# PreibischLab/multiview-simulation

Measured on AMD Instinct MI355X. Metric: simulated Mvoxel/s (views x input voxels / s), 512^3 volume x 8 views, higher is better.
Workload: dtype f32 (f64 attenuation/reductions/Poisson)

## Files before the change

include/mvsim.h:

```cpp
#ifndef MVSIM_H
#define MVSIM_H

#include <stddef.h>
#include <stdint.h>

#ifdef __cplusplus
extern "C" {
#endif

#define MVSIM_OK       0
#define MVSIM_EINVAL  (-1)
#define MVSIM_ENOMEM  (-2)
#define MVSIM_EHIP    (-3)
#define MVSIM_EFFT    (-4)
#define MVSIM_ERCCL   (-5)
#define MVSIM_ENODEV  (-6)

typedef struct mvsim_ctx mvsim_ctx;

const char* mvsim_version(void);
const char* mvsim_last_error(void);
int  mvsim_device_count(int* count);
int  mvsim_create(int device, mvsim_ctx** ctx);
int  mvsim_destroy(mvsim_ctx* ctx);
// ... 368 lines not shown
    int64_t  dim[3];
    int64_t  min[3], max[3];
    int32_t  inc;  float snr;
    uint64_t seed; uint32_t stream;
} mvsim_interval_job;
int mvsim_interval_out_dim(const mvsim_interval_job* job, int64_t out_dim[3]);
int mvsim_extract_intervals_dev(mvsim_ctx* ctx, const mvsim_interval_job* jobs, int n, float* const* out_dev);
int mvsim_extract_intervals(mvsim_ctx* ctx, const mvsim_interval_job* jobs, int n, float* const* out_host);
int mvsim_tile_interval(const int64_t dim[3], const double overlap_ratio[3], int tile,
                        int64_t min[3], int64_t max[3], int64_t overlap[3]);

typedef struct mvsim_view_params {
    int32_t  axis;
    int32_t  degrees;
    double   delta;
    float    min_value;
    float    target_average;
    int32_t  inc;
    float    snr;
    uint64_t seed;
    uint32_t stream;
    int32_t  conv_method;
} mvsim_view_params;

typedef struct mvsim_view_outputs {
    float* rot;
    float* att;
    float* con;
    float* acq;
} mvsim_view_outputs;

void mvsim_view_params_default(mvsim_view_params* p);

int mvsim_simulate_view_dev(mvsim_ctx* ctx, const float* gt, const int64_t dim[3],
                            float* psf_host, const int64_t kdim[3],
                            const mvsim_view_params* params, const mvsim_view_outputs* out,
                            double* correction);
int mvsim_simulate_views_dev(mvsim_ctx* ctx, const float* gt, const int64_t dim[3], float* const* psf_host,
                             const int64_t kdim[3], const mvsim_view_params* params, const mvsim_view_outputs* outs,
                             int n_views);
int mvsim_simulate_views(mvsim_ctx* ctx, const float* gt_host, const int64_t dim[3], float* const* psf_host,
                         const int64_t kdim[3], const mvsim_view_params* params, float* const* acq_host, int n_views);
typedef struct mvsim_iteration_outputs {
    float* iso;
    float* view;
    float* view_weights;
    float* view_psf;
} mvsim_iteration_outputs;
int mvsim_simulate_iteration_dev(mvsim_ctx* ctx, const float* gt, const int64_t dim[3],
                                 float* psf_host, const int64_t kdim[3],
                                 const mvsim_view_params* params, int back_degrees,
                                 const mvsim_view_outputs* out, const mvsim_iteration_outputs* more);
int mvsim_simulate_view(mvsim_ctx* ctx, const float* gt, const int64_t dim[3],
                        float* psf_host, const int64_t kdim[3],
                        const mvsim_view_params* params, const mvsim_view_outputs* out,
                        double* correction);

int mvsim_simulate_view_async(mvsim_ctx* ctx, const float* gt_host, uint64_t gt_generation, const int64_t dim[3],
                              float* psf_host, const int64_t kdim[3], const mvsim_view_params* params,
                              const mvsim_view_outputs* out_host, int64_t* ticket);
int mvsim_wait(mvsim_ctx* ctx, int64_t ticket, double* correction);
int mvsim_get_transfer_stats(mvsim_ctx* ctx, int64_t* views_as_u16, int64_t* fallbacks);
int mvsim_simulate_view_zslabs(mvsim_ctx* ctx, const float* const* gt_slabs, const int64_t* gt_slab_nz, int n_gt_slabs,
                               const int64_t dim[3], float* psf_host, const int64_t kdim[3],
                               const mvsim_view_params* params, float* const* acq_slabs, const int64_t* acq_slab_nz,
                               int n_acq_slabs, double* correction);

int mvsim_rotate_around_axis_zslabs(mvsim_ctx* ctx, const float* const* in_slabs, const int64_t* in_slab_nz, int n_in, const int64_t dim[3],
                                    int axis, int degrees, float* const* out_slabs, const int64_t* out_slab_nz, int n_out);
int mvsim_attenuate3d_zslabs(mvsim_ctx* ctx, const float* const* in_slabs, const int64_t* in_slab_nz, int n_in, const int64_t dim[3],
                             double delta, float* const* out_slabs, const int64_t* out_slab_nz, int n_out);
int mvsim_convolve_zslabs(mvsim_ctx* ctx, const float* const* in_slabs, const int64_t* in_slab_nz, int n_in, const int64_t dim[3],
                          float* psf, const int64_t kdim[3], int method, float* const* out_slabs, const int64_t* out_slab_nz, int n_out);
int mvsim_extract_slices_zslabs(mvsim_ctx* ctx, const float* const* in_slabs, const int64_t* in_slab_nz, int n_in, const int64_t dim[3],
                                int inc, float snr, uint64_t seed, uint32_t stream, float* const* out_slabs, const int64_t* out_slab_nz,
                                int n_out);

typedef struct mvsim_timings {
    float rotate_ms, attenuate_ms, psf_ms, convolve_ms, adjust_ms, extract_ms, total_ms;
    float pass_a_ms, pass_b_ms, pass_c_ms, pass_d_ms, pass_e_ms;
} mvsim_timings;
int mvsim_fft_geometry(const int64_t dim[3], const int64_t kdim[3], int64_t geometry[5]);
int mvsim_zpass_geometry(const int64_t dim[3], const int64_t kdim[3], int inc, int64_t out[4]);
int mvsim_stencil_geometry(const int64_t kdim[3], int64_t geometry[5]);
int mvsim_extract_path(const int64_t dim[3], int inc, int index_inc, uint64_t index_offset, int aligned16, int queue_share, int64_t path[4]);
int mvsim_get_extract_path(mvsim_ctx* ctx, int64_t path[5]);
int mvsim_fused_tail_geometry(mvsim_ctx* ctx, const int64_t dim[3], const int64_t kdim[3], int inc, int want_con, int64_t out[2]);
int mvsim_get_plane_stats(mvsim_ctx* ctx, int64_t stats[3]);
int mvsim_get_tail_path(mvsim_ctx* ctx, int64_t out[2]);
int mvsim_get_psf_cache_stats(mvsim_ctx* ctx, int64_t out[4]);
int mvsim_get_queue_stats(mvsim_ctx* ctx, int64_t stats[6]);
int mvsim_enable_timing(mvsim_ctx* ctx, int enable);
int mvsim_get_timings(mvsim_ctx* ctx, mvsim_timings* t);

#define MVSIM_UNIQUE_ID_BYTES 128
int mvsim_comm_unique_id(unsigned char id[MVSIM_UNIQUE_ID_BYTES]);
int mvsim_comm_init(mvsim_ctx* ctx, int nranks, int rank, const unsigned char id[MVSIM_UNIQUE_ID_BYTES]);
int mvsim_comm_library_info(char* path, size_t path_capacity, int* version);
int mvsim_comm_broadcast_volume(mvsim_ctx* ctx, float* vol_dev, int64_t count, int root);
int mvsim_comm_register_volume(mvsim_ctx* ctx, float* vol_dev, int64_t count);
typedef struct mvsim_bcast_op { int32_t stage, kind, peer, pad; int64_t first, count; } mvsim_bcast_op;
int mvsim_comm_broadcast_plan(int nranks, int rank, int root, int64_t count, int pieces, mvsim_bcast_op* ops, int capacity, int* n_ops);
int mvsim_comm_unregister_volume(mvsim_ctx* ctx, const float* vol_dev);
int mvsim_comm_allreduce_sum(mvsim_ctx* ctx, float* buf_dev, int64_t count);
int mvsim_comm_allreduce_sum_f64(mvsim_ctx* ctx, double* value_host);
int mvsim_comm_allreduce_sum_f64_dev(mvsim_ctx* ctx, double* value_dev, void* hip_stream);
int mvsim_comm_destroy(mvsim_ctx* ctx);
int mvsim_shard_views(int n_views, int nranks, int rank, int* view_idx, int max_out);

typedef struct mvsim_group mvsim_group;
int        mvsim_group_create(int ndev, const int* devices, mvsim_group** group);
int        mvsim_group_destroy(mvsim_group* group);
int        mvsim_group_size(const mvsim_group* group);
mvsim_ctx* mvsim_group_ctx(mvsim_group* group, int index);
int        mvsim_group_broadcast_volume(mvsim_group* group, const float* gt_host, const int64_t dim[3]);
int        mvsim_group_simulate_views(mvsim_group* group, float* const* psf_host, const int64_t kdim[3],
                                      const mvsim_view_params* params, int n_views, float* const* acq_host);

int mvsim_slab_range(int64_t nz, int nranks, int rank, int64_t* z0, int64_t* z1);
int mvsim_view_slab_convolve_dev(mvsim_ctx* ctx, const float* gt, const int64_t dim[3], float* psf_host,
                                 const int64_t kdim[3], const mvsim_view_params* params, int64_t z0, int64_t z1,
                                 double* slab_sum);
int mvsim_view_slab_finish_dev(mvsim_ctx* ctx, const int64_t dim[3], const mvsim_view_params* params, int64_t z0,
                               int64_t z1, double total_sum, float* acq, int64_t* n_planes);
int mvsim_view_slab_dev(mvsim_ctx* ctx, mvsim_ctx* comm_ctx, const float* gt, const int64_t dim[3], float* psf_host,
                        const int64_t kdim[3], const mvsim_view_params* params, int64_t z0, int64_t z1, float* acq,
                        int64_t* n_planes);

#ifdef __cplusplus
}
#endif
#endif
```

multiview-simulation_amd/__init__.py:

```python
from __future__ import annotations

import ctypes as C
import math
import os

import numpy as np

from . import _lib
from ._lib import DeconParams, DeconStat, IntervalJob, MvsimError, MvsimNoDeviceError, Sphere, Timings, ViewOutputs, ViewParams
from .aberrations import ContextAberrations
from .deconvolution import ContextDeconvolution, MultiViewDeconvolution, decon_geometry, decon_params, flip_psf
from .detection import ContextDetection, DifferenceOfGaussian, dog_geometry, dog_params, dog_taps
from ._lib import DogParams, MatchParams
from .registration import BeadRegistration, ContextRegistration, descriptor_subsets, fit_affine, match_geometry, match_params
from ._lib import FuseParams, FuseView
from .fusion import (ContextFusion, ViewFusion, fuse_invert, fuse_params, fusion_bounds, fusion_geometry, psf_matrix,
                     transform_psf)
from ._lib import PsfParams, PsfResult
from .psf import (ContextPsf, PsfExtraction, gaussian_psf, psf_finish, psf_geometry, psf_offsets, psf_params, psf_rendered,
                  psf_select)
from .phantoms import ContextPhantoms

__all__ = ["AffineTransform3D", "BeadRegistration", "Context", "DeconParams", "DifferenceOfGaussian", "DogParams", "MatchParams", "MultiViewDeconvolution", "Group", "Hessian", "HypersphereCollectionRealRandomAccessible", "JavaRandom", "Lightsheet",
           "PerlinNoiseRealRandomAccessible", "PointRejectionSampling", "RayTracingTest", "Raytrace", "RefractiveIndexMap", "ClearingMap", "SimpleCalculatedRealRandomAccessible", "SimulateBeads",
           "SimulateBeads2", "SimulateMultiViewAberrations", "SimulateMultiViewDataset", "Tools", "VolumeInjection", "broadcast_plan", "default_context", "MvsimError", "MvsimNoDeviceError", "ViewParams", "shard_views",
           "version", "zpass_geometry", "ViewFusion", "FuseParams", "PsfExtraction", "PsfParams"]


def broadcast_plan(nranks: int, rank: int, root: int, count: int, pieces: int = 8):
    L = _lib.load()
    n = C.c_int(0)
    _lib.check(L.mvsim_comm_broadcast_plan(nranks, rank, root, count, pieces, None, 0, C.byref(n)))
    ops = (_lib.BcastOp * max(1, n.value))()
    _lib.check(L.mvsim_comm_broadcast_plan(nranks, rank, root, count, pieces, ops, n.value, C.byref(n)))
    return [(o.stage, "send" if o.kind == 0 else "recv", o.peer, o.first, o.count) for o in ops[: n.value]]


def version() -> str:
    return _lib.load().mvsim_version().decode()


def zpass_geometry(dim_xyz, kdim_xyz, inc: int = 1):
    g = (C.c_int64 * 4)()
    rc = _lib.load().mvsim_zpass_geometry((C.c_int64 * 3)(*dim_xyz), (C.c_int64 * 3)(*kdim_xyz), int(inc), g)
    return tuple(int(x) for x in g) if rc == 0 else None


class JavaRandom:
    _MULT = 0x5DEECE66D
    _MASK = (1 << 48) - 1

    def __init__(self, seed: int):
        self.setSeed(seed)

    def setSeed(self, seed: int) -> None:
        self._s = (seed ^ self._MULT) & self._MASK
        self._pending = None

    def next(self, bits: int) -> int:
        self._s = (self._s * self._MULT + 0xB) & self._MASK
        v = self._s >> (48 - bits)
        v &= 0xFFFFFFFF
        return v - (1 << 32) if v & 0x80000000 else v

    def nextInt(self, bound: int | None = None) -> int:
        if bound is None:
            return self.next(32)
        if bound <= 0:
            raise ValueError("bound must be positive")
        r = self.next(31)
        m = bound - 1
        if bound & m == 0:
            return (bound * r) >> 31
        u = r
        while True:
            r = u % bound
            t = (u - r + m) & 0xFFFFFFFF
            if not (t & 0x80000000):
                return r
            u = self.next(31)

    def nextLong(self) -> int:
        v = ((self.next(32) << 32) + self.next(32)) & 0xFFFFFFFFFFFFFFFF
        return v - (1 << 64) if v & (1 << 63) else v

    def nextDouble(self) -> float:
        return ((self.next(26) << 27) + self.next(27)) * (1.0 / (1 << 53))

    def nextGaussian(self) -> float:
        from .phantoms import strict_log
        if self._pending is not None:
            g, self._pending = self._pending, None
            return g
        while True:
            v1 = 2 * self.nextDouble() - 1
            v2 = 2 * self.nextDouble() - 1
            s = v1 * v1 + v2 * v2
            if not (s >= 1 or s == 0):
                break
        multiplier = math.sqrt(-2 * strict_log(s) / s)
        self._pending = v2 * multiplier
        return v1 * multiplier

    def shuffle(self, lst: list) -> None:
        for i in range(len(lst), 1, -1):
            j = self.nextInt(i)
            lst[i - 1], lst[j] = lst[j], lst[i - 1]


def _seed_from(rnd) -> int:
    if rnd is None:
        rnd = SimulateMultiViewDataset.rnd
    if isinstance(rnd, int):
        return rnd & 0xFFFFFFFFFFFFFFFF
    return rnd.nextLong() & 0xFFFFFFFFFFFFFFFF


def _as_volume(a, name="image") -> np.ndarray:
    v = np.ascontiguousarray(a, dtype=np.float32)
    if v.ndim != 3:
        raise ValueError(f"{name}: expected 3 dimensions, got {v.ndim}")
    if v.size == 0:
        raise ValueError(f"{name}: empty interval")
    return v


def _dim(v: np.ndarray):
    nz, ny, nx = v.shape
# ... 1069 lines not shown
```

multiview-simulation_amd/_lib.py:

```python
from __future__ import annotations

import ctypes as C
import os

HERE = os.path.dirname(os.path.abspath(__file__))
LIB_PATH = os.path.join(HERE, "libmvsim.so")

MVSIM_OK, MVSIM_EINVAL, MVSIM_ENOMEM, MVSIM_EHIP, MVSIM_EFFT, MVSIM_ERCCL, MVSIM_ENODEV = 0, -1, -2, -3, -4, -5, -6
UNIQUE_ID_BYTES = 128


class MvsimError(RuntimeError):

    def __init__(self, status: int, message: str):
        super().__init__(f"libmvsim status {status}: {message}")
        self.status = status


class MvsimNoDeviceError(MvsimError):
    pass


class ViewParams(C.Structure):
    _fields_ = [
# ... 125 lines not shown
    def as_dict(self):
        return {n: float(getattr(self, n)) for n, _ in self._fields_}


_i64p = C.POINTER(C.c_int64)
_vp = C.c_void_p
_dp = C.POINTER(C.c_double)

SIGNATURES = {
    "mvsim_version": (C.c_char_p, []),
    "mvsim_last_error": (C.c_char_p, []),
    "mvsim_device_count": (C.c_int, [C.POINTER(C.c_int)]),
    "mvsim_create": (C.c_int, [C.c_int, C.POINTER(_vp)]),
    "mvsim_destroy": (C.c_int, [_vp]),
    "mvsim_set_stream": (C.c_int, [_vp, _vp]),
    "mvsim_synchronize": (C.c_int, [_vp]),
    "mvsim_join": (C.c_int, [_vp]),
    "mvsim_set_option": (C.c_int, [_vp, C.c_char_p, C.c_char_p]),
    "mvsim_release_caches": (C.c_int, [_vp]),
    "mvsim_dev_alloc": (C.c_int, [_vp, C.c_size_t, C.POINTER(_vp)]),
    "mvsim_dev_free": (C.c_int, [_vp, _vp]),
    "mvsim_upload": (C.c_int, [_vp, _vp, _vp, C.c_size_t]),
    "mvsim_dev_memset": (C.c_int, [_vp, _vp, C.c_int, C.c_size_t]),
    "mvsim_host_alloc": (C.c_int, [_vp, C.c_size_t, C.POINTER(C.c_void_p)]),
    "mvsim_host_free": (C.c_int, [_vp, _vp]),
    "mvsim_download": (C.c_int, [_vp, _vp, _vp, C.c_size_t]),
    "mvsim_axis_rotation": (C.c_int, [_i64p, C.c_int, C.c_int, C.POINTER(C.c_double)]),
    "mvsim_extract_nz": (C.c_int64, [C.c_int64, C.c_int]),
    "mvsim_isotropic_nz": (C.c_int64, [C.c_int64, C.c_int]),
    "mvsim_poisson_mul": (C.c_double, [C.c_double]),
    "mvsim_rotate_around_axis": (C.c_int, [_vp, _vp, _i64p, C.c_int, C.c_int, _vp]),
    "mvsim_attenuate3d": (C.c_int, [_vp, _vp, _i64p, C.c_double, _vp]),
    "mvsim_norm_image": (C.c_int, [_vp, _vp, C.c_int64]),
    "mvsim_convolve": (C.c_int, [_vp, _vp, _i64p, _vp, _i64p, C.c_int, _vp]),
    "mvsim_adjust_image": (C.c_int, [_vp, _vp, C.c_int64, C.c_float, C.c_float, C.POINTER(C.c_double)]),
    "mvsim_extract_slices": (C.c_int, [_vp, _vp, _i64p, C.c_int, C.c_float, C.c_uint64, C.c_uint32, _vp]),
    "mvsim_poisson_process": (C.c_int, [_vp, _vp, C.c_int64, C.c_double, C.c_uint64, C.c_uint32, C.c_uint64]),
    "mvsim_make_isotropic": (C.c_int, [_vp, _vp, _i64p, C.c_int, _vp]),
    "mvsim_compute_weight_image": (C.c_int, [_vp, _i64p, _vp]),
    "mvsim_rotate_around_axis_dev": (C.c_int, [_vp, _vp, _i64p, C.c_int, C.c_int, _vp]),
    "mvsim_attenuate3d_dev": (C.c_int, [_vp, _vp, _i64p, C.c_double, _vp]),
    "mvsim_convolve_dev": (C.c_int, [_vp, _vp, _i64p, _vp, _i64p, C.c_int, _vp]),
    "mvsim_adjust_image_dev": (C.c_int, [_vp, _vp, C.c_int64, C.c_float, C.c_float, C.POINTER(C.c_double)]),
    "mvsim_extract_slices_dev": (C.c_int, [_vp, _vp, _i64p, C.c_int, C.c_float, C.c_uint64, C.c_uint32, _vp]),
    "mvsim_make_isotropic_dev": (C.c_int, [_vp, _vp, _i64p, C.c_int, _vp]),
    "mvsim_interval_out_dim": (C.c_int, [C.POINTER(IntervalJob), _i64p]),
    "mvsim_extract_intervals_dev": (C.c_int, [_vp, C.POINTER(IntervalJob), C.c_int, C.POINTER(_vp)]),
    "mvsim_extract_intervals": (C.c_int, [_vp, C.POINTER(IntervalJob), C.c_int, C.POINTER(_vp)]),
    "mvsim_tile_interval": (C.c_int, [_i64p, _dp, C.c_int, _i64p, _i64p, _i64p]),
    "mvsim_draw_spheres": (C.c_int, [_vp, _vp, _i64p, C.c_double, C.c_double, C.c_int, C.c_int,
                                     C.POINTER(C.c_uint64), C.POINTER(C.c_int64)]),
    "mvsim_draw_spheres_dev": (C.c_int, [_vp, _vp, _i64p, C.c_double, C.c_double, C.c_int, C.c_int,
                                         C.POINTER(C.c_uint64), C.POINTER(C.c_int64)]),
    "mvsim_downsample2x": (C.c_int, [_vp, _vp, _i64p, _vp]),
    "mvsim_downsample2x_dev": (C.c_int, [_vp, _vp, _i64p, _vp]),
    "mvsim_compute_weight_image_dev": (C.c_int, [_vp, _i64p, _vp]),
    "mvsim_sum_views_dev": (C.c_int, [_vp, C.POINTER(_vp), C.c_int, C.c_int64, _vp]),
    "mvsim_normalize_weights_dev": (C.c_int, [_vp, C.POINTER(_vp), C.c_int, C.c_int64, _vp, C.c_float]),
    "mvsim_normalize_weights": (C.c_int, [_vp, C.POINTER(_vp), C.c_int, C.c_int64, C.c_float]),
    "mvsim_view_params_default": (None, [C.POINTER(ViewParams)]),
    "mvsim_simulate_view_dev": (C.c_int, [_vp, _vp, _i64p, _vp, _i64p, C.POINTER(ViewParams),
                                          C.POINTER(ViewOutputs), C.POINTER(C.c_double)]),
    "mvsim_get_plane_stats": (C.c_int, [_vp, _i64p]),
    "mvsim_get_tail_path": (C.c_int, [_vp, _i64p]),
    "mvsim_get_psf_cache_stats": (C.c_int, [_vp, _i64p]),
    "mvsim_get_queue_stats": (C.c_int, [_vp, _i64p]),
    "mvsim_get_transfer_stats": (C.c_int, [_vp, C.POINTER(C.c_int64), C.POINTER(C.c_int64)]),
    "mvsim_simulate_views_dev": (C.c_int, [_vp, _vp, _i64p, C.POINTER(_vp), _i64p, C.POINTER(ViewParams),
                                           C.POINTER(ViewOutputs), C.c_int]),
    "mvsim_simulate_views": (C.c_int, [_vp, _vp, _i64p, C.POINTER(_vp), _i64p, C.POINTER(ViewParams), C.POINTER(_vp), C.c_int]),
    "mvsim_simulate_iteration_dev": (C.c_int, [_vp, _vp, _i64p, _vp, _i64p, C.POINTER(ViewParams), C.c_int,
                                               C.POINTER(ViewOutputs), C.POINTER(IterationOutputs)]),
    "mvsim_simulate_view": (C.c_int, [_vp, _vp, _i64p, _vp, _i64p, C.POINTER(ViewParams),
                                      C.POINTER(ViewOutputs), C.POINTER(C.c_double)]),
    "mvsim_splat_spheres": (C.c_int, [_vp, _vp, _i64p, _vp, C.c_int64]),
    "mvsim_splat_spheres_dev": (C.c_int, [_vp, _vp, _i64p, _vp, C.c_int64]),
    "mvsim_simulate_view_async": (C.c_int, [_vp, _vp, C.c_uint64, _i64p, _vp, _i64p, C.POINTER(ViewParams),
                                            C.POINTER(ViewOutputs), C.POINTER(C.c_int64)]),
    "mvsim_wait": (C.c_int, [_vp, C.c_int64, C.POINTER(C.c_double)]),
    "mvsim_simulate_view_zslabs": (C.c_int, [_vp, C.POINTER(_vp), _i64p, C.c_int, _i64p, _vp, _i64p, C.POINTER(ViewParams),
                                             C.POINTER(_vp), _i64p, C.c_int, C.POINTER(C.c_double)]),
    "mvsim_fft_geometry": (C.c_int, [_i64p, _i64p, _i64p]),
    "mvsim_zpass_geometry": (C.c_int, [_i64p, _i64p, C.c_int, _i64p]),
    "mvsim_rotate_around_axis_zslabs": (C.c_int, [_vp, C.POINTER(_vp), _i64p, C.c_int, _i64p, C.c_int, C.c_int, C.POINTER(_vp), _i64p, C.c_int]),
    "mvsim_attenuate3d_zslabs": (C.c_int, [_vp, C.POINTER(_vp), _i64p, C.c_int, _i64p, C.c_double, C.POINTER(_vp), _i64p, C.c_int]),
    "mvsim_convolve_zslabs": (C.c_int, [_vp, C.POINTER(_vp), _i64p, C.c_int, _i64p, _vp, _i64p, C.c_int, C.POINTER(_vp), _i64p, C.c_int]),
    "mvsim_extract_slices_zslabs": (C.c_int, [_vp, C.POINTER(_vp), _i64p, C.c_int, _i64p, C.c_int, C.c_float, C.c_uint64, C.c_uint32,
                                              C.POINTER(_vp), _i64p, C.c_int]),
    "mvsim_stencil_geometry": (C.c_int, [_i64p, _i64p]),
    "mvsim_extract_path": (C.c_int, [_i64p, C.c_int, C.c_int, C.c_uint64, C.c_int, C.c_int, _i64p]),
    "mvsim_fused_tail_geometry": (C.c_int, [_vp, _i64p, _i64p, C.c_int, C.c_int, _i64p]),
    "mvsim_get_extract_path": (C.c_int, [_vp, _i64p]),
    "mvsim_enable_timing": (C.c_int, [_vp, C.c_int]),
    "mvsim_get_timings": (C.c_int, [_vp, C.POINTER(Timings)]),
    "mvsim_comm_unique_id": (C.c_int, [C.POINTER(C.c_ubyte)]),
    "mvsim_comm_init": (C.c_int, [_vp, C.c_int, C.c_int, C.POINTER(C.c_ubyte)]),
    "mvsim_comm_library_info": (C.c_int, [C.c_char_p, C.c_size_t, C.POINTER(C.c_int)]),
    "mvsim_comm_broadcast_volume": (C.c_int, [_vp, _vp, C.c_int64, C.c_int]),
    "mvsim_comm_broadcast_plan": (C.c_int, [C.c_int, C.c_int, C.c_int, C.c_int64, C.c_int, _vp, C.c_int, C.POINTER(C.c_int)]),
    "mvsim_comm_register_volume": (C.c_int, [_vp, _vp, C.c_int64]),
    "mvsim_comm_unregister_volume": (C.c_int, [_vp, _vp]),
    "mvsim_comm_allreduce_sum": (C.c_int, [_vp, _vp, C.c_int64]),
    "mvsim_comm_allreduce_sum_f64": (C.c_int, [_vp, C.POINTER(C.c_double)]),
    "mvsim_slab_range": (C.c_int, [C.c_int64, C.c_int, C.c_int, C.POINTER(C.c_int64), C.POINTER(C.c_int64)]),
    "mvsim_view_slab_convolve_dev": (C.c_int, [_vp, _vp, _i64p, _vp, _i64p, _vp, C.c_int64, C.c_int64,
                                               C.POINTER(C.c_double)]),
    "mvsim_view_slab_finish_dev": (C.c_int, [_vp, _i64p, _vp, C.c_int64, C.c_int64, C.c_double, _vp,
                                             C.POINTER(C.c_int64)]),
    "mvsim_view_slab_dev": (C.c_int, [_vp, _vp, _vp, _i64p, _vp, _i64p, _vp, C.c_int64, C.c_int64, _vp, C.POINTER(C.c_int64)]),
    "mvsim_comm_allreduce_sum_f64_dev": (C.c_int, [_vp, _vp, _vp]),
    "mvsim_host_copy": (C.c_int, [_vp, _vp, _vp, C.c_size_t]),
    "mvsim_comm_destroy": (C.c_int, [_vp]),
    "mvsim_group_create": (C.c_int, [C.c_int, C.POINTER(C.c_int), C.POINTER(_vp)]),
    "mvsim_group_destroy": (C.c_int, [_vp]),
    "mvsim_group_size": (C.c_int, [_vp]),
    "mvsim_group_ctx": (_vp, [_vp, C.c_int]),
    "mvsim_group_broadcast_volume": (C.c_int, [_vp, _vp, _i64p]),
    "mvsim_group_simulate_views": (C.c_int, [_vp, C.POINTER(_vp), _i64p, C.POINTER(ViewParams), C.c_int, C.POINTER(_vp)]),
    "mvsim_shard_views": (C.c_int, [C.c_int, C.c_int, C.c_int, C.POINTER(C.c_int), C.c_int]),
    "mvsim_beads_random_points": (C.c_int, [C.POINTER(C.c_uint64), C.c_int64, _i64p, _i64p, C.POINTER(C.c_double)]),
    "mvsim_render_beads": (C.c_int, [_vp, C.POINTER(C.c_double), _i64p, C.c_int64, C.POINTER(C.c_double), C.c_int, _i64p, _i64p,
                                     C.POINTER(C.c_double), C.POINTER(_vp), C.POINTER(_vp)]),
    "mvsim_render_beads_dev": (C.c_int, [_vp, C.POINTER(C.c_double), _i64p, C.c_int64, C.POINTER(C.c_double), C.c_int, _i64p, _i64p,
                                         C.POINTER(C.c_double), C.POINTER(_vp), C.POINTER(_vp)]),
    "mvsim_beads_normalize": (C.c_int, [_vp, _vp, C.c_int64]),
    "mvsim_beads_normalize_dev": (C.c_int, [_vp, _vp, C.c_int64]),
    "mvsim_perlin_init": (C.c_int, [C.POINTER(C.c_uint64), C.c_int32, _dp, C.POINTER(C.c_int32), _dp]),
    "mvsim_perlin_at": (C.c_int, [_vp, C.POINTER(Perlin), _vp, C.c_int64, _vp]),
    "mvsim_perlin_at_dev": (C.c_int, [_vp, C.POINTER(Perlin), _vp, C.c_int64, _vp]),
    "mvsim_perlin_raster": (C.c_int, [_vp, C.POINTER(Perlin), _i64p, _i64p, _vp]),
    "mvsim_perlin_raster_dev": (C.c_int, [_vp, C.POINTER(Perlin), _i64p, _i64p, _vp]),
    "mvsim_spheres_at": (C.c_int, [_vp, C.POINTER(SphereSet), _vp, C.c_int64, _vp]),
    "mvsim_spheres_at_dev": (C.c_int, [_vp, C.POINTER(SphereSet), _vp, C.c_int64, _vp]),
    "mvsim_spheres_raster": (C.c_int, [_vp, C.POINTER(SphereSet), _i64p, _i64p, C.c_int, _vp]),
    "mvsim_spheres_raster_dev": (C.c_int, [_vp, C.POINTER(SphereSet), _i64p, _i64p, C.c_int, _vp]),
    "mvsim_rejection_sample": (C.c_int, [_vp, C.POINTER(C.c_uint64), _dp, _dp, C.c_int64, C.POINTER(Density), C.c_int64, _dp,
                                         C.POINTER(C.c_int64)]),
    "mvsim_lightsheet_fit": (C.c_int, [C.c_double, C.c_double, C.c_double, C.c_double, _dp]),
    "mvsim_hessian_at": (C.c_int, [_vp, _vp, _i64p, _dp, C.c_int64, _dp, _dp, _dp]),
    "mvsim_hessian_at_dev": (C.c_int, [_vp, _vp, _i64p, _dp, C.c_int64, _dp, _dp, _dp]),
    "mvsim_hessian_images": (C.c_int, [_vp, _vp, _i64p, _vp, _vp]),
    "mvsim_hessian_images_dev": (C.c_int, [_vp, _vp, _i64p, _vp, _vp]),
    "mvsim_refract3d_ray_starts": (C.c_int, [_vp, C.POINTER(C.c_uint64), _i64p, C.c_int, C.c_int, _dp, C.c_int64, _dp, _dp]),
    "mvsim_camera_ray_starts": (C.c_int, [_vp, C.POINTER(C.c_uint64), _i64p, C.c_int, _dp]),
    "mvsim_refract3d": (C.c_int, [_vp, _vp, _vp, _i64p, C.c_int, C.c_int, C.c_double, C.c_double, C.c_double, C.c_int64,
                                  C.POINTER(C.c_uint64), _vp, _vp, C.POINTER(RaySteps)]),
    "mvsim_refract3d_dev": (C.c_int, [_vp, _vp, _vp, _i64p, C.c_int, C.c_int, C.c_double, C.c_double, C.c_double, C.c_int64,
                                      C.POINTER(C.c_uint64), _vp, _vp, C.POINTER(RaySteps)]),
    "mvsim_trace_params_default": (C.c_int, [_i64p, C.POINTER(TraceParams)]),
    "mvsim_trace_rays": (C.c_int, [_vp, _vp, _vp, _i64p, _dp, _dp, C.POINTER(C.c_float), C.c_int64, C.POINTER(TraceParams), _vp, _vp,
                                   C.POINTER(RaySteps), _dp, _dp, C.POINTER(C.c_int64)]),
    "mvsim_trace_rays_dev": (C.c_int, [_vp, _vp, _vp, _i64p, _dp, _dp, C.POINTER(C.c_float), C.c_int64, C.POINTER(TraceParams), _vp, _vp,
                                       C.POINTER(RaySteps), _dp, _dp, C.POINTER(C.c_int64)]),
    "mvsim_sandbox_ray_starts": (C.c_int, [_vp, C.POINTER(C.c_uint64), _i64p, C.c_int, C.c_int, C.c_int64, _dp, _dp]),
    "mvsim_grid_ray_starts": (C.c_int, [_vp, _i64p, C.c_int, C.c_int, C.c_int64, _dp, _dp, C.POINTER(C.c_int64)]),
    "mvsim_draw_simple_image": (C.c_int, [_vp, _vp, _i64p, C.c_float, C.c_float]),
    "mvsim_draw_simple_image_dev": (C.c_int, [_vp, _vp, _i64p, C.c_float, C.c_float]),
    "mvsim_hessian_plane": (C.c_int, [_vp, _vp, _i64p, C.c_int, _vp, _vp]),
    "mvsim_hessian_plane_dev": (C.c_int, [_vp, _vp, _i64p, C.c_int, _vp, _vp]),
    "mvsim_volume_inject": (C.c_int, [_vp, _vp, _vp, _i64p, _dp, _dp, _dp, C.c_int64, C.c_int]),
    "mvsim_volume_inject_dev": (C.c_int, [_vp, _vp, _vp, _i64p, _dp, _dp, _dp, C.c_int64, C.c_int]),
    "mvsim_volume_inject_info": (C.c_int, [_dp, C.POINTER(C.c_int32), _dp, C.POINTER(C.c_int32)]),
    "mvsim_volume_normalize": (C.c_int, [_vp, _vp, _vp, C.c_int64, _vp]),
    "mvsim_volume_normalize_dev": (C.c_int, [_vp, _vp, _vp, C.c_int64, _vp]),
    "mvsim_volume_project": (C.c_int, [_vp, _vp, _vp, _i64p, _vp]),
    "mvsim_volume_project_dev": (C.c_int, [_vp, _vp, _vp, _i64p, _vp]),
# ... 90 lines not shown
```

multiview-simulation_amd/build.py:

```python
from __future__ import annotations

import os
import shutil
import subprocess
import sys

HERE = os.path.dirname(os.path.abspath(__file__))
CSRC = os.path.join(HERE, "csrc")
LIB = os.path.join(HERE, "libmvsim.so")
SOURCES = ["api.cpp", "api_view.cpp", "api_host.cpp", "api_sims.cpp", "comm.cpp", "kernels.hip", "rotate.hip", "extract.hip", "extract_interval.hip", "fftconv.hip", "fft_driver.hip", "fft_passes.hip", "zconv.hip", "rotate_fft.hip", "stencil.hip", "phantom.hip", "beads.hip", "aberrations.hip", "raytrace.hip", "procedural.hip", "sphere_walk.hip", "api_decon.cpp", "deconvolve.hip", "api_detect.cpp", "detect.hip", "api_register.cpp", "register.hip", "api_fuse.cpp", "fuse.hip", "api_psf.cpp", "psf.hip"]
HEADERS = ["common.h", "api_internal.h", "host_pool.h", "jrandom.h", "extract_plan.h", "interval_plan.h", "poisson_dev.h", "poisson_recipe.h", "fft_dev.h", "fft_host.h", "rotate_rounds.h", "row_bits.h", "rotate_dev.h", "sphere_walk.h", "aberr_dev.h", "bricks.h", "decon.h", "detect.h", "register.h", "register_dev.h", "fuse.h", "fuse_dev.h", "psf.h", "psf_dev.h", "psf_cache.h", "../../include/mvsim.h"]
ROCM = os.environ.get("ROCM_PATH", "/opt/rocm")


def _hipcc() -> str:
    for cand in (os.path.join(ROCM, "bin", "hipcc"), shutil.which("hipcc")):
        if cand and os.path.exists(cand):
            return cand
    raise RuntimeError("hipcc not found (ROCm toolchain required to build libmvsim.so)")


def sources():
    return [os.path.join(CSRC, s) for s in SOURCES if os.path.exists(os.path.join(CSRC, s))]


def source_sha() -> str:
    import hashlib
    h = hashlib.sha256()
    files = sorted(sources() + [os.path.normpath(os.path.join(CSRC, x)) for x in HEADERS])
    for f in files:
        h.update(os.path.basename(f).encode() + b"\0")
        with open(f, "rb") as fh:
            h.update(fh.read())
    return h.hexdigest()[:16]


def _common_flags():
    return [
        "--offload-arch=gfx950", "-O3", "-std=c++17", "-fPIC", "-ffp-contract=off", "-fno-fast-math",
        *os.environ.get("MVSIM_EXTRA_CFLAGS", "").split(),
        "-Wall", "-Wno-unused-result", "-I" + os.path.join(ROCM, "include"),
    ]


def is_current() -> bool:
    if not os.path.exists(LIB) or not os.path.exists(LIB + ".flags"):
        return False
    with open(LIB + ".flags") as fh:
        if fh.read() != " ".join(_common_flags()):
            return False
    t = os.path.getmtime(LIB)
    deps = sources() + [os.path.normpath(os.path.join(CSRC, h)) for h in HEADERS] + [os.path.abspath(__file__)]
    return all(os.path.getmtime(d) <= t for d in deps if os.path.exists(d))


def build(force: bool = False, verbose: bool = False) -> str:
    if not force and is_current():
        return LIB
    hipcc = _hipcc()
    objs = []
    os.makedirs(os.path.join(HERE, "build"), exist_ok=True)
    common = _common_flags()
    flags_id = " ".join(common)
    hdr_time = max(os.path.getmtime(os.path.normpath(os.path.join(CSRC, h))) for h in HEADERS)
    hdr_time = max(hdr_time, os.path.getmtime(os.path.abspath(__file__)))
    procs = []
    for src in sources():
        obj = os.path.join(HERE, "build", os.path.basename(src) + ".o")
        objs.append(obj)
        stamp = obj + ".flags"
        fresh = (not force and os.path.exists(obj) and os.path.exists(stamp) and open(stamp).read() == flags_id
                 and os.path.getmtime(obj) >= max(os.path.getmtime(src), hdr_time))
        if fresh:
            continue
        cmd = [hipcc, "-x", "hip", "-c", src, "-o", obj] + common
        if verbose:
            print(" ".join(cmd), file=sys.stderr)
        procs.append((src, stamp, subprocess.Popen(cmd, stdout=subprocess.PIPE, stderr=subprocess.STDOUT, text=True)))
    failed = False
    for src, stamp, p in procs:
        out, _ = p.communicate()
        if p.returncode != 0:
            failed = True
            if os.path.exists(stamp):
                os.remove(stamp)
            sys.stderr.write(f"--- {src} ---\n{out}\n")
        else:
            with open(stamp, "w") as fh:
                fh.write(flags_id)
            if verbose and out.strip():
                sys.stderr.write(out)
    if failed:
        raise RuntimeError("hipcc failed")
    link = [hipcc, "-shared", "-fPIC", "--offload-arch=gfx950", "-o", LIB] + objs + [
# ... 13 lines not shown
```

multiview-simulation_amd/csrc/api.cpp:

```cpp
#include "api_internal.h"

#include <cstdlib>
#include <mutex>
#include <thread>

namespace mvsim {

static thread_local char g_err[512] = "";

void set_error(const char* fmt, ...)
{
    va_list ap;
    va_start(ap, fmt);
    vsnprintf(g_err, sizeof(g_err), fmt, ap);
    va_end(ap);
}

int parse_option(Options& o, const char* name, const char* value)
{
    if (!name || !value) return MVSIM_EINVAL;
    const std::string n(name), v(value);
    auto word = [&](std::initializer_list<std::pair<const char*, int>> words, auto* dst) {
        for (const auto& w : words)
            if (v == w.first) { *dst = w.second; return MVSIM_OK; }
        return MVSIM_EINVAL;
    };
    auto flag = [&](bool* dst) { return word({{"1", 1}, {"on", 1}, {"true", 1}, {"0", 0}, {"off", 0}, {"false", 0}}, dst); };
    auto number = [&](size_t digits, long long lo, long long hi, auto* dst, int when_auto = -1) {
        if (when_auto >= 0 && v == "auto") { *dst = when_auto; return MVSIM_OK; }
        if (v.empty() || v.size() > digits || v.find_first_not_of("0123456789") != std::string::npos) return MVSIM_EINVAL;
        const long long k = atoll(v.c_str());
        if (k < lo || k > hi) return MVSIM_EINVAL;
        *dst = k;
        return MVSIM_OK;
    };
    if (n == "fft_zpass") return word({{"auto", 0}, {"direct", 1}, {"fft", 2}, {"inline", 3}}, &o.zpass);
    if (n == "fft_backend") return word({{"custom", 0}, {"auto", 0}, {"rocfft", 1}}, &o.rocfft);
    if (n == "fused_rotate") return word({{"1", 1}, {"on", 1}, {"lds", 1}, {"0", 0}, {"off", 0}, {"2", 2}, {"lane", 2}, {"3", 3}, {"auto", 3}}, &o.fused_rotate);
    if (n == "poisson_queue") return word({{"1", 1}, {"on", 1}, {"0", 0}, {"off", 0}}, &o.poisson_queue);
    if (n == "poisson_queue_share") return number(2, 1, 16, &o.poisson_queue_share, 0);
    if (n == "attenuate") return word({{"serial", 0}, {"scan", 1}}, &o.attenuate_scan);
    if (n == "early_sum") return flag(&o.early_sum);
    if (n == "zconv_strided") return flag(&o.zconv_strided);
    if (n == "exp") return number(2, 0, 15, &o.exp);
    if (n == "beads_pair_cap") return number(10, 1024, 1LL << 31, &o.beads_pair_cap);
    if (n == "reject_batch") return number(7, 1, 1LL << 20, &o.reject_batch, 0);
    if (n == "dog_pass") return word({{"both", 0}, {"xy", 1}, {"z", 2}}, &o.dog_pass);
    if (n == "sphere_walk") return word({{"host", 0}, {"device", 1}, {"device_only", 2}, {"auto", -1}}, &o.sphere_walk);
    if (n == "fuse_tail") return flag(&o.fuse_tail);
    if (n == "psf_overlap") return flag(&o.psf_overlap);
    if (n == "fused_fftx") return word({{"auto", 2}, {"1", 1}, {"on", 1}, {"0", 0}, {"off", 0}, {"roles", 3}}, &o.fused_fftx);
    if (n == "tail_overlap") return word({{"0", 0}, {"off", 0}, {"1", 1}, {"on", 1}, {"own", 1}, {"2", 2}, {"any", 2}}, &o.tail_overlap);
    if (n == "acq_transfer") return word({{"auto", 1}, {"u16", 1}, {"f32", 0}}, &o.acq_u16);
    if (n == "host_threads") return number(3, 1, 256, &o.host_threads, 0);
    if (n == "view_batch") return word({{"auto", 2}, {"1", 1}, {"on", 1}, {"0", 0}, {"off", 0}}, &o.view_batch);
    if (n == "view_lanes") return number(2, 1, MVSIM_MAX_VIEWS, &o.view_lanes, 0);
    if (n == "graph") { bool g = false; const int rc = flag(&g); o.graph = g ? 1 : 0; return rc; }
    if (n == "broadcast") {
        int how = 0;
        if (word({{"scatter_allgather", 0}, {"auto", 0}, {"ring", 1}, {"peer_copy", 2}, {"pipelined", 3}}, &how) != MVSIM_OK) return MVSIM_EINVAL;
        o.bcast_ring = how == 1; o.bcast_peer_copy = how == 2; o.bcast_pipelined = how == 3;
        return MVSIM_OK;
    }
    if (n == "skip_empty") return flag(&o.skip_empty);
    if (n == "skip_rows") return flag(&o.skip_rows);
    if (n == "skip_tail") return flag(&o.skip_tail);
    if (n == "psf_cache") return number(7, 0, 1 << 20, &o.psf_cache);
    if (n == "fft_pad") {
        long long a = 0, b = 0, c = 0;
        if (v == "auto" || v.empty()) { o.fft_pad[0] = o.fft_pad[1] = o.fft_pad[2] = 0; return MVSIM_OK; }
        if (sscanf(v.c_str(), "%lld,%lld,%lld", &a, &b, &c) != 3 || a < 0 || b < 0 || c < 0) return MVSIM_EINVAL;
        o.fft_pad[0] = a; o.fft_pad[1] = b; o.fft_pad[2] = c;
        return MVSIM_OK;
    }
    return MVSIM_EINVAL;
}

const Options& env_options()
{
    static Options o;
    static std::once_flag once;
    std::call_once(once, [] {
        if (const char* e = getenv("MVSIM_FFT_ZPASS")) (void)parse_option(o, "fft_zpass", e);
        if (const char* e = getenv("MVSIM_FFT_BACKEND")) (void)parse_option(o, "fft_backend", e);
        if (const char* e = getenv("MVSIM_FFT_PAD")) (void)parse_option(o, "fft_pad", e);
        if (getenv("MVSIM_NO_FUSED_ROTATE")) o.fused_rotate = 0;
        if (getenv("MVSIM_POISSON_NOQUEUE")) o.poisson_queue = 0;
        if (getenv("MVSIM_NO_EARLY_SUM")) o.early_sum = false;
        if (getenv("MVSIM_NO_FUSE_TAIL")) o.fuse_tail = false;
        if (const char* e = getenv("MVSIM_GRAPH")) (void)parse_option(o, "graph", e);
        if (const char* e = getenv("MVSIM_BROADCAST")) (void)parse_option(o, "broadcast", e);
        if (const char* e = getenv("MVSIM_OPTIONS")) {
            std::string all(e);
            size_t pos = 0;
            while (pos < all.size()) {
                size_t end = all.find(';', pos);
                if (end == std::string::npos) end = all.size();
                const std::string kv = all.substr(pos, end - pos);
                const size_t eq = kv.find('=');
                if (eq != std::string::npos) (void)parse_option(o, kv.substr(0, eq).c_str(), kv.substr(eq + 1).c_str());
                pos = end + 1;
            }
        }
    });
    return o;
}

int ensure_lds_attr(mvsim_ctx* ctx, const void* kernel, size_t bytes)
{
    if (bytes <= 64 * 1024) return MVSIM_OK;
    if (bytes > 160 * 1024) { set_error("kernel needs %zu bytes of LDS (> 160 KiB)", bytes); return MVSIM_EINVAL; }
    if (ctx->lds_attr_set.count(kernel)) return MVSIM_OK;
    MVSIM_HIP(hipFuncSetAttribute(kernel, hipFuncAttributeMaxDynamicSharedMemorySize, 160 * 1024));
    ctx->lds_attr_set.insert(kernel);
    return MVSIM_OK;
}

int DevBuf::reserve(size_t need)
{
    if (need <= bytes) return MVSIM_OK;
    if (epoch) *epoch += 1;
    if (p) { (void)hipFree(p); p = nullptr; bytes = 0; }
    hipError_t e = hipMalloc(&p, need);
    if (e != hipSuccess) {
        p = nullptr;
        set_error("hipMalloc(%zu bytes) failed: %s", need, hipGetErrorString(e));
// ... 799 lines not shown
    if (fallbacks) *fallbacks = ctx->u16_fallbacks;
    return MVSIM_OK;
}

int mvsim_stencil_geometry(const int64_t kdim[3], int64_t geometry[5])
{
    if (!kdim || !geometry) { set_error("invalid argument: null pointer"); return MVSIM_EINVAL; }
    if (!stencil_chunk_geometry(kdim, geometry)) {
        set_error("direct stencil: PSF outside 1..64 taps per axis");
        return MVSIM_EINVAL;
    }
    return MVSIM_OK;
}

int mvsim_extract_path(const int64_t dim[3], int inc, int index_inc, uint64_t index_offset, int aligned16, int queue_share, int64_t path[4])
{
    if (!dim || !path) { set_error("invalid argument: null pointer"); return MVSIM_EINVAL; }
    MVSIM_TRY(check_dim(dim));
    MVSIM_CHECK_ARG(inc >= 1 && index_inc >= 0, "inc must be >= 1 and index_inc >= 0");
    MVSIM_CHECK_ARG(0 <= queue_share && queue_share <= 16, "queue_share must be 0 (no queue) or 1..16 sixteenths");
    extract_path(dim, inc, index_inc, index_offset, aligned16 != 0, queue_share, path);
    return MVSIM_OK;
}

int mvsim_get_extract_path(mvsim_ctx* ctx, int64_t path[5])
{
    MVSIM_CHECK_ARG(ctx != nullptr && path != nullptr, "null pointer");
    std::memcpy(path, ctx->extract_path, sizeof(ctx->extract_path));
    return MVSIM_OK;
}

int mvsim_get_tail_path(mvsim_ctx* ctx, int64_t out[2])
{
    MVSIM_CHECK_ARG(ctx != nullptr && out != nullptr, "null pointer");
    out[0] = ctx->tail_path[0]; out[1] = ctx->tail_path[1];
    return MVSIM_OK;
}

int mvsim_get_psf_cache_stats(mvsim_ctx* ctx, int64_t out[4])
{
    MVSIM_CHECK_ARG(ctx != nullptr && out != nullptr, "null pointer");
    const PsfCache::Stats& st = ctx->psf_cache.stats();
    out[0] = st.hits; out[1] = st.misses; out[2] = st.evictions; out[3] = st.bytes;
    return MVSIM_OK;
}

int mvsim_fused_tail_geometry(mvsim_ctx* ctx, const int64_t dim[3], const int64_t kdim[3], int inc, int want_con, int64_t out[2])
{
    MVSIM_CHECK_ARG(ctx != nullptr && dim && kdim && out, "null pointer");
    MVSIM_TRY(check_dim(dim));
    MVSIM_CHECK_ARG(inc >= 1, "inc must be >= 1");
    ExtractPlan fp{};
    if (!ctx->opt.fuse_tail || ctx->opt.poisson_queue != 1 || !fused_tail_geometry(dim, kdim, inc, want_con != 0, ctx->opt, &fp)) {
        set_error("this view would not take the fused tail");
        return MVSIM_EINVAL;
    }
    out[0] = fp.blocks; out[1] = fp.segcap;
    return MVSIM_OK;
}

int mvsim_fft_geometry(const int64_t dim[3], const int64_t kdim[3], int64_t geometry[5])
{
    if (!dim || !kdim || !geometry) { set_error("invalid argument: null pointer"); return MVSIM_EINVAL; }
    MVSIM_TRY(check_dim(dim));
    if (!custom_fft_geometry(dim, kdim, geometry, env_options())) {
        set_error("no hand-written FFT size for this volume / PSF");
        return MVSIM_EINVAL;
    }
    return MVSIM_OK;
}

int mvsim_zpass_geometry(const int64_t dim[3], const int64_t kdim[3], int inc, int64_t out[4])
{
    if (!dim || !kdim || !out) { set_error("invalid argument: null pointer"); return MVSIM_EINVAL; }
    MVSIM_TRY(check_dim(dim));
    MVSIM_CHECK_ARG(inc >= 1, "inc must be >= 1");
    if (!custom_zpass_geometry(dim, kdim, inc, out, env_options())) {
        set_error("this view's z pass is not the direct convolution");
        return MVSIM_EINVAL;
    }
    return MVSIM_OK;
}

int mvsim_enable_timing(mvsim_ctx* ctx, int enable)
{
    MVSIM_TRY(set_device(ctx));
    if (enable && !ctx->ev_created) {
        for (int k = 0; k < mvsim_ctx::TIMING_SLOTS; ++k)
            for (int s = 0; s < ST_COUNT; ++s) {
                MVSIM_HIP(hipEventCreate(&ctx->evr[k][s][0]));
                MVSIM_HIP(hipEventCreate(&ctx->evr[k][s][1]));
            }
        ctx->ev_created = true;
    }
    ctx->timing = enable != 0;
    ctx->ev_cur = 0;
    ctx->ev_calls = 0;
    for (int s = 0; s < ST_COUNT; ++s) ctx->ev_used[0][s] = false;
    return MVSIM_OK;
}

int mvsim_get_timings(mvsim_ctx* ctx, mvsim_timings* t)
{
    MVSIM_TRY(set_device(ctx));
    MVSIM_CHECK_ARG(t != nullptr, "timings pointer is null");
    MVSIM_CHECK_ARG(ctx->ev_created, "timing was never enabled");
    MVSIM_HIP(hipStreamSynchronize(ctx->stream));
    double sum[ST_COUNT] = {};
    int cnt[ST_COUNT] = {};
    const long long calls = ctx->ev_calls == 0 ? 1 : ctx->ev_calls;
    const int nslots = (int)(calls < mvsim_ctx::TIMING_SLOTS ? calls : mvsim_ctx::TIMING_SLOTS);
    for (int j = 0; j < nslots; ++j) {
        const int k = ((ctx->ev_cur - j) % mvsim_ctx::TIMING_SLOTS + mvsim_ctx::TIMING_SLOTS) % mvsim_ctx::TIMING_SLOTS;
        for (int s = 0; s < ST_COUNT; ++s) {
            if (!ctx->ev_used[k][s]) continue;
            float ms = 0.f;
            MVSIM_HIP(hipEventElapsedTime(&ms, ctx->evr[k][s][0], ctx->evr[k][s][1]));
            sum[s] += ms;
            cnt[s] += 1;
            ctx->ev_used[k][s] = false;
        }
    }
    float ms[ST_COUNT];
    float total = 0.f;
    for (int s = 0; s < ST_COUNT; ++s) {
        ms[s] = cnt[s] ? (float)(sum[s] / cnt[s]) : 0.f;
        if (s == ST_PSF && cnt[ST_CONVOLVE] > cnt[s]) ms[s] = (float)(sum[s] / cnt[ST_CONVOLVE]);
        if (s == ST_PSF && ctx->psf_on_side) ms[s] = 0.f;
        if (s < ST_PASS_A) total += ms[s];
    }
    t->rotate_ms = ms[ST_ROTATE]; t->attenuate_ms = ms[ST_ATTENUATE]; t->psf_ms = ms[ST_PSF];
    t->convolve_ms = ms[ST_CONVOLVE]; t->adjust_ms = ms[ST_ADJUST]; t->extract_ms = ms[ST_EXTRACT];
    t->total_ms = total;
    t->pass_a_ms = ms[ST_PASS_A]; t->pass_b_ms = ms[ST_PASS_B]; t->pass_c_ms = ms[ST_PASS_C];
    t->pass_d_ms = ms[ST_PASS_D]; t->pass_e_ms = ms[ST_PASS_E];
    ctx->last = *t;
    ctx->ev_cur = 0;
    ctx->ev_calls = 0;
    return MVSIM_OK;
}

}
```

multiview-simulation_amd/csrc/api_view.cpp:

```cpp
#include "api_internal.h"

using namespace mvsim;

void mvsim::view_graphs_release(mvsim_ctx* ctx)
{
    for (auto& g : ctx->graphs) {
        if (g.exec) (void)hipGraphExecDestroy(g.exec);
        if (g.graph) (void)hipGraphDestroy(g.graph);
    }
    ctx->graphs.clear();
    ctx->graph_seen.clear();
}

extern "C" {

static bool ranges_meet(const void* a, size_t abytes, const char* lo, const char* hi)
{
    const char* p = reinterpret_cast<const char*>(a);
    return a && lo && p < hi && lo < p + abytes;
}

static int view_enqueue(mvsim_ctx* ctx, const float* gt, const int64_t dim[3], const int64_t kdim[3], const mvsim_view_params* p,
                        const mvsim_view_outputs* o, bool overlap_ok = false)
{
// ... 45 lines not shown
    const int method = pick_method(p->conv_method, kdim);
    const bool materialise = o->con != nullptr;
    const bool noise = p->snr >= 0.0f;
    ConvTail tail;
    tail.zstride = (!materialise && p->inc > 1 && (!noise || ctx->opt.poisson_queue == 1)) ? p->inc : 1;
    tail.corr_n = n; tail.min_value = p->min_value; tail.target_average = p->target_average;
    tail.x_done = x_done;
    tail.plane_nz = x_done ? plane_nz : nullptr;
    tail.row_bits = x_done ? row_bits : nullptr;
    tail.want_sparse = tail.plane_nz != nullptr &&
                       tail_sparse_caller(ctx->opt.skip_tail, materialise, extract_stage_queued(ctx, dim, p->inc, noise));
    if (method == 1 && ctx->opt.fuse_tail && (!noise || ctx->opt.poisson_queue == 1)) {
        const size_t qb = noise ? fused_tail_queue_bytes(dim, kdim, p->inc, materialise, ctx->opt) : 0;
        if (!noise || qb > 0) {
            if (qb) MVSIM_TRY(ctx->pqueue.reserve(qb));
            tail.want_fuse = true;
            tail.min_value = p->min_value; tail.target_average = p->target_average;
            tail.con_adj = materialise ? con : nullptr;
            tail.acq = o->acq; tail.inc = p->inc; tail.noise = noise;
            tail.mul = mvsim_poisson_mul((double)p->snr); tail.seed = p->seed; tail.stream = p->stream;
        }
    }
    MVSIM_TRY(convolve_dev_impl(ctx, att, dim, kdim, method, con, &tail));
    if (tail.fused) {
        const int64_t fused[5] = {EXTRACT_FUSED_TAIL, 0, tail.fused_blocks, noise ? (int64_t)tail.fused_segcap : 0, 1};
        std::memcpy(ctx->extract_path, fused, sizeof(fused));
        ctx->tail_path[0] = ctx->tail_path[1] = 0;
        return MVSIM_OK;
    }
    if (tail.sparse && (materialise || method != 1)) { set_error("sparse tail behind a view that did not ask for it"); return MVSIM_EINVAL; }

    ev_begin(ctx, ST_ADJUST);
    if (method == 2) MVSIM_TRY(launch_sum(ctx->stream, con, n, partial, scal));
    if (!tail.corr_done) MVSIM_TRY(launch_adjust_corr(ctx->stream, scal, n, p->min_value, p->target_average));
    if (materialise) MVSIM_TRY(launch_adjust_apply(ctx->stream, con, n, scal, p->min_value));
    ev_end(ctx, ST_ADJUST);

    const int64_t n_out = dim[0] * dim[1] * mvsim_extract_nz(dim[2], p->inc);
    ExtractOps ops;
    ops.in = con; ops.out = o->acq; ops.scal = scal;
    ops.min_value = p->min_value; ops.noise = noise; ops.mul = mvsim_poisson_mul((double)p->snr); ops.seed = p->seed; ops.stream = p->stream;
    ops.adjust = !materialise;
    if (tail.sparse) { ops.empty_flags = tail.sparse_flags; ops.empty_stride = tail.sparse_stride; }
    ExtractPlan xpl;
    MVSIM_TRY(extract_stage_plan(ctx, tail.zstride > 1 ? ExtractGeom::compact(dim, p->inc) : ExtractGeom::strided(dim, p->inc), ops, &xpl));
    if (x_done) overlap_ok = false;
    if (tail.sparse) overlap_ok = false;
    hipStream_t tail_on = ctx->stream;
    if (overlap_ok) {
        if (!ctx->tail_stream) {
            MVSIM_HIP(hipStreamCreateWithFlags(&ctx->tail_stream, hipStreamNonBlocking));
            MVSIM_HIP(hipEventCreateWithFlags(&ctx->ev_tail_fork, hipEventDisableTiming));
            MVSIM_HIP(hipEventCreateWithFlags(&ctx->ev_tail, hipEventDisableTiming));
        }
        MVSIM_HIP(hipEventRecord(ctx->ev_tail_fork, ctx->stream));
        MVSIM_HIP(hipStreamWaitEvent(ctx->tail_stream, ctx->ev_tail_fork, 0));
        tail_on = ctx->tail_stream;
    }
    StreamSwap swap(ctx, tail_on);
    MVSIM_TRY(extract_stage_run(ctx, xpl, ops));
    if (overlap_ok) {
        MVSIM_HIP(hipEventRecord(ctx->ev_tail, ctx->tail_stream));
        ctx->tail_pending = true;
        ctx->tail_lo[0] = reinterpret_cast<const char*>(o->acq); ctx->tail_hi[0] = ctx->tail_lo[0] + (size_t)n_out * sizeof(float);
        ctx->tail_lo[1] = reinterpret_cast<const char*>(con);    ctx->tail_hi[1] = ctx->tail_lo[1] + vbytes;
    }
    return MVSIM_OK;
}


static std::string view_graph_key(mvsim_ctx* ctx, const float* gt, const int64_t dim[3], const int64_t kdim[3],
                                  const mvsim_view_params* p, const mvsim_view_outputs* o)
{
    std::string k;
    auto add = [&](const void* ptr, size_t bytes) { k.append(reinterpret_cast<const char*>(ptr), bytes); };
    add(&gt, sizeof(gt)); add(dim, 3 * sizeof(int64_t)); add(kdim, 3 * sizeof(int64_t));
    add(&p->axis, sizeof(p->axis)); add(&p->degrees, sizeof(p->degrees)); add(&p->delta, sizeof(p->delta));
    add(&p->min_value, sizeof(p->min_value)); add(&p->target_average, sizeof(p->target_average)); add(&p->inc, sizeof(p->inc));
    add(&p->snr, sizeof(p->snr)); add(&p->seed, sizeof(p->seed)); add(&p->stream, sizeof(p->stream));
    add(&p->conv_method, sizeof(p->conv_method));
    add(&o->rot, sizeof(o->rot)); add(&o->att, sizeof(o->att)); add(&o->con, sizeof(o->con)); add(&o->acq, sizeof(o->acq));
    add(&ctx->stream, sizeof(ctx->stream));
    const Options& q = ctx->opt;
    const int oo[16] = {q.zpass, q.rocfft ? 1 : 0, q.fused_rotate, q.poisson_queue, q.early_sum ? 1 : 0, q.fuse_tail ? 1 : 0, q.psf_overlap ? 1 : 0,
                        q.attenuate_scan ? 1 : 0, q.fused_fftx, q.zconv_strided ? 1 : 0, q.skip_empty ? 1 : 0, q.exp, q.poisson_queue_share, ctx->queue_share_learned,
                        q.skip_rows ? 1 : 0, q.skip_tail ? 1 : 0};
    add(oo, sizeof(oo));
    add(q.fft_pad, sizeof(q.fft_pad));
    return k;
}

static int view_graph_launch(mvsim_ctx* ctx, const float* gt, const int64_t dim[3], const int64_t kdim[3], const mvsim_view_params* p,
                             const mvsim_view_outputs* o)
{
    const std::string key = view_graph_key(ctx, gt, dim, kdim, p, o);
    ctx->graph_tick += 1;
    const unsigned long long epoch = ctx->alloc_epoch;
    if (ctx->graph_epoch != epoch) {
        for (auto& g : ctx->graphs) { (void)hipGraphExecDestroy(g.exec); (void)hipGraphDestroy(g.graph); }
        ctx->graphs.clear();
        ctx->graph_epoch = epoch;
    }
    for (auto& g : ctx->graphs)
        if (g.key == key) {
            g.last_use = ctx->graph_tick;
            MVSIM_HIP(hipGraphLaunch(g.exec, ctx->stream));
            return MVSIM_OK;
        }
    if (!ctx->graph_seen.count(key)) {
        if (ctx->graph_seen.size() > 4096) ctx->graph_seen.clear();
        ctx->graph_seen.insert(key);
        return view_enqueue(ctx, gt, dim, kdim, p, o);
    }
    MVSIM_HIP(hipStreamBeginCapture(ctx->stream, hipStreamCaptureModeRelaxed));
    const int rc = view_enqueue(ctx, gt, dim, kdim, p, o);
    hipGraph_t graph = nullptr;
    const hipError_t e = hipStreamEndCapture(ctx->stream, &graph);
    if (rc != MVSIM_OK) { if (graph) (void)hipGraphDestroy(graph); return rc; }
    if (ctx->alloc_epoch != epoch) {
        if (graph) (void)hipGraphDestroy(graph);
        return view_enqueue(ctx, gt, dim, kdim, p, o);
    }
    if (e != hipSuccess || !graph) { set_error("hipStreamEndCapture failed: %s", hipGetErrorString(e)); return MVSIM_EHIP; }
    hipGraphExec_t exec = nullptr;
    const hipError_t ei = hipGraphInstantiate(&exec, graph, nullptr, nullptr, 0);
    if (ei != hipSuccess) { (void)hipGraphDestroy(graph); set_error("hipGraphInstantiate failed: %s", hipGetErrorString(ei)); return MVSIM_EHIP; }
    if (ctx->graphs.size() >= 32) {
        size_t victim = 0;
        for (size_t i = 1; i < ctx->graphs.size(); ++i) if (ctx->graphs[i].last_use < ctx->graphs[victim].last_use) victim = i;
        (void)hipGraphExecDestroy(ctx->graphs[victim].exec);
        (void)hipGraphDestroy(ctx->graphs[victim].graph);
        ctx->graphs.erase(ctx->graphs.begin() + (long)victim);
    }
    ctx->graphs.push_back(mvsim_ctx::ViewGraph{key, graph, exec, ctx->graph_tick});
    MVSIM_HIP(hipGraphLaunch(exec, ctx->stream));
    return MVSIM_OK;
}

static int simulate_view_dev(mvsim_ctx* ctx, const float* gt, const int64_t dim[3], float* psf_host, const int64_t kdim[3],
                             const mvsim_view_params* p, const mvsim_view_outputs* o, double* correction, bool keep_psf_dev)
{
    MVSIM_TRY(set_device(ctx, true));
    const bool overlap = ctx->opt.tail_overlap != 0 && (ctx->opt.tail_overlap == 2 || ctx->stream == ctx->own_stream) &&
                         !ctx->opt.graph && !correction && dim &&
                         dim[0] > 0 && dim[1] > 0 && dim[2] > 0 && dim[0] * dim[1] * dim[2] >= ((int64_t)1 << 24);
    if (!overlap) MVSIM_TRY(join_tail(ctx));
    MVSIM_TRY(check_dim(dim));
    MVSIM_CHECK_ARG(gt && p && o, "null pointer");
    MVSIM_CHECK_ARG(o->acq != nullptr, "outputs.acq is required");
    MVSIM_CHECK_ARG(p->axis >= 0 && p->axis <= 2, "axis must be 0, 1 or 2");
    MVSIM_CHECK_ARG(p->inc >= 1, "inc must be >= 1");
    MVSIM_CHECK_ARG(p->conv_method >= 0 && p->conv_method <= 2, "conv_method must be 0, 1 or 2");
    MVSIM_CHECK_ARG(dim[0] <= dim[1], "attenuate3d: Nx > Ny walks outside the interval in the reference");
    ev_next(ctx);
    MVSIM_TRY(psf_prepare(ctx, psf_host, kdim, dim, !keep_psf_dev && kdim && pick_method(p->conv_method, kdim) == 1));
    int64_t P[3];
    const bool capturable = pick_method(p->conv_method, kdim) == 2 || custom_fft_sizes(dim, kdim, P, ctx->opt);
    if (ctx->opt.graph && !ctx->timing && capturable) MVSIM_TRY(view_graph_launch(ctx, gt, dim, kdim, p, o));
    else MVSIM_TRY(view_enqueue(ctx, gt, dim, kdim, p, o, overlap));
    if (correction) {
        double *partial, *scal;
        MVSIM_TRY(scal_ptr(ctx, &partial, &scal));
        MVSIM_HIP(hipMemcpyAsync(correction, scal + 1, sizeof(double), hipMemcpyDeviceToHost, ctx->stream));
        MVSIM_HIP(hipStreamSynchronize(ctx->stream));
    }
    return MVSIM_OK;
}

int mvsim_simulate_view_dev(mvsim_ctx* ctx, const float* gt, const int64_t dim[3], float* psf_host,
// ... 367 lines not shown
```

multiview-simulation_amd/csrc/common.h:

```cpp
#pragma once

#include <hip/hip_runtime.h>
#include <rocfft/rocfft.h>
#include <roctracer/roctx.h>

#include <algorithm>
#include <array>
#include <cstdarg>
#include <cstdint>
#include <cstdio>
#include <map>
#include <string>
#include <type_traits>
#include <unordered_set>
#include <utility>
#include <vector>

#include "../../include/mvsim.h"
#include "extract_plan.h"
#include "interval_plan.h"
#include "psf_cache.h"
#include "rotate_dev.h"
#include "sphere_walk.h"

// ... 37 lines not shown
    do {                                                                                        \
        int rc_ = (expr);                                                                       \
        if (rc_ != MVSIM_OK) return rc_;                                                        \
    } while (0)

#define MVSIM_CHECK_ARG(cond, msg)                                                              \
    do {                                                                                        \
        if (!(cond)) {                                                                          \
            mvsim::set_error("invalid argument: %s", msg);                                      \
            return MVSIM_EINVAL;                                                                \
        }                                                                                       \
    } while (0)

struct DevBuf {
    void*  p     = nullptr;
    size_t bytes = 0;
    unsigned long long* epoch = nullptr;
    int    reserve(size_t need);
    void   release();
    template <class T> T* as() const { return reinterpret_cast<T*>(p); }
};

struct Scratch {
    DevBuf b[12];
    ~Scratch() { for (DevBuf& x : b) x.release(); }
};

inline int suggested_kernel_diameter(double sigma)
{
    if (!(sigma > 0)) return 3;
    const int s = 2 * (int)(3 * sigma + 0.5) + 1;
    return s > 3 ? s : 3;
}

inline bool affine_is_x_rotation(const Affine& a)
{
    return a.m[0] == 1.0 && a.m[1] == 0.0 && a.m[2] == 0.0 && a.m[3] == 0.0 && a.m[4] == 0.0 && a.m[8] == 0.0;
}

struct FftPlan {
    int64_t      P[3]      = {0, 0, 0};
    rocfft_plan  fwd       = nullptr;
    rocfft_plan  inv       = nullptr;
    rocfft_execution_info info = nullptr;
    size_t       work_bytes = 0;
};

struct PinnedRing {
    static constexpr int SLOTS = 4;
    void*      p[SLOTS]     = {};
    size_t     bytes[SLOTS] = {};
    hipEvent_t ev[SLOTS]    = {};
    bool       busy[SLOTS]  = {};
    int        next         = 0;
    int  acquire(size_t need, int* slot);
    void release_all();
};

struct CountsStaging {
    DevBuf dev;
    void*  host       = nullptr;
    size_t host_bytes = 0;
    std::vector<long long> count;
    std::vector<size_t>    body;
    std::vector<char>      packed;
    int  reserve(const long long* counts, int views);
    int  pack(hipStream_t s, int view, const float* src);
    int  fetch(hipStream_t s);
    int  land(mvsim_ctx* ctx, const float* const* src_dev, float* const* dst_host);
    void release();
};

struct Options {
    int     zpass = 0;
    bool    rocfft = false;
    int     fused_rotate = 3;
    int     fused_fftx = 2;
    bool    attenuate_scan = false;
    int     poisson_queue = 1;
    int     poisson_queue_share = 16;
    bool    early_sum = true;
    int     exp = 0;
    bool    zconv_strided = true;
    bool    psf_overlap = true;
    int     tail_overlap = 1;
    bool    fuse_tail = false;
    int     graph = 0;
    int     acq_u16 = 1;
    int     host_threads = 0;
    int     view_lanes = 0;
    int     view_batch = 2;
    bool    bcast_ring = false;
    bool    bcast_peer_copy = false;
    bool    bcast_pipelined = false;
    int64_t fft_pad[3] = {0, 0, 0};
    bool    skip_empty = true;
    bool    skip_rows = true;
    int     psf_cache = 1024;
    bool    skip_tail = true;
    int64_t beads_pair_cap = (int64_t)1 << 28;
    int64_t reject_batch = 0;
    int     dog_pass = 0;
    int     sphere_walk = -1;
};
const Options& env_options();
int parse_option(Options& o, const char* name, const char* value);

enum Stage { ST_ROTATE = 0, ST_ATTENUATE, ST_PSF, ST_CONVOLVE, ST_ADJUST, ST_EXTRACT, ST_PASS_A, ST_PASS_B, ST_PASS_C, ST_PASS_D,
             ST_PASS_E, ST_COUNT };

}

struct mvsim_ctx {
    mvsim_ctx();
    mvsim_ctx(const mvsim_ctx&) = delete;
    mvsim_ctx& operator=(const mvsim_ctx&) = delete;
    template <class F> void each_workspace(F&& f);
    unsigned long long alloc_epoch = 1;
    int         roctx_depth = 0;
    int         device     = 0;
    hipStream_t own_stream = nullptr;
    hipStream_t stream     = nullptr;
    int         num_cu     = 256;

    mvsim::DevBuf vol_a, vol_b, vol_c;
    mvsim::DevBuf out_buf;
    mvsim::DevBuf psf_dev;
    mvsim::PsfCache psf_cache;
    mvsim::PsfCache::Entry* psf_entry = nullptr;
    mvsim::DevBuf view_tab;
    mvsim::DevBuf interval_tab;
    mvsim::DevBuf stencil_psf;
    mvsim::PinnedRing pinned;
    mvsim::DevBuf fft_real;
    mvsim::DevBuf fft_spec_img, fft_spec_psf;
    mvsim::DevBuf fft_work;
    mvsim::DevBuf pqueue;
    mvsim::DevBuf sphere_list;
    mvsim::DevBuf beads_buf[8];
    mvsim::DevBuf proc_buf[10];
    mvsim::DevBuf walk_buf[4];
    mvsim::DevBuf plane_flags;
    int*          empty_hint = nullptr;
    unsigned int* queue_hint = nullptr;
    int           queue_share_learned = 0;
    int64_t       extract_path[5] = {-1, 0, 0, 0, 0};
    int64_t       tail_path[2] = {0, 0};
    int           views_since_flags = 0;
    mvsim::DevBuf weight_img;
    mvsim::DevBuf decon_work[2];
    mvsim::DevBuf decon_psf;
    mvsim::DevBuf decon_stat;
    mvsim::DevBuf detect_buf[6];
    mvsim::DevBuf register_buf[4];
    mvsim::DevBuf fuse_buf;
    mvsim::DevBuf psfx_buf[3];
    int64_t       weight_dim[3] = {0, 0, 0};
    mvsim::DevBuf host_gt, host_rot, host_att, host_con;
    mvsim::DevBuf partials;
    mvsim::DevBuf partials_e;
    mvsim::DevBuf cfft_f, cfft_g;
    mvsim::DevBuf cfft_g1, cfft_g2;
    mvsim::Options opt;
    std::unordered_set<const void*> lds_attr_set;
    std::map<std::string, void*> box_weights;
    mvsim::DevBuf partials_z;
// ... 193 lines not shown
                     int rays_per_pixel, int64_t n, double* pos3, double* dir3);
int aberr_hessian_at_dev(mvsim_ctx* ctx, const float* img, const int64_t dim[3], const double* xyz, int64_t n, double* matrix9,
                         double* eigvec3, double* eigval);
int aberr_hessian_images_dev(mvsim_ctx* ctx, const float* img, const int64_t dim[3], int z0, int planes, float* eigval, float* eigvec);
int64_t trace_rays_per_range(int64_t pair_cap, int64_t max_moves);
struct StepRanges {
    Scratch ws;
    int64_t rays_per_range = 0, max_rays = 0;
    int     max_moves = 0;
    double *slot_xyz = nullptr, *xyz = nullptr;
    float  *slot_val = nullptr, *val = nullptr;
    int    *moves = nullptr, *offs = nullptr;
    int reserve(mvsim_ctx* ctx, int64_t nrays, int max_moves);
    int finish(mvsim_ctx* ctx, const char* who, int64_t r0, int nr, const int64_t dim[3], const double sigma[3], double sumw, float* image,
               float* weight, mvsim_ray_steps* steps);
};
int trace_rays_dev(mvsim_ctx* ctx, const float* ri_img, const float* img, const int64_t dim[3], const double* pos3, const double* dir3,
                   const float* intensity, int64_t n, const mvsim_trace_params* tp, double sumw, float* image, float* weight,
                   mvsim_ray_steps* steps, double* end_pos3, double* end_dir3, int64_t* n_capped);
int trace_ray_starts(mvsim_ctx* ctx, int bundle, uint64_t state, const int64_t dim[3], int x, int z, int64_t n, double* pos3, double* dir3);
int draw_simple_image_dev(mvsim_ctx* ctx, float* out, const int64_t dim[3], float low, float high);
int aberr_normalize_dev(mvsim_ctx* ctx, const float* image, const float* weight, int64_t n, float* out);
int aberr_project_dev(mvsim_ctx* ctx, const float* image, const float* weight, const int64_t dim[3], float* proj);
int launch_weight_image(hipStream_t s, float* out, const int64_t dim[3]);
int launch_weights(hipStream_t s, float* const* views, int nv, int64_t n, const float* sum_in, float* sum_out,
                   float osem, bool sum_only);

int launch_pad_mirror(hipStream_t s, const float* img, const int64_t dim[3], const int64_t kdim[3],
                      float* padded, const int64_t P[3]);
int launch_psf_embed(hipStream_t s, const float* psf, const int64_t kdim[3], float* padded, const int64_t P[3]);
int launch_cmul(hipStream_t s, float2* f, const float2* g, int64_t n);
int launch_crop_scale_sum(hipStream_t s, const float* real, const int64_t P[3], float* out,
                          const int64_t dim[3], float scale, double* partial, double* scal);
int launch_stencil(mvsim_ctx* ctx, const float* img, const int64_t dim[3], const float* psf,
                   const int64_t kdim[3], float* out);
bool stencil_chunk_geometry(const int64_t kdim[3], int64_t out[5]);
int ensure_lds_attr(mvsim_ctx* ctx, const void* kernel, size_t bytes);

struct ConvTail {
    int views = 1;
    int zstride = 1;
    bool     want_fuse = false;
    float    min_value = 0.f, target_average = 1.f;
    float*   con_adj = nullptr;
    float*   acq = nullptr;
    int      inc = 1;
    bool     noise = false;
    double   mul = 0.0;
    uint64_t seed = 0;
    uint32_t stream = 0;
    bool     fused = false;
    long long    fused_blocks = 0;
    unsigned int fused_segcap = 0;
    bool     x_done = false;
    long long corr_n = 0;
    bool      corr_done = false;
    const int* plane_nz = nullptr;
    const unsigned int* row_bits = nullptr;
    bool       want_sparse = false;
    bool       sparse = false;
    const int* sparse_flags = nullptr;
    int        sparse_stride = 0;
};
size_t fused_tail_queue_bytes(const int64_t dim[3], const int64_t kdim[3], int inc, bool con_wanted, const Options& opt);
int comm_allreduce_f64_on_stream(mvsim_ctx* cc, double* value_dev, hipStream_t s);
int rotate_attenuate_fftx(mvsim_ctx* ctx, const float* gt, float* rot_or_null, float* att_or_null, const int64_t dim[3],
                          const int64_t kdim[3], const Affine& inv, double delta, bool* done, const int** plane_nz = nullptr,
                          int z_first = 0, int nzl = -1, const unsigned int** row_bits = nullptr);
int fft_convolve(mvsim_ctx* ctx, const float* img_dev, const int64_t dim[3], const float* psf_dev,
                 const int64_t kdim[3], float* out_dev, ConvTail* tail);
void fft_release(mvsim_ctx* ctx);
void choose_padded(const int64_t dim[3], const int64_t kdim[3], int64_t P[3], const Options& opt);
bool custom_fft_sizes(const int64_t dim[3], const int64_t kdim[3], int64_t P[3], const Options& opt);
int  join_tail(mvsim_ctx* ctx);
struct ConvPlan {
    int     n[3], k[3];
    int64_t P[3];
    int     px, py, pz, M;
    int     tile_y, tile_z;
    bool    zdirect;
    bool    ymirror;
    bool    early;
    bool    zinline_auto;
    int     hxp, pyb;
    int     e_rows;
    size_t spectrum_bytes(int nz_in, int nz_out, int nz_pitch, int views) const
    {
        const size_t planes = zdirect ? (size_t)views * std::max(nz_in, std::max(nz_out, nz_pitch)) : (size_t)pz;
        return (size_t)hxp * (zdirect ? pyb : py) * planes * sizeof(float2);
    }
};
bool conv_plan(const int64_t dim[3], const int64_t kdim[3], const Options& opt, ConvPlan* pl);
int  custom_fft_convolve(mvsim_ctx* ctx, const float* img, const int64_t dim[3], const float* psf,
                         const int64_t kdim[3], float* out, ConvTail* tail);
struct SlabRange {
    int z_in0, nz_in, z_out0, nz_out;
};
int  custom_fft_convolve_slab(mvsim_ctx* ctx, const float* img, const int64_t dim[3], const float* psf,
                              const int64_t kdim[3], const SlabRange& slab, float* out, ConvTail* tail);
void custom_fft_release(mvsim_ctx* ctx);
bool custom_fft_geometry(const int64_t dim[3], const int64_t kdim[3], int64_t g[5], const Options& opt);
bool custom_zpass_geometry(const int64_t dim[3], const int64_t kdim[3], int inc, int64_t g[4], const Options& opt);
bool fused_tail_geometry(const int64_t dim[3], const int64_t kdim[3], int inc, bool con_wanted, const Options& opt, ExtractPlan* fp);
bool custom_fft_batchable(const mvsim_ctx* ctx, const int64_t dim[3], const int64_t kdim[3]);

inline const char* stage_name(int st)
{
    static const char* const names[ST_COUNT] = {"mvsim:rotate", "mvsim:attenuate", "mvsim:psf_spectrum", "mvsim:convolve", "mvsim:adjust",
                                               "mvsim:extract_poisson", "mvsim:pass_A_x_r2c", "mvsim:pass_B_y_fwd", "mvsim:pass_C_z",
                                               "mvsim:pass_D_y_inv", "mvsim:pass_E_x_c2r"};
    return names[st];
}
inline void ev_begin(mvsim_ctx* ctx, int st)
{
    (void)roctxRangePushA(stage_name(st));
    ctx->roctx_depth += 1;
    if (ctx->timing) (void)hipEventRecord(ctx->evr[ctx->ev_cur][st][0], ctx->stream);
}
inline void ev_end(mvsim_ctx* ctx, int st)
{
    if (ctx->roctx_depth > 0) { (void)roctxRangePop(); ctx->roctx_depth -= 1; }
    if (ctx->timing) {
        (void)hipEventRecord(ctx->evr[ctx->ev_cur][st][1], ctx->stream);
        ctx->ev_used[ctx->ev_cur][st] = true;
    }
}
inline void ev_rebalance(mvsim_ctx* ctx)
{
    while (ctx->roctx_depth > 0) { (void)roctxRangePop(); ctx->roctx_depth -= 1; }
}
inline void ev_next(mvsim_ctx* ctx)
{
    if (!ctx->timing) return;
    if (ctx->ev_calls > 0) ctx->ev_cur = (ctx->ev_cur + 1) % mvsim_ctx::TIMING_SLOTS;
    ctx->ev_calls += 1;
    for (int s = 0; s < ST_COUNT; ++s) ctx->ev_used[ctx->ev_cur][s] = false;
}

constexpr int SCAL_DOUBLES = 2 * MVSIM_MAX_VIEWS;
constexpr size_t PARTIALS_BYTES = (size_t)(SUM_BLOCKS + SCAL_DOUBLES + 8) * sizeof(double);
inline double* scal_of(mvsim_ctx* ctx, int view = 0) { return ctx->partials.as<double>() + SUM_BLOCKS + 2 * view; }

void comm_forget_range(mvsim_ctx* ctx, const void* p, size_t bytes);

void axis_rotation_host(const int64_t dim[3], int axis, int degrees, double m[12]);
void affine_invert_host(const double m[12], double inv[12]);

}
```

multiview-simulation_amd/csrc/fft_driver.hip:

```cpp
#include "fft_host.h"

#include <algorithm>
#include <cmath>
#include <cstdlib>
#include <cstring>

namespace mvsim {
namespace fft {

#ifndef MVSIM_ZINLINE_MIN_KZ
#define MVSIM_ZINLINE_MIN_KZ 48
#endif

__global__ __launch_bounds__(1024) void k_plane_flags_finish(const int* __restrict__ flags, int n, int kz, int c, unsigned int* __restrict__ bits,
                                                             int nwords, int* __restrict__ dil, int* __restrict__ empty_hint)
{
    __shared__ unsigned char sf[16384];
    __shared__ int cnt, cnt_dil;
    const int t = threadIdx.x;
    const bool in_lds = n <= 16384;
    if (t == 0) { cnt = 0; cnt_dil = 0; }
    __syncthreads();
    int mine = 0;
    for (int z = t; z < n; z += 1024) {
// ... 36 lines not shown
                                                          double* __restrict__ scal, double factor, long long corr_n,
                                                          float min_value, float target)
{
    __shared__ double sh[16];
    partial += (long long)blockIdx.x * count;
    scal += 2 * blockIdx.x;
    double a0 = 0.0, a1 = 0.0, a2 = 0.0, a3 = 0.0;
    long long i = threadIdx.x;
    for (; i + 3 * 1024 < count; i += 4 * 1024) {
        a0 += partial[i];
        a1 += partial[i + 1024];
        a2 += partial[i + 2 * 1024];
        a3 += partial[i + 3 * 1024];
    }
    for (; i < count; i += 1024) a0 += partial[i];
    double acc = (a0 + a1) + (a2 + a3);
#pragma unroll
    for (int off = 32; off > 0; off >>= 1) acc += __shfl_down(acc, off, 64);
    if ((threadIdx.x & 63) == 0) sh[threadIdx.x >> 6] = acc;
    __syncthreads();
    if (threadIdx.x == 0) {
        double t = 0.0;
        for (int w = 0; w < 16; ++w) t += sh[w];
        const double sum = t * factor;
        scal[0] = sum;
        if (corr_n > 0) scal[1] = (double)(target - min_value) / (sum / (double)corr_n);
    }
}

struct LenEntry {
    int len, nrad, rad[5];
    int nl;
    int nlx;
};

static constexpr LenEntry kLens[] = {
#define X(L, ...) {L, (int)(sizeof((int[]){__VA_ARGS__}) / sizeof(int)), {__VA_ARGS__}, Cfg<L>::NL, CfgX<L>::NL},
    MVSIM_FFT_SIZES(X)
#undef X
};

static const LenEntry* pick_len(int64_t need)
{
    const LenEntry* e = std::lower_bound(std::begin(kLens), std::end(kLens), need, [](const LenEntry& x, int64_t v) { return x.len < v; });
    return e == std::end(kLens) ? nullptr : e;
}
static const LenEntry* find_len(int L)
{
    const LenEntry* e = pick_len(L);
    return e && e->len == L ? e : nullptr;
}

static int lines_per_tile(int L) { const LenEntry* e = find_len(L); return e ? e->nl : 16; }
}

bool custom_fft_sizes(const int64_t dim[3], const int64_t kdim[3], int64_t P[3], const Options& opt)
{
    if (opt.rocfft) return false;
    for (int d = 0; d < 3; ++d) {
        const int64_t need = dim[d] + kdim[d] - 1;
        const fft::LenEntry* e = fft::pick_len(d == 0 ? (need + 1) / 2 : need);
        if (!e) return false;
        P[d] = d == 0 ? 2 * (int64_t)e->len : e->len;
    }
    return true;
}

bool conv_plan(const int64_t dim[3], const int64_t kdim[3], const Options& opt, ConvPlan* pl)
{
    using namespace fft;
    if (!custom_fft_sizes(dim, kdim, pl->P, opt)) return false;
    for (int d = 0; d < 3; ++d) { pl->n[d] = (int)dim[d]; pl->k[d] = (int)kdim[d]; }
    pl->px = (int)pl->P[0]; pl->py = (int)pl->P[1]; pl->pz = (int)pl->P[2]; pl->M = pl->px / 2;
    pl->tile_y = lines_per_tile(pl->py); pl->tile_z = lines_per_tile(pl->pz);
    const int ny = pl->n[1], ky = pl->k[1], kz = pl->k[2];
    pl->zdirect = opt.zpass == 2 ? false : kz <= 64;
    pl->ymirror = pl->zdirect && ny > 1 && ky / 2 < ny && ky - 1 - ky / 2 < ny;
    pl->early = pl->zdirect && opt.early_sum;
    pl->zinline_auto = opt.zpass == 0 && kz >= MVSIM_ZINLINE_MIN_KZ && pl->pz >= 512 && pl->tile_z == 16;
    const int tw_max = std::max(pl->tile_y, pl->zdirect ? NLZ : pl->tile_z);
    pl->hxp = (pl->M + 1 + tw_max - 1) / tw_max * tw_max;
    pl->pyb = (pl->py + ZB - 1) / ZB * ZB;
    pl->e_rows = find_len(pl->M)->nlx;
    return true;
}

int ensure_twiddles(mvsim_ctx* ctx, int L, int kind, const float2** out)
{
    const int key = L * 2 + kind;
    auto it = ctx->twiddles.find(key);
    if (it != ctx->twiddles.end()) { *out = reinterpret_cast<const float2*>(it->second); return MVSIM_OK; }
    std::vector<float2> h((size_t)L + 1, make_float2(0.f, 0.f));
    if (kind == 1) {
        for (int k = 0; k <= L; ++k) {
            const double a = -2.0 * M_PI * (double)k / (double)L;
            h[k] = make_float2((float)std::cos(a), (float)std::sin(a));
        }
    } else {
        const fft::LenEntry* pd = fft::find_len(L);
        if (!pd) { set_error("custom FFT: no plan for length %d", L); return MVSIM_EINVAL; }
        int P = 1, off = 0;
        for (int i = 0; i < pd->nrad; ++i) {
            const int R = pd->rad[i];
            if (P > 1) {
                for (int r = 1; r < R; ++r)
                    for (int k = 0; k < P; ++k) {
                        const double a = -2.0 * M_PI * (double)r * (double)k / ((double)P * (double)R);
                        h[(size_t)off + (size_t)(r - 1) * P + k] = make_float2((float)std::cos(a), (float)std::sin(a));
                    }
                off += (R - 1) * P;
            }
            P *= R;
        }
    }
    void* d = nullptr;
    MVSIM_HIP(hipMalloc(&d, h.size() * sizeof(float2)));
    hipError_t e = hipMemcpy(d, h.data(), h.size() * sizeof(float2), hipMemcpyHostToDevice);
    if (e != hipSuccess) { (void)hipFree(d); set_error("twiddle upload failed: %s", hipGetErrorString(e)); return MVSIM_EHIP; }
    ctx->twiddles[key] = d;
    *out = reinterpret_cast<const float2*>(d);
    return MVSIM_OK;
}

static int ensure_box_weights(mvsim_ctx* ctx, int N, int P, int len, bool half, const double2** out)
{
    char key[64];
    snprintf(key, sizeof(key), "%d/%d/%d/%d", N, P, len, half ? 1 : 0);
    auto it = ctx->box_weights.find(key);
    if (it != ctx->box_weights.end()) { *out = reinterpret_cast<const double2*>(it->second); return MVSIM_OK; }
    std::vector<double> ct((size_t)P), st((size_t)P);
    for (int j = 0; j < P; ++j) {
        const double a = 2.0 * M_PI * (double)j / (double)P;
        ct[j] = std::cos(a); st[j] = std::sin(a);
    }
    std::vector<double2> h((size_t)len, make_double2(0.0, 0.0));
    for (int k = 0; k < len; ++k) {
        if (half && k > P / 2) break;
        if (!half && k >= P) break;
        long double re = 0.0L, im = 0.0L;
        for (int n = 0; n < N; ++n) {
            const int j = (int)(((long long)k * n) % P);
            re += ct[j]; im += st[j];
        }
        const double c = half ? ((k == 0 || 2 * k == P) ? 1.0 : 2.0) : 1.0;
        h[k] = make_double2(c * (double)re, c * (double)im);
    }
    void* d = nullptr;
    MVSIM_HIP(hipMalloc(&d, h.size() * sizeof(double2)));
    hipError_t e = hipMemcpy(d, h.data(), h.size() * sizeof(double2), hipMemcpyHostToDevice);
    if (e != hipSuccess) { (void)hipFree(d); set_error("weight upload failed: %s", hipGetErrorString(e)); return MVSIM_EHIP; }
    ctx->box_weights[key] = d;
    *out = reinterpret_cast<const double2*>(d);
    return MVSIM_OK;
}

static bool fused_tail_of(const ConvPlan& pl, int inc, bool con_wanted, ExtractPlan* fp)
{
    if (!pl.early || (pl.n[0] & 3) != 0) return false;
    const int64_t dim[3] = {pl.n[0], pl.n[1], pl.n[2]};
    const long long nk = con_wanted ? pl.n[2] : (pl.n[2] - 1) / inc + 1;
    const long long rows = pl.n[1] * nk;
    if (rows * pl.n[0] >= (1ll << 32)) return false;
    *fp = ExtractPlan{};
    fp->geom = ExtractGeom::compact(dim, inc);
    fp->kernel = EXTRACT_FUSED_TAIL; fp->share = 16;
    fp->blocks = (int)((rows + pl.e_rows - 1) / pl.e_rows);
    fp->segcap = fp->full_items = (unsigned int)(pl.e_rows * pl.n[0]);
    fp->layout = QueueLayout(fp->blocks, fp->segcap, false);
    return true;
}

bool fused_tail_geometry(const int64_t dim[3], const int64_t kdim[3], int inc, bool con_wanted, const Options& opt, ExtractPlan* fp)
{
    ConvPlan pl;
    return conv_plan(dim, kdim, opt, &pl) && fused_tail_of(pl, inc, con_wanted, fp);
}

size_t fused_tail_queue_bytes(const int64_t dim[3], const int64_t kdim[3], int inc, bool con_wanted, const Options& opt)
{
    ExtractPlan fp{};
    return fused_tail_geometry(dim, kdim, inc, con_wanted, opt, &fp) ? fp.layout.total_bytes : 0;
}

void custom_fft_release(mvsim_ctx* ctx)
{
    for (auto& kv : ctx->twiddles) (void)hipFree(kv.second);
    ctx->twiddles.clear();
    for (auto& kv : ctx->box_weights) (void)hipFree(kv.second);
    ctx->box_weights.clear();
    ctx->partials_z.release();
    ctx->cfft_f.release();
    ctx->cfft_g.release();
    ctx->cfft_g1.release();
    ctx->cfft_g2.release();
}

bool custom_fft_geometry(const int64_t dim[3], const int64_t kdim[3], int64_t g[5], const Options& opt)
{
    ConvPlan pl;
    if (!conv_plan(dim, kdim, opt, &pl)) return false;
    g[0] = pl.px; g[1] = pl.py; g[2] = pl.zdirect ? pl.n[2] : pl.pz; g[3] = pl.hxp; g[4] = pl.zdirect ? 1 : 0;
    return true;
}

bool custom_zpass_geometry(const int64_t dim[3], const int64_t kdim[3], int inc, int64_t g[4], const Options& o)
{
    using namespace fft;
    ConvPlan pl;
    if (inc < 1 || !conv_plan(dim, kdim, o, &pl) || !pl.zdirect) return false;
    const int nz = pl.n[2], kz = pl.k[2];
    const int zstride = (pl.early && inc > 1) ? inc : 1;
    int frows = 0;
    size_t lds = 0;
    const int zs_chunk = (zstride > 1 && o.zconv_strided && o.zpass != 3) ? zconv_strided_chunk(nz, kz, zstride, (o.exp & 2) != 0, &frows, &lds) : 0;
    if (zs_chunk == 0 && (o.zpass == 3 || pl.zinline_auto)) return false;
    const int zc = zs_chunk > 0 ? zs_chunk : zconv_chunk(nz, kz);
    g[0] = zs_chunk > 0 ? zstride : 0; g[1] = zc; g[2] = (nz + zc - 1) / zc; g[3] = pl.hxp / NLZ;
    return true;
}

bool custom_fft_batchable(const mvsim_ctx* ctx, const int64_t dim[3], const int64_t kdim[3])
{
    const Options& o = ctx->opt;
    ConvPlan pl;
    return conv_plan(dim, kdim, o, &pl) && pl.early && !o.fuse_tail && o.zpass != 3 && !pl.zinline_auto && pl.ymirror;
}

int rotate_attenuate_fftx(mvsim_ctx* ctx, const float* gt, float* rot_or_null, float* att_or_null, const int64_t dim[3],
                          const int64_t kdim[3], const Affine& inv, double delta, bool* done, const int** plane_nz, int z_first, int nzl,
                          const unsigned int** row_bits)
{
    using namespace fft;
    *done = false;
    if (plane_nz) *plane_nz = nullptr;
    if (row_bits) *row_bits = nullptr;
    if (ctx->opt.fused_fftx == 0) return MVSIM_OK;
    if (!affine_is_x_rotation(inv)) return MVSIM_OK;
    ConvPlan pl;
    if (!conv_plan(dim, kdim, ctx->opt, &pl)) return MVSIM_OK;
    const int nx = pl.n[0], ny = pl.n[1], nz = pl.n[2], kx = pl.k[0];
    if (nzl < 0) { z_first = 0; nzl = nz; }
    if (z_first < 0 || nzl < 1 || z_first + nzl > nz) return MVSIM_OK;
    if (!pl.ymirror || nx > 1024 || nx < 64 || kx > nx || nx > ny) return MVSIM_OK;
    const int px = pl.px, py = pl.py, M = pl.M, hxp = pl.hxp;
    if (!rot_fftx_len_ok(M)) return MVSIM_OK;
    if (ctx->opt.fused_fftx == 2 && (int64_t)nx * nzl < 131072) return MVSIM_OK;
    const size_t cbytes = pl.spectrum_bytes(nzl, 0, 0, 1);
    MVSIM_TRY(ctx->cfft_f.reserve(cbytes));
    MVSIM_TRY(ctx->cfft_g.reserve(cbytes));
    const float2 *tw_m, *tw_px;
    MVSIM_TRY(ensure_twiddles(ctx, M, 0, &tw_m));
    MVSIM_TRY(ensure_twiddles(ctx, px, 1, &tw_px));
    RotFftArgs a{};
    a.in = gt; a.rot_out = rot_or_null; a.att_out = att_or_null; a.dst = ctx->cfft_f.as<float2>();
    a.twg = tw_m; a.twx = tw_px;
    a.nx = nx; a.ny = ny; a.nz = nz; a.steps = nx;
    a.z_first = z_first; a.nzl = nzl;
    a.hxp = hxp; a.py = py;
    a.halo_r = kx / 2; a.halo_l = kx - 1 - kx / 2;
    a.a = inv; a.delta = delta;
    bool want_flags = plane_nz && ctx->opt.skip_empty && nzl == nz;
    if (want_flags) {
        if (!ctx->empty_hint) {
            MVSIM_HIP(hipHostMalloc(reinterpret_cast<void**>(&ctx->empty_hint), 4 * sizeof(int), hipHostMallocDefault));
            ctx->empty_hint[0] = -1; ctx->empty_hint[1] = -1; ctx->empty_hint[2] = 0; ctx->empty_hint[3] = 0;
        }
        const int hint = *reinterpret_cast<volatile int*>(ctx->empty_hint);
        if (hint == 0 && ctx->views_since_flags < 15) { want_flags = false; ctx->views_since_flags += 1; }
        else ctx->views_since_flags = 0;
    }
    if (want_flags) {
        const bool want_rows = row_bits && ctx->opt.skip_rows && pl.zdirect && row_bits_len_ok(py) && !(py % 2 == 0 && lines_split_exists(py / 2));
        const size_t flag_bytes = ((size_t)(3 * nz + 1024) * sizeof(int) + 255) & ~(size_t)255;
        MVSIM_TRY(ctx->plane_flags.reserve(flag_bytes + (want_rows ? row_bits_bytes(py, nz) : 0)));
        a.plane_nz = ctx->plane_flags.as<int>();
        *plane_nz = a.plane_nz;
        if (want_rows) {
            a.rowbits = reinterpret_cast<unsigned int*>(ctx->plane_flags.as<char>() + flag_bytes);
            a.ky = pl.k[1];
            *row_bits = a.rowbits;
        }
    }
    MVSIM_TRY(launch_rot_fftx(ctx, M, a, rot_or_null != nullptr || att_or_null != nullptr, ctx->opt.fused_fftx >= 2));
    *done = true;
    return MVSIM_OK;
}

namespace fft {
struct ConvRun {
    const ConvPlan& pl;
    SlabRange slab;
    bool is_slab;
    long long plane;
    int V, zstride;
    int nzp;
    int nk;
    int zs_chunk, zs_frows;
    size_t zs_lds;
    bool zinline;
    long long corr_n;
    float corr_min, corr_target;
    const float2 *tw_m, *tw_px, *tw_py, *tw_pz;
    float2 *F, *G, *G1, *G2;
    double* scal;
    const int *pnz, *pnz_dil;
    const unsigned int* pnz_bits;
    const unsigned int* rowbits;
};

static int psf_passes(mvsim_ctx* ctx, const ConvRun& r, const float* psf)
{
    const ConvPlan& pl = r.pl;
    const int kx = pl.k[0], ky = pl.k[1], kz = pl.k[2], hxp = pl.hxp, V = r.V;
    SrcMap m{};
    m.x = DimMap{kx, pl.px, kx - kx / 2, kx / 2, 1, kx / 2};
    m.y = DimMap{ky, ky, ky, 0, 1, 0};
    m.z = DimMap{kz * V, kz * V, kz * V, 0, 1, 0};
    MVSIM_TRY(launch_r2c(ctx, pl.M, psf, m, r.G1, r.tw_m, r.tw_px, hxp, (long long)ky * kz * V));
    LinesArgs a{};
    a.src = r.G1; a.dst = r.G2; a.spec = nullptr; a.tw = r.tw_py;
    a.src_es = hxp; a.src_outer = (long long)hxp * ky;
    a.dst_es = hxp; a.dst_outer = r.plane;
    if (pl.zdirect) { a.dst_outer = (long long)ZB * hxp; a.dst_blk = (long long)kz * V * ZB * hxp; }
    a.lmap = DimMap{ky, pl.py, ky - ky / 2, ky / 2, 1, ky / 2};
    MVSIM_TRY(launch_lines(ctx, pl.py, FWD, true, a, hxp / pl.tile_y, kz * V));
    if (pl.zdirect) return MVSIM_OK;
    LinesArgs c{};
    c.src = r.G2; c.dst = r.G; c.spec = nullptr; c.tw = r.tw_pz;
    c.src_es = r.plane; c.src_outer = hxp;
    c.dst_es = r.plane; c.dst_outer = hxp;
    c.lmap = DimMap{kz, pl.pz, kz - kz / 2, kz / 2, 1, kz / 2};
    c.dst_tile_major = 1;
    return launch_lines(ctx, pl.pz, FWD, true, c, hxp / pl.tile_z, pl.py);
}

static int psf_spectrum(mvsim_ctx* ctx, const ConvRun& r, const float* psf, PsfCache::Entry* entry, bool flags_follow)
{
    hipStream_t s = ctx->stream;
    const bool hit = entry && entry->filled;
    const bool side = ctx->opt.psf_overlap && (int64_t)r.pl.n[0] * r.pl.n[1] * r.pl.n[2] >= (int64_t)1 << 24 && (!hit || flags_follow);
    ctx->psf_on_side = side;
    if (side) {
        if (!ctx->side_stream) {
            MVSIM_HIP(hipStreamCreateWithFlags(&ctx->side_stream, hipStreamNonBlocking));
            MVSIM_HIP(hipEventCreateWithFlags(&ctx->ev_fork, hipEventDisableTiming));
            MVSIM_HIP(hipEventCreateWithFlags(&ctx->ev_join, hipEventDisableTiming));
        }
        MVSIM_HIP(hipEventRecord(ctx->ev_fork, s));
        MVSIM_HIP(hipStreamWaitEvent(ctx->side_stream, ctx->ev_fork, 0));
        if (hit) return MVSIM_OK;
        ctx->stream = ctx->side_stream;
    }
    if (hit) return MVSIM_OK;
    ev_begin(ctx, ST_PSF);
    const int rc = psf_passes(ctx, r, psf);
    ev_end(ctx, ST_PSF);
    if (entry && rc == MVSIM_OK) entry->filled = true;
    if (side) {
        ctx->stream = s;
        MVSIM_HIP(hipEventRecord(ctx->ev_join, ctx->side_stream));
    }
    return rc;
}

static int pass_a(mvsim_ctx* ctx, const ConvRun& r, const float* img)
{
    const ConvPlan& pl = r.pl;
    const int planes = r.slab.nz_in * r.V;
    SrcMap m{};
    DimMap* dm[3] = {&m.x, &m.y, &m.z};
    for (int d = 0; d < 3; ++d) *dm[d] = DimMap{pl.n[d], (int)pl.P[d], pl.n[d] + pl.k[d] / 2, pl.k[d] - 1 - pl.k[d] / 2, 0, 0};
    if (pl.zdirect) m.z = DimMap{planes, planes, planes, 0, 0, 0};
    if (pl.ymirror) { m.y = DimMap{pl.n[1], pl.py, pl.n[1], 0, 0, 0}; m.enum_y = pl.n[1]; }
    const long long rows = pl.zdirect ? (long long)(pl.ymirror ? pl.n[1] : pl.py) * planes : (long long)pl.py * pl.pz;
    ev_begin(ctx, ST_PASS_A);
    MVSIM_TRY(launch_r2c(ctx, pl.M, img, m, r.F, r.tw_m, r.tw_px, pl.hxp, rows));
    ev_end(ctx, ST_PASS_A);
    return MVSIM_OK;
}

static int plane_flags_setup(mvsim_ctx* ctx, ConvRun& r, const int* pnz)
{
    const int nz = r.pl.n[2], kz = r.pl.k[2];
    int* base = ctx->plane_flags.as<int>();
    const int nwords = (nz + 2 * NZ_EXT + 64 + 31) / 32 + ZNIT + 2;
    const bool side = ctx->psf_on_side;
    hipLaunchKernelGGL(k_plane_flags_finish, dim3(1), dim3(1024), 0, side ? ctx->side_stream : ctx->stream, pnz, nz, kz, kz / 2,
                       reinterpret_cast<unsigned int*>(base + 2 * nz), nwords, base + nz, ctx->empty_hint);
    MVSIM_HIP(hipGetLastError());
    if (side) MVSIM_HIP(hipEventRecord(ctx->ev_join, ctx->side_stream));
    r.pnz = pnz;
    r.pnz_dil = base + nz;
    r.pnz_bits = reinterpret_cast<const unsigned int*>(base + 2 * nz);
    return MVSIM_OK;
}

static int pass_b(mvsim_ctx* ctx, const ConvRun& r)
{
    const ConvPlan& pl = r.pl;
    const int hxp = pl.hxp, ny = pl.n[1], ky = pl.k[1], kz = pl.k[2];
    LinesArgs b{};
    b.src = r.F; b.dst = r.F; b.tw = r.tw_py; b.src_es = b.dst_es = hxp; b.src_outer = b.dst_outer = r.plane;
    b.lmap = DimMap{0, 0, 0, 0, 1, 0};
    if (pl.ymirror) { b.lmap = DimMap{ny, pl.py, ny + ky / 2, ky - 1 - ky / 2, 0, 0}; b.src_mirror = 1; }
    b.gap_lo = ny + ky / 2; b.gap_hi = pl.py - (ky - 1 - ky / 2);
    if (pl.zdirect) {
        b.outer_skip_lo = 1 << 30;
        b.dst = r.G; b.dst_outer = (long long)ZB * hxp; b.dst_blk = (long long)r.slab.nz_in * r.V * ZB * hxp;
    } else {
        b.outer_skip_lo = pl.n[2] + kz / 2;
        b.outer_skip_len = std::max(0, pl.pz - (kz - 1 - kz / 2) - b.outer_skip_lo);
    }
    if (r.pnz) { b.nzflags = r.pnz; b.nz_stride = 1; }
    if (r.rowbits) { b.rowbits = r.rowbits; b.rowbits_stride = row_bits_words(pl.py); }
    ev_begin(ctx, ST_PASS_B);
    MVSIM_TRY(launch_lines(ctx, pl.py, FWD, false, b, hxp / pl.tile_y, pl.zdirect ? r.slab.nz_in * r.V : pl.pz - b.outer_skip_len));
    ev_end(ctx, ST_PASS_B);
    return MVSIM_OK;
}

static int zpass_inline(mvsim_ctx* ctx, const ConvRun& r)
{
    const ConvPlan& pl = r.pl;
    const int nz = pl.n[2], kz = pl.k[2], pz = pl.pz, hxp = pl.hxp;
    LinesArgs c{};
    c.src = r.G; c.dst = r.F; c.tw = r.tw_pz;
    c.src_es = c.dst_es = (long long)ZB * hxp; c.src_outer = c.dst_outer = hxp;
    c.src_oblk = (long long)r.slab.nz_in * ZB * hxp; c.dst_oblk = (long long)r.slab.nz_out * ZB * hxp;
    c.lmap = DimMap{nz, pz, nz + kz / 2, kz - 1 - kz / 2, 0, 0};
    c.src_mirror = 1;
    c.gap_lo = nz + kz / 2; c.gap_hi = pz - (kz - 1 - kz / 2);
    c.outer_skip_lo = 1 << 30;
    c.store_limit = nz;
    c.taps = r.G2; c.taps_es = (long long)ZB * hxp; c.taps_outer = hxp; c.taps_oblk = (long long)kz * ZB * hxp;
    c.pmap = DimMap{kz, pz, kz - kz / 2, kz / 2, 1, kz / 2};
    const float scale_f = (float)(0.25 / ((double)pl.px * (double)pl.py * (double)pz));
    const long long zblocks = (long long)(hxp / pl.tile_z) * pl.py;
    if (pl.early) {
        MVSIM_TRY(ensure_box_weights(ctx, pl.n[0], pl.px, hxp, true, &c.wx));
        MVSIM_TRY(ensure_box_weights(ctx, pl.n[1], pl.py, pl.py, false, &c.wy));
        MVSIM_TRY(ctx->partials_z.reserve((size_t)zblocks * sizeof(double)));
        c.sum_partial = ctx->partials_z.as<double>();
    }
    MVSIM_TRY(launch_lines(ctx, pz, CONVZ, false, c, hxp / pl.tile_z, pl.py));
    if (pl.early) {
        hipLaunchKernelGGL(k_reduce_partials, dim3(1), dim3(1024), 0, ctx->stream, c.sum_partial, zblocks, r.scal, (double)scale_f,
                           r.corr_n, r.corr_min, r.corr_target);
        MVSIM_HIP(hipGetLastError());
    }
    return MVSIM_OK;
}

static int zpass_direct(mvsim_ctx* ctx, const ConvRun& r)
{
    const ConvPlan& pl = r.pl;
    const int kz = pl.k[2], hxp = pl.hxp, V = r.V;
    ZConvArgs z{};
    z.src = r.G; z.dst = r.F; z.taps = r.G2; z.hxp = hxp; z.nz = r.slab.nz_out; z.kz = kz; z.c = kz / 2;
    z.zs = (long long)ZB * hxp; z.src_blk = (long long)r.slab.nz_in * V * ZB * hxp; z.dst_blk = (long long)r.nzp * V * ZB * hxp;
    z.taps_blk = (long long)kz * V * ZB * hxp;
    z.src_view = (long long)r.slab.nz_in * z.zs; z.dst_view = (long long)r.nzp * z.zs; z.taps_view = (long long)kz * z.zs;
    z.nz_global = pl.n[2]; z.z_in0 = r.slab.z_in0; z.z_out0 = r.slab.z_out0;
    z.zc = r.zs_chunk > 0 ? r.zs_chunk : zconv_chunk(r.slab.nz_out, kz);
    z.stride = r.zs_chunk > 0 ? r.zstride : 1; z.frows = r.zs_frows;
    z.nzbits = r.pnz_bits;
    const float scale_f = (float)(0.25 / ((double)pl.px * (double)pl.py));
    long long zblocks = 0;
    if (pl.early) {
        MVSIM_TRY(ensure_box_weights(ctx, pl.n[0], pl.px, hxp, true, &z.wx));
        MVSIM_TRY(ensure_box_weights(ctx, pl.n[1], pl.py, pl.py, false, &z.wy));
        zblocks = zconv_blocks(z, pl.py);
        MVSIM_TRY(ctx->partials_z.reserve((size_t)zblocks * V * sizeof(double)));
        z.sum_partial = ctx->partials_z.as<double>();
    }
    if (r.zs_chunk > 0) MVSIM_TRY(launch_zconv_strided(ctx, z, pl.py, r.zs_lds, V));
    else MVSIM_TRY(launch_zconv(ctx, z, pl.py, V));
    if (pl.early) {
        hipLaunchKernelGGL(k_reduce_partials, dim3(V), dim3(1024), 0, ctx->stream, z.sum_partial, zblocks, r.scal, (double)scale_f,
                           r.corr_n, r.corr_min, r.corr_target);
        MVSIM_HIP(hipGetLastError());
    }
    return MVSIM_OK;
}

static int zpass_fft(mvsim_ctx* ctx, const ConvRun& r)
{
    const ConvPlan& pl = r.pl;
    const int nz = pl.n[2], kz = pl.k[2], hxp = pl.hxp;
    LinesArgs c{};
    c.src = r.F; c.dst = r.F; c.spec = r.G; c.tw = r.tw_pz;
    c.src_es = c.dst_es = c.spec_es = r.plane; c.src_outer = c.dst_outer = c.spec_outer = hxp;
    c.lmap = DimMap{0, 0, 0, 0, 1, 0};
    c.gap_lo = nz + kz / 2; c.gap_hi = pl.pz - (kz - 1 - kz / 2);
    c.outer_skip_lo = 1 << 30;
    c.store_limit = nz;
    return launch_lines(ctx, pl.pz, CONV, false, c, hxp / pl.tile_z, pl.py);
}

static int pass_d(mvsim_ctx* ctx, const ConvRun& r, float2* dst)
{
    const ConvPlan& pl = r.pl;
    const int hxp = pl.hxp;
    LinesArgs d{};
    d.src = r.F; d.dst = dst; d.tw = r.tw_py; d.src_es = d.dst_es = hxp;
    d.src_outer = d.dst_outer = r.plane * r.zstride;
    if (pl.zdirect) { d.src_outer = (long long)ZB * hxp * r.zstride; d.src_blk = (long long)r.nzp * r.V * ZB * hxp; }
    d.lmap = DimMap{0, 0, 0, 0, 1, 0};
    d.outer_skip_lo = 1 << 30;
    d.store_limit = pl.n[1];
    if (r.pnz) { d.nzflags = r.pnz_dil; d.nz_stride = r.zstride; }
    ev_begin(ctx, ST_PASS_D);
    MVSIM_TRY(launch_lines(ctx, pl.py, INV, false, d, hxp / pl.tile_y, r.nk));
    ev_end(ctx, ST_PASS_D);
    return MVSIM_OK;
}

static int fused_tail_args(mvsim_ctx* ctx, const ConvRun& r, const ConvTail& tail, const ExtractPlan& fp, C2RFuse* fz)
{
    if (!tail.corr_done) {
        ev_begin(ctx, ST_ADJUST);
        MVSIM_TRY(launch_adjust_corr(ctx->stream, r.scal, (int64_t)r.pl.n[0] * r.pl.n[1] * r.pl.n[2], tail.min_value, tail.target_average));
        ev_end(ctx, ST_ADJUST);
    }
    fz->scal = r.scal; fz->min_value = tail.min_value; fz->con = tail.con_adj; fz->acq = tail.acq;
    fz->acq_every = tail.con_adj ? tail.inc : 1; fz->idx_zstride = r.zstride; fz->noise = tail.noise ? 1 : 0;
    fz->mul = tail.mul; fz->k0 = (uint32_t)tail.seed; fz->k1 = (uint32_t)(tail.seed >> 32); fz->stream = tail.stream;
    if (tail.noise) {
        if (ctx->pqueue.bytes < fp.layout.total_bytes) {
            set_error("fused tail: queue workspace not reserved");
            return MVSIM_EINVAL;
        }
        const QueueLayout::Region q = fp.layout.region(ctx->pqueue.p);
        fz->qcount = q.counts; fz->queue = reinterpret_cast<PItem*>(q.items);
        fz->segcap = fp.segcap;
    }
    return MVSIM_OK;
}
}

int custom_fft_convolve(mvsim_ctx* ctx, const float* img, const int64_t dim[3], const float* psf,
                        const int64_t kdim[3], float* out, ConvTail* tail)
{
    const SlabRange whole{0, (int)dim[2], 0, (int)dim[2]};
    return custom_fft_convolve_slab(ctx, img, dim, psf, kdim, whole, out, tail);
}

int custom_fft_convolve_slab(mvsim_ctx* ctx, const float* img, const int64_t dim[3], const float* psf,
                             const int64_t kdim[3], const SlabRange& slab, float* out, ConvTail* tail)
{
    using namespace fft;
    ConvPlan pl;
    if (!conv_plan(dim, kdim, ctx->opt, &pl)) { set_error("custom FFT: no hand-written size for this volume / PSF"); return MVSIM_EINVAL; }
    const Options& o = ctx->opt;
    const int kz = pl.k[2];
    ConvRun r{pl, slab};
    r.plane = (long long)pl.hxp * pl.py;
    r.is_slab = slab.nz_in != pl.n[2] || slab.nz_out != pl.n[2];
    r.V = (tail && tail->views > 1) ? tail->views : 1;
    r.zstride = (tail && pl.early && tail->zstride > 1 && (!r.is_slab || slab.z_out0 % tail->zstride == 0)) ? tail->zstride : 1;
    ExtractPlan fp{};
    const bool fuse = tail && tail->want_fuse && !r.is_slab && tail->acq &&
                      fused_tail_of(pl, tail->inc, tail->con_adj != nullptr, &fp) &&
                      ((reinterpret_cast<uintptr_t>(tail->acq) | reinterpret_cast<uintptr_t>(tail->con_adj)) & 15) == 0;
    if (fuse) r.zstride = tail->con_adj ? 1 : tail->inc;
    if (tail) { tail->zstride = r.zstride; tail->fused = fuse; tail->fused_blocks = fp.blocks; tail->fused_segcap = fp.segcap; }
    r.corr_n = (tail && tail->corr_n > 0 && !r.is_slab) ? tail->corr_n : 0;
    r.corr_min = tail ? tail->min_value : 0.f; r.corr_target = tail ? tail->target_average : 1.f;
    if (tail) tail->corr_done = r.corr_n > 0;
    const bool x_done = tail && tail->x_done;
    if (r.is_slab && !pl.zdirect) {
        set_error("z-slab tiling needs the direct z pass (PSF depth %d > 64 or option fft_zpass=fft)", kz);
        return MVSIM_EINVAL;
    }
    if (r.V > 1 && (r.is_slab || !pl.early || fuse || x_done || tail->plane_nz)) {
        set_error("stacked views need the direct z pass with the early sum on whole views");
        return MVSIM_EINVAL;
    }
    const int nkv = (r.slab.nz_out - 1) / r.zstride + 1;
    r.nzp = r.V > 1 ? nkv * r.zstride : r.slab.nz_out;
    r.nk = nkv * r.V;
    const size_t cbytes = pl.spectrum_bytes(r.slab.nz_in, r.slab.nz_out, r.nzp, r.V);
    const long long rows_out_early = (long long)pl.n[1] * r.slab.nz_out * r.V;
    if (x_done && cbytes > ctx->cfft_f.bytes) {
        set_error("custom FFT: the spectrum needs %zu bytes, the fused x transform left it in %zu", cbytes, ctx->cfft_f.bytes);
        return MVSIM_EINVAL;
    }
    if (!x_done) MVSIM_TRY(ctx->cfft_f.reserve(cbytes));
    MVSIM_TRY(ctx->cfft_g.reserve(cbytes));
    r.zs_chunk = (pl.zdirect && r.zstride > 1 && o.zconv_strided && o.zpass != 3)
                     ? zconv_strided_chunk(slab.nz_out, kz, r.zstride, (o.exp & 2) != 0, &r.zs_frows, &r.zs_lds) : 0;
    r.zinline = pl.zdirect && !r.is_slab && r.zs_chunk == 0 && r.V == 1 && (o.zpass == 3 || pl.zinline_auto);
    const size_t g2_bytes = (size_t)r.V * pl.hxp * pl.pyb * kz * sizeof(float2);
    PsfCache::Entry* pe = ctx->psf_entry;
    ctx->psf_entry = nullptr;
    if (pe && !(r.V == 1 && !r.is_slab && pl.zdirect && !r.zinline && psf == pe->psf && pe->g2_bytes == g2_bytes)) pe = nullptr;
    if (!(pe && pe->filled)) MVSIM_TRY(ctx->cfft_g1.reserve((size_t)r.V * pl.hxp * pl.k[1] * kz * sizeof(float2)));
    if (!pe) MVSIM_TRY(ctx->cfft_g2.reserve(g2_bytes));
    MVSIM_TRY(ctx->partials.reserve(PARTIALS_BYTES));
    MVSIM_TRY(ctx->partials_e.reserve((size_t)((rows_out_early + 3) / 4 + 16) * sizeof(double)));
    r.scal = scal_of(ctx);
    MVSIM_TRY(ensure_twiddles(ctx, pl.M, 0, &r.tw_m));
    MVSIM_TRY(ensure_twiddles(ctx, pl.px, 1, &r.tw_px));
    MVSIM_TRY(ensure_twiddles(ctx, pl.py, 0, &r.tw_py));
    if (!pl.zdirect || r.zinline) MVSIM_TRY(ensure_twiddles(ctx, pl.pz, 0, &r.tw_pz));
    r.F = ctx->cfft_f.as<float2>(); r.G = ctx->cfft_g.as<float2>();
    r.G1 = ctx->cfft_g1.as<float2>(); r.G2 = pe ? static_cast<float2*>(pe->g2) : ctx->cfft_g2.as<float2>();
    hipStream_t s = ctx->stream;

    const bool flags_follow = x_done && tail->plane_nz && !r.zinline && !r.is_slab && !fuse;
    MVSIM_TRY(psf_spectrum(ctx, r, psf, pe, flags_follow));

    ev_begin(ctx, ST_CONVOLVE);
    if (x_done) {
        if (!pl.ymirror || r.V != 1) { set_error("x_done without the geometry of the fused x transform"); return MVSIM_EINVAL; }
        if (tail->row_bits) {
            if (r.is_slab || !pl.zdirect) { set_error("row bits on a view pass B cannot read them for"); return MVSIM_EINVAL; }
            r.rowbits = tail->row_bits;
        }
    } else {
        MVSIM_TRY(pass_a(ctx, r, img));
    }
    if (flags_follow) MVSIM_TRY(plane_flags_setup(ctx, r, tail->plane_nz));
    MVSIM_TRY(pass_b(ctx, r));
    if (ctx->psf_on_side) MVSIM_HIP(hipStreamWaitEvent(s, ctx->ev_join, 0));
    ev_begin(ctx, ST_PASS_C);
    if (r.zinline) MVSIM_TRY(zpass_inline(ctx, r));
    else if (pl.zdirect) MVSIM_TRY(zpass_direct(ctx, r));
    else MVSIM_TRY(zpass_fft(ctx, r));
    ev_end(ctx, ST_PASS_C);
    float2* Fz = pl.zdirect ? r.G : r.F;
    MVSIM_TRY(pass_d(ctx, r, Fz));
    C2RFuse fz{};
    if (fuse) MVSIM_TRY(fused_tail_args(ctx, r, *tail, fp, &fz));
    ev_begin(ctx, ST_PASS_E);
    const float scale = (float)(0.25 / ((double)pl.px * (double)pl.py * ((pl.zdirect && !r.zinline) ? 1.0 : (double)pl.pz)));
    int nblk = 0;
    const bool sparse = tail_sparse_ok(tail && tail->want_sparse, r.pnz_dil != nullptr, fuse) && r.V == 1 && !r.is_slab;
    if (tail) { tail->sparse = sparse; tail->sparse_flags = sparse ? r.pnz_dil : nullptr; tail->sparse_stride = sparse ? r.zstride : 0; }
    MVSIM_TRY(launch_c2r(ctx, pl.M, Fz, out, r.tw_m, r.tw_px, pl.hxp, pl.py * r.zstride, pl.n[0], pl.n[1], (long long)pl.n[1] * r.nk, scale,
                         pl.early ? nullptr : ctx->partials_e.as<double>(), &nblk, fuse ? &fz : nullptr,
                         C2REmpty{r.pnz_dil, r.zstride, sparse ? 1 : 0}));
    if (fuse && nblk != fp.blocks) { set_error("fused tail: block count mismatch"); return MVSIM_EINVAL; }
    if (!pl.early) hipLaunchKernelGGL(k_reduce_partials, dim3(1), dim3(1024), 0, s, ctx->partials_e.as<double>(), (long long)nblk, r.scal, 1.0,
                                      r.corr_n, r.corr_min, r.corr_target);
    MVSIM_HIP(hipGetLastError());
    ev_end(ctx, ST_PASS_E);
    if (fuse && tail->noise) {
        ev_end(ctx, ST_CONVOLVE);
        ev_begin(ctx, ST_EXTRACT);
        ExtractOps ops;
        ops.out = tail->acq; ops.queue_ws = ctx->pqueue.p; ops.mul = tail->mul; ops.seed = tail->seed; ops.stream = tail->stream;
        MVSIM_TRY(launch_resolve(s, fp, ops));
        ev_end(ctx, ST_EXTRACT);
        return MVSIM_OK;
    }
    ev_end(ctx, ST_CONVOLVE);
    return MVSIM_OK;
}

}
```

multiview-simulation_amd/csrc/fft_host.h:

```cpp
#pragma once
#include "fft_dev.h"

namespace mvsim {
struct PItem;
namespace fft {

enum Mode { FWD = 0, INV = 1, CONV = 2, CONVZ = 3 };

struct LinesArgs {
    const float2* src;
    float2*       dst;
    const float2* spec;
    const float2* tw;
    long long     src_es, src_outer, dst_es, dst_outer, spec_es, spec_outer;
    DimMap        lmap;
    int           gap_lo, gap_hi;
    int           outer_skip_lo, outer_skip_len;
    int           store_limit;
    int           dst_tile_major;
    long long     src_blk, dst_blk;
    int           src_mirror;
    const int*    nzflags;
    int           nz_stride;
    long long     src_oblk, dst_oblk;
    const float2* taps;
    long long     taps_es, taps_oblk, taps_outer;
    DimMap        pmap;
    const double2* wx;
    const double2* wy;
    double*       sum_partial;
    int           pair_tiles;
    const unsigned int* rowbits;
    int           rowbits_stride;
};

#ifndef MVSIM_ZBS
#define MVSIM_ZBS 4
#endif
constexpr int ZBS = MVSIM_ZBS, ZB = 1 << ZBS;
constexpr int NZ_EXT = 96;

__device__ __forceinline__ int mirror_index(int i, int n)
{
    if (n == 1) return 0;
    const int p = 2 * n - 2;
    i %= p;
    if (i < 0) i += p;
    return i < n ? i : p - i;
}

__device__ __forceinline__ float4 keep4(float4 t, bool keep)
{
    const unsigned int m = keep ? 0xFFFFFFFFu : 0u;
    return make_float4(__uint_as_float(__float_as_uint(t.x) & m), __uint_as_float(__float_as_uint(t.y) & m),
                       __uint_as_float(__float_as_uint(t.z) & m), __uint_as_float(__float_as_uint(t.w) & m));
}

__device__ __forceinline__ long long line_off(int n, long long es, long long blk)
{
    return blk ? (long long)(n >> ZBS) * blk + (long long)(n & (ZB - 1)) * es : (long long)n * es;
}

struct C2RFuse {
    const double* scal;
    float         min_value;
    float*        con;
    float*        acq;
    int           acq_every;
    int           idx_zstride;
    int           noise;
    double        mul;
    uint32_t      k0, k1, stream;
    PItem*        queue;
    unsigned int* qcount;
    unsigned int  segcap;
};

struct C2REmpty {
    const int* flags;
    int        stride;
    int        sparse;
};

#ifndef MVSIM_EXP_NLZ
#define MVSIM_EXP_NLZ 16
#endif
#ifndef MVSIM_ZNIT
#define MVSIM_ZNIT 9
#endif
constexpr int NLZ = MVSIM_EXP_NLZ, ZU = 16, ZJ = 8, ZT = 256;
constexpr int ZRPI = ZT / (NLZ / 2);
constexpr int ZNIT = MVSIM_ZNIT;

struct ZConvArgs {
    const float2* src;
    float2*       dst;
    const float2* taps;
    long long     src_blk, dst_blk, taps_blk, zs;
    int           hxp, nz, kz, c, zc;
    int           nz_global, z_in0, z_out0;
    const double2* wx;
    const double2* wy;
    double*       sum_partial;
    const unsigned int* nzbits;
    int           stride, frows;
    int           nch, nkxb, py, plain_order;
    long long     src_view, dst_view, taps_view;
};

template <class K> static int set_lds(mvsim_ctx* ctx, K kernel, size_t bytes)
{
    return ensure_lds_attr(ctx, reinterpret_cast<const void*>(kernel), bytes);
}

int  launch_lines(mvsim_ctx* ctx, int L, int mode, bool sparse, const LinesArgs& a, int tiles, int nouter);
bool lines_split_exists(int LH);
int  launch_r2c(mvsim_ctx* ctx, int M, const float* src, const SrcMap& map, float2* dst, const float2* tw, const float2* twx, int hxp,
                long long rows);
int  launch_c2r(mvsim_ctx* ctx, int M, const float2* srcc, float* out, const float2* tw, const float2* twx, int hxp, int py, int nx, int ny,
                long long rows, float scale, double* partial, int* nblocks, const C2RFuse* fuse, const C2REmpty& em);
int       zconv_chunk(int nz, int kz);
long long zconv_blocks(const ZConvArgs& a, int py, int cols = 0);
int       zconv_strided_chunk(int nz, int kz, int s, bool force, int* frows_out, size_t* lds_out);
int       launch_zconv(mvsim_ctx* ctx, const ZConvArgs& args, int py, int views = 1);
int       launch_zconv_strided(mvsim_ctx* ctx, const ZConvArgs& args, int py, size_t lds, int views = 1);

}

int ensure_twiddles(mvsim_ctx* ctx, int L, int kind, const float2** out);

}
```

multiview-simulation_amd/csrc/fft_passes.hip:

```cpp
#include "fft_host.h"
#include "poisson_dev.h"

namespace mvsim {
namespace fft {

#if defined(MVSIM_DEV_ATTRIBUTION) && defined(MVSIM_EXP_LINES_STAMPS)
constexpr int STAMP_BLOCKS = 1 << 20;
__device__ unsigned long long g_line_stamps[2][STAMP_BLOCKS][8];
#define MVSIM_STAMP(k)                                                                                                       \
    do {                                                                                                                     \
        if (!SPARSE && (MODE == FWD || MODE == INV) && threadIdx.x == 0) {                                                   \
            const unsigned long long sb_ = (unsigned long long)blockIdx.y * gridDim.x + blockIdx.x;                          \
            if (sb_ < (unsigned long long)STAMP_BLOCKS) g_line_stamps[MODE == INV][sb_][k] = __builtin_amdgcn_s_memtime();   \
        }                                                                                                                    \
    } while (0)
#else
#define MVSIM_STAMP(k) do { } while (0)
#endif

#ifndef MVSIM_ROWBITS_MASKED
#define MVSIM_ROWBITS_MASKED 0
#endif

__device__ __forceinline__ long long outer_off(int by, long long outer, long long oblk)
{
    return oblk ? (long long)(by >> ZBS) * oblk + (long long)(by & (ZB - 1)) * outer : (long long)by * outer;
}

template <int L> constexpr int lines_blocks_per_cu() { return 2 * Cfg<L>::LDS <= 160 * 1024 ? 2 : 1; }
template <class PLAN, int MODE, bool SPARSE>
__global__ __launch_bounds__(Cfg<PLAN::len>::T, (lines_blocks_per_cu<PLAN::len>() * Cfg<PLAN::len>::T + 255) / 256)
void k_fft_lines(LinesArgs p)
{
    constexpr int L = PLAN::len;
    using C = Cfg<L>;
    constexpr int NL = C::NL, LP = C::LP, T = C::T, LW = C::LW, NW = C::NW;
    constexpr int LPR = NL / 2;
    constexpr int ROWS = T / LPR;
    constexpr int NIT = (L + ROWS - 1) / ROWS;
    extern __shared__ __align__(16) float2 lds[];
    float2* buf = lds;
    float2* tw = lds + NL * LP;
    const int tid = threadIdx.x, lane = tid & 63, wave = tid >> 6;
    const int c2 = (tid % LPR) * 2;
    const int r0 = tid / LPR;
    float2* wbuf = buf + wave * LW * LP;
    int tile_x = (int)blockIdx.x, tile_o = (int)blockIdx.y;
    if constexpr (NL * sizeof(float2) < 128) {
        const unsigned nt = gridDim.x, total = nt * gridDim.y, b = blockIdx.y * nt + blockIdx.x;
        if ((nt & 1u) == 0 && b < (total & ~15u) && p.pair_tiles) {
            const unsigned xcd = b & 7u, slot = b >> 3;
            const unsigned lin = ((((slot >> 1) << 3) + xcd) << 1) | (slot & 1u);
            tile_x = (int)(lin % nt); tile_o = (int)(lin / nt);
        }
    }
    MVSIM_STAMP(0);
    const int by = tile_o >= p.outer_skip_lo ? tile_o + p.outer_skip_len : tile_o;
    constexpr bool ROWBITS = MODE == FWD && !SPARSE && row_bits_len_ok(L);
    constexpr int RB_WPI = ROWS >= 32 ? ROWS / 32 : 1;
    constexpr int RB_N = (ROWBITS && ROWS >= 32) ? NIT * RB_WPI : 1;
    unsigned int rb[RB_N];
    const unsigned int* rec = nullptr;
    if constexpr (ROWBITS) {
        const int* const nzf = p.nzflags;
        const unsigned int* const rbp = p.rowbits;
        if (rbp) {
            rec = rbp + (long long)by * p.rowbits_stride;
            const int flag = *(nzf ? nzf + by * p.nz_stride : reinterpret_cast<const int*>(rbp));
            if constexpr (ROWS >= 32) {
#pragma unroll
                for (int i = 0; i < RB_N; ++i) rb[i] = i < row_bits_words(L) ? rec[i] : 0u;
            }
            if (nzf && flag == 0) return;
        } else if (nzf) {
            if (nzf[by * p.nz_stride] == 0) return;
        }
    } else if (p.nzflags) {
        if (p.nzflags[by * p.nz_stride] == 0) return;
    }
    const float2* sbase = p.src + outer_off(by, p.src_outer, p.src_oblk) + (long long)tile_x * NL + c2;
    float4 vp[MODE == CONVZ ? NIT : 1];
    if (MODE == CONVZ) {
        const float2* tbase = p.taps + outer_off(by, p.taps_outer, p.taps_oblk) + (long long)tile_x * NL + c2;
#pragma unroll
        for (int it = 0; it < NIT; ++it) {
            const int n = r0 + it * ROWS;
            vp[it] = make_float4(0.f, 0.f, 0.f, 0.f);
            if ((L % ROWS == 0) || n < L) {
                const int t = map_src(p.pmap, n);
                if (t >= 0) vp[it] = *reinterpret_cast<const float4*>(tbase + (long long)t * p.taps_es);
            }
        }
    }
    float4 v[NIT];
    bool under_bits = false;
    if constexpr (ROWBITS) {
        if (rec) {
            under_bits = true;
#pragma unroll
            for (int it = 0; it < NIT; ++it) {
                const int n = r0 + it * ROWS;
                bool keep;
                if constexpr (ROWS >= 32) {
                    unsigned int w = rb[it * RB_WPI];
                    if constexpr (RB_WPI > 1) {
                        const int sel = __builtin_amdgcn_readfirstlane(r0 >> 5);
#pragma unroll
                        for (int k = 1; k < RB_WPI; ++k) w = sel == k ? rb[it * RB_WPI + k] : w;
                    }
                    keep = (w >> (r0 & 31)) & 1u;
                } else {
                    keep = n < L && ((rec[n >> 5] >> (n & 31)) & 1u);
                }
                const int sn = keep ? (p.src_mirror ? map_src(p.lmap, n) : n) : 0;
#if MVSIM_ROWBITS_MASKED
                v[it] = keep4(*reinterpret_cast<const float4*>(sbase + line_off(sn, p.src_es, p.src_blk)), keep);
#else
                v[it] = make_float4(0.f, 0.f, 0.f, 0.f);
                if (keep) v[it] = *reinterpret_cast<const float4*>(sbase + line_off(sn, p.src_es, p.src_blk));
#endif
            }
        }
    }
    if (!under_bits) {
#pragma unroll
    for (int it = 0; it < NIT; ++it) {
        const int n = r0 + it * ROWS;
        v[it] = make_float4(0.f, 0.f, 0.f, 0.f);
        if ((L % ROWS == 0) || n < L) {
            if (SPARSE) {
                const int sn = map_src(p.lmap, n);
                if (sn >= 0) v[it] = *reinterpret_cast<const float4*>(sbase + sn * p.src_es);
            } else if (n < p.gap_lo || n >= p.gap_hi) {
                const int sn = p.src_mirror ? map_src(p.lmap, n) : n;
                v[it] = *reinterpret_cast<const float4*>(sbase + line_off(sn, p.src_es, p.src_blk));
            }
        }
    }
    }
    MVSIM_STAMP(1);
    for (int i = tid; i < L; i += T) tw[i] = p.tw[i];
    MVSIM_STAMP(2);
    constexpr int R1 = PLAN::R1, IT1 = (LW * (L / R1) + 63) / 64;
    float2 ps[MODE == CONVZ ? IT1 : 1][MODE == CONVZ ? R1 : 1];
    if constexpr (MODE == CONVZ) {
#pragma unroll
        for (int it = 0; it < NIT; ++it) {
            const int n = r0 + it * ROWS;
            if ((L % ROWS == 0) || n < L) {
                buf[c2 * LP + n] = make_float2(vp[it].x, vp[it].y);
                buf[(c2 + 1) * LP + n] = make_float2(vp[it].z, vp[it].w);
            }
        }
        __syncthreads();
        PLAN::template run<LW>(wbuf, tw, lane);
        PLAN::template capture_first_pass<LW, IT1>(wbuf, lane, ps);
        __syncthreads();
    }
#pragma unroll
    for (int it = 0; it < NIT; ++it) {
        const int n = r0 + it * ROWS;
        if ((L % ROWS == 0) || n < L) {
            float2 a = make_float2(v[it].x, v[it].y), b = make_float2(v[it].z, v[it].w);
            if (MODE == INV) { a = cconj(a); b = cconj(b); }
            buf[c2 * LP + n] = a;
            buf[(c2 + 1) * LP + n] = b;
        }
    }
    __syncthreads();
    MVSIM_STAMP(3);
    PLAN::template run<LW>(wbuf, tw, lane);
    MVSIM_STAMP(4);
    if (MODE == CONV) {
        const float2* gl = p.spec + (((long long)tile_o * gridDim.x + tile_x) * NL + (long long)wave * LW) * L;
        PLAN::template run_op<LW>(wbuf, tw, lane, LoadMulConj{gl, L});
    }
    if constexpr (MODE == CONVZ) PLAN::template run_op<LW>(wbuf, tw, lane, LoadMulConjReg<IT1, R1>{ps});
    if (MODE == FWD && p.dst_tile_major) {
        float2* gl = p.dst + (((long long)tile_o * gridDim.x + tile_x) * NL + (long long)wave * LW) * L;
#pragma unroll
        for (int j = 0; j < LW; ++j)
            for (int n2 = lane * 2; n2 < L; n2 += 128) {
                const float2 a = wbuf[j * LP + n2], b = wbuf[j * LP + n2 + 1];
                *reinterpret_cast<float4*>(gl + j * L + n2) = make_float4(a.x, a.y, b.x, b.y);
            }
        return;
    }
    __syncthreads();
    MVSIM_STAMP(5);
    float2* dbase = p.dst + outer_off(by, p.dst_outer, p.dst_oblk) + (long long)tile_x * NL + c2;
    const int nstore = p.store_limit > 0 ? p.store_limit : L;
    float2 sa = make_float2(0.f, 0.f), sb = make_float2(0.f, 0.f);
#pragma unroll
    for (int it = 0; it < NIT; ++it) {
        const int n = r0 + it * ROWS;
        if (((L % ROWS == 0) || n < L) && n < nstore) {
            float2 a = buf[c2 * LP + n], b = buf[(c2 + 1) * LP + n];
            if (MODE != FWD) { a = cconj(a); b = cconj(b); }
            *reinterpret_cast<float4*>(dbase + line_off(n, p.dst_es, p.dst_blk)) = make_float4(a.x, a.y, b.x, b.y);
            if (MODE == CONVZ) { sa = cadd(sa, a); sb = cadd(sb, b); }
        }
    }
    MVSIM_STAMP(6);
    if constexpr (MODE == CONVZ) {
        if (p.sum_partial) {
            __syncthreads();
            float2* red = buf;
            red[r0 * NL + c2] = sa;
            red[r0 * NL + c2 + 1] = sb;
            __syncthreads();
            double t = 0.0;
            if (tid < NL) {
                double sre = 0.0, sim = 0.0;
                for (int r = 0; r < ROWS; ++r) { const float2 q = red[r * NL + tid]; sre += (double)q.x; sim += (double)q.y; }
                const double2 a = p.wx[tile_x * NL + tid], b = p.wy[by];
                const double wr = a.x * b.x - a.y * b.y, wi = a.x * b.y + a.y * b.x;
                t = sre * wr - sim * wi;
            }
            if (wave == 0) {
#pragma unroll
                for (int off = 32; off > 0; off >>= 1) t += __shfl_down(t, off, 64);
                if (lane == 0) p.sum_partial[(long long)tile_o * gridDim.x + tile_x] = t;
            }
        }
    }
}

template <class PLANH, int MODE>
__global__ __launch_bounds__(Cfg<PLANH::len>::T, (2 * Cfg<PLANH::len>::T + 255) / 256)
void k_fft_lines_split(LinesArgs p, const float2* __restrict__ tw2)
{
    static_assert(MODE == FWD || MODE == INV, "the image's y passes");
    constexpr int LH = PLANH::len;
    using C = Cfg<LH>;
    constexpr int NL = C::NL, LP = C::LP, T = C::T, LW = C::LW;
    static_assert(2 * C::LDS <= 160 * 1024, "tiles of the half length, two per CU");
    constexpr int LPR = NL / 2;
    constexpr int ROWS = T / LPR;
    constexpr int NIT = (LH + ROWS - 1) / ROWS;
    extern __shared__ __align__(16) float2 lds[];
    float2* buf = lds;
    float2* tw = lds + NL * LP;
    const int tid = threadIdx.x, lane = tid & 63, wave = tid >> 6;
    const int c2 = (tid % LPR) * 2;
    const int r0 = tid / LPR;
    float2* wbuf = buf + wave * LW * LP;
    int tile_x = (int)blockIdx.x, tile_o = (int)blockIdx.y;
    if constexpr (NL * sizeof(float2) < 128) {
        const unsigned nt = gridDim.x, total = nt * gridDim.y, b = blockIdx.y * nt + blockIdx.x;
        if ((nt & 1u) == 0 && b < (total & ~15u) && p.pair_tiles) {
            const unsigned xcd = b & 7u, slot = b >> 3;
            const unsigned lin = ((((slot >> 1) << 3) + xcd) << 1) | (slot & 1u);
            tile_x = (int)(lin % nt); tile_o = (int)(lin / nt);
        }
    }
    const int by = tile_o >= p.outer_skip_lo ? tile_o + p.outer_skip_len : tile_o;
    if (p.nzflags) {
        if (p.nzflags[by * p.nz_stride] == 0) return;
    }
    const float2* sbase = p.src + outer_off(by, p.src_outer, p.src_oblk) + (long long)tile_x * NL + c2;
    const int mir_n = p.src_mirror ? p.lmap.n : (1 << 30), mir_a = p.src_mirror ? p.lmap.a : (1 << 30), mir_P = p.lmap.P, mir_b = p.lmap.b;
    auto row = [&](int pos) -> float4 {
        if (pos >= p.gap_lo && pos < p.gap_hi) return make_float4(0.f, 0.f, 0.f, 0.f);
        int sn = pos;
        if (pos >= mir_a) {
            if (pos < mir_P - mir_b) return make_float4(0.f, 0.f, 0.f, 0.f);
            sn = pos - mir_P;
// ... 62 lines not shown
{
    hipStream_t s = ctx->stream;
    using C = Cfg<PLAN::len>;
    dim3 grid(tiles, nouter), block(C::T);
#define MVSIM_LL(MODE_, SP_)                                                                 \
    do {                                                                                     \
        MVSIM_TRY(set_lds(ctx, k_fft_lines<PLAN, MODE_, SP_>, C::LDS));                           \
        hipLaunchKernelGGL((k_fft_lines<PLAN, MODE_, SP_>), grid, block, C::LDS, s, a);      \
    } while (0)
    if (mode == FWD && sparse) MVSIM_LL(FWD, true);
    else if (mode == FWD) MVSIM_LL(FWD, false);
    else if (mode == INV) MVSIM_LL(INV, false);
    else if (mode == CONVZ) MVSIM_LL(CONVZ, false);
    else MVSIM_LL(CONV, false);
#undef MVSIM_LL
    MVSIM_HIP(hipGetLastError());
    return MVSIM_OK;
}
template <int LH> constexpr bool split_half_ok()
{
    return Cfg<LH>::NL == 8 && Cfg<LH>::T == 512 && 2 * Cfg<LH>::LDS <= 160 * 1024 && 2 * Cfg<2 * LH>::LDS > 160 * 1024;
}

template <int LH, int... Rs>
static int launch_lines_split_t(mvsim_ctx* ctx, int mode, const LinesArgs& a, const float2* tw2, int tiles, int nouter)
{
    using PLANH = Plan<LH, Rs...>;
    using C = Cfg<LH>;
    constexpr int WIDE = C::NL / Cfg<2 * LH>::NL;
    if (tiles % WIDE) { set_error("custom FFT: %d tiles of 8 columns do not pair up", tiles); return MVSIM_EINVAL; }
    dim3 grid(tiles / WIDE, nouter), block(C::T);
    if (mode == FWD) {
        MVSIM_TRY(set_lds(ctx, k_fft_lines_split<PLANH, FWD>, C::LDS));
        hipLaunchKernelGGL((k_fft_lines_split<PLANH, FWD>), grid, block, C::LDS, ctx->stream, a, tw2);
    } else {
        MVSIM_TRY(set_lds(ctx, k_fft_lines_split<PLANH, INV>, C::LDS));
        hipLaunchKernelGGL((k_fft_lines_split<PLANH, INV>), grid, block, C::LDS, ctx->stream, a, tw2);
    }
    MVSIM_HIP(hipGetLastError());
    return MVSIM_OK;
}

using LinesFn = int (*)(mvsim_ctx*, int mode, bool sparse, const LinesArgs&, int tiles, int nouter);
using LinesSplitFn = int (*)(mvsim_ctx*, int mode, const LinesArgs&, const float2* tw2, int tiles, int nouter);

template <int LH, int... Rs> constexpr LinesSplitFn lines_split_of()
{
    if constexpr (LH >= 1024 && LH <= 1120 && split_half_ok<LH>()) return &launch_lines_split_t<LH, Rs...>;
    else return nullptr;
}

static LinesFn lines_fn(int L)
{
    switch (L) {
#define X(L_, ...) case L_: return &launch_lines_t<Plan<L_, __VA_ARGS__>>;
    MVSIM_FFT_SIZES(X)
#undef X
    default: return nullptr;
    }
}

static LinesSplitFn lines_split_fn(int LH)
{
    switch (LH) {
#define X(L_, ...) case L_: return lines_split_of<L_, __VA_ARGS__>();
    MVSIM_FFT_SIZES(X)
#undef X
    default: return nullptr;
    }
}

bool lines_split_exists(int LH) { return lines_split_fn(LH) != nullptr; }

int launch_lines(mvsim_ctx* s, int L, int mode, bool sparse, const LinesArgs& a0, int tiles, int nouter)
{
    const LinesFn lines = lines_fn(L);
    if (!lines) { set_error("custom FFT: unsupported length %d", L); return MVSIM_EINVAL; }
    LinesArgs a = a0;
    a.pair_tiles = (s->opt.exp & 4) ? 0 : 1;
    if (a.rowbits && (mode != FWD || sparse || !row_bits_len_ok(L) || a.rowbits_stride != row_bits_words(L))) {
        set_error("custom FFT: row bits on a pass that does not read them (length %d, mode %d)", L, mode);
        return MVSIM_EINVAL;
    }
    const LinesSplitFn split = (L % 2 || a.rowbits) ? nullptr : lines_split_fn(L / 2);
    if ((mode == FWD || mode == INV) && !sparse && !a.dst_tile_major && !(s->opt.exp & 8) && split && tiles % 2 == 0 &&
        (!a.src_mirror || (a.lmap.mode == 0 && a.lmap.b < a.lmap.n && a.lmap.a - a.lmap.n < a.lmap.n))) {
        const float2* tw2 = nullptr;
        MVSIM_TRY(ensure_twiddles(s, L / 2, 0, &a.tw));
        MVSIM_TRY(ensure_twiddles(s, L, 1, &tw2));
        return split(s, mode, a, tw2, tiles, nouter);
    }
    return lines(s, mode, sparse, a, tiles, nouter);
}

template <class PLAN>
__global__ __launch_bounds__(CfgX<PLAN::len>::T) void k_fft_x_r2c(const float* __restrict__ src, SrcMap map,
                                                                 float2* __restrict__ dst,
                                                                 const float2* __restrict__ twg,
                                                                 const float2* __restrict__ twx, int hxp,
                                                                 long long rows)
{
    constexpr int M = PLAN::len;
    using C = CfgX<M>;
    constexpr int NR = C::NL, LP = C::LP, T = C::T, LW = C::LW;
    constexpr int PAIRS = (M + 1) / 2;
    extern __shared__ __align__(16) float2 lds[];
    float2* tw = lds + NR * LP;
    const int tid = threadIdx.x, lane = tid & 63, wave = tid >> 6;
    float2* wbuf = lds + wave * LW * LP;
    const long long row0 = (long long)blockIdx.x * NR + wave * LW;

    const int nxs = map.x.n;
    const bool fast_x = (nxs & 3) == 0 && map.x.mode == 0;
    long long offs[LW], drows[LW];
#pragma unroll
    for (int j = 0; j < LW; ++j) {
        const long long row = row0 + j;
        offs[j] = -1;
        drows[j] = row;
        if (row < rows) {
            const unsigned py = (unsigned)(map.enum_y ? map.enum_y : map.y.P);
            const unsigned urow = (unsigned)row;
            const int z = (int)(urow / py), y = (int)(urow - (unsigned)z * py);
            const int sy = map_src(map.y, y), sz = map_src(map.z, z);
            if (sy >= 0 && sz >= 0) offs[j] = (long long)nxs * (sy + (long long)map.y.n * sz);
            drows[j] = (long long)z * map.y.P + y;
        }
    }
    bool any_row = false;
#pragma unroll
    for (int j = 0; j < LW; ++j) any_row |= offs[j] >= 0;
    if (!any_row && map.x.mode == 0) {
        for (int i = tid; i < M; i += T) tw[i] = twg[i];
        __syncthreads();
        return;
    }
    constexpr int LITEMS = LW * PAIRS;
    constexpr int LIT = (LITEMS + 63) / 64;
    float4 v[LIT];
#pragma unroll
    for (int it = 0; it < LIT; ++it) {
        const int e = lane + it * 64;
        const int j = e / PAIRS, q = e - j * PAIRS;
        long long off = -1;
#pragma unroll
        for (int jj = 0; jj < LW; ++jj) off = (j == jj) ? offs[jj] : off;
        float4 t = make_float4(0.f, 0.f, 0.f, 0.f);
        if (off >= 0 && e < LITEMS) {
            const float* __restrict__ srow = src + off;
            if (fast_x && 4 * q + 3 < nxs) {
                t = *reinterpret_cast<const float4*>(srow + 4 * q);
            } else {
                const int s0 = map_src(map.x, 4 * q), s1 = map_src(map.x, 4 * q + 1);
                const int s2 = map_src(map.x, 4 * q + 2), s3 = map_src(map.x, 4 * q + 3);
                t.x = s0 >= 0 ? srow[s0] : 0.f;
                t.y = s1 >= 0 ? srow[s1] : 0.f;
                t.z = s2 >= 0 ? srow[s2] : 0.f;
                t.w = s3 >= 0 ? srow[s3] : 0.f;
            }
        }
        v[it] = t;
    }
    for (int i = tid; i < M; i += T) tw[i] = twg[i];
#pragma unroll
    for (int it = 0; it < LIT; ++it) {
        const int e = lane + it * 64;
        if (e < LITEMS) {
            const int j = e / PAIRS, q = e - j * PAIRS;
// ... 356 lines not shown
```

multiview-simulation_amd/csrc/psf_cache.h:

```cpp
#pragma once

#include <cstddef>
#include <cstdint>
#include <cstring>
#include <list>
#include <vector>

namespace mvsim {

struct PsfKey {
    int64_t kdim[3];
    int32_t px, py, pyb, hxp;
    int32_t zdirect, tile_y;
    int32_t views, reserved;
};
static_assert(sizeof(PsfKey) == 3 * 8 + 8 * 4, "PsfKey must not have padding");

inline uint64_t psf_hash64(const void* data, size_t bytes, uint64_t seed)
{
    const unsigned char* p = static_cast<const unsigned char*>(data);
    const uint64_t m = 0x9E3779B97F4A7C15ull;
    uint64_t h[4] = {seed ^ 0x243F6A8885A308D3ull, seed ^ 0x13198A2E03707344ull, seed ^ 0xA4093822299F31D0ull, seed ^ 0x082EFA98EC4E6C89ull};
    size_t i = 0;
    for (; i + 32 <= bytes; i += 32) {
        uint64_t w[4];
        std::memcpy(w, p + i, 32);
        for (int k = 0; k < 4; ++k) { h[k] = (h[k] ^ w[k]) * m; h[k] ^= h[k] >> 29; }
    }
    uint64_t r = (uint64_t)bytes * m;
    for (; i < bytes; ++i) r = (r ^ p[i]) * 0x100000001B3ull;
    for (int k = 0; k < 4; ++k) { r = (r ^ h[k]) * m; r ^= r >> 32; }
    return r;
}

class PsfCache {
public:
    typedef void* (*DevAlloc)(size_t bytes);
    typedef void (*DevFree)(void* p);
    typedef uint64_t (*Hash)(const void* data, size_t bytes, uint64_t seed);

    struct Entry {
        uint64_t hash = 0;
        PsfKey key{};
        std::vector<float> taps;
        void* g2 = nullptr;
        void* psf = nullptr;
        size_t g2_bytes = 0, psf_bytes = 0;
        bool filled = false;
    };
    struct Stats { int64_t hits = 0, misses = 0, evictions = 0, bytes = 0; };

    PsfCache() = default;
    PsfCache(const PsfCache&) = delete;
    PsfCache& operator=(const PsfCache&) = delete;
    ~PsfCache() { clear(); }

    void configure(DevAlloc a, DevFree f, Hash h = psf_hash64) { alloc_ = a; free_ = f; hash_ = h; }
    const Stats& stats() const { return stats_; }
    size_t entries() const { return lru_.size(); }

    Entry* find(const PsfKey& key, const float* taps, size_t n)
    {
        const uint64_t h = hash_of(key, taps, n);
        for (auto it = lru_.begin(); it != lru_.end(); ++it) {
            if (it->hash != h || std::memcmp(&it->key, &key, sizeof(PsfKey)) != 0 || it->taps.size() != n) continue;
            if (std::memcmp(it->taps.data(), taps, n * sizeof(float)) != 0) continue;
            lru_.splice(lru_.begin(), lru_, it);
            stats_.hits += 1;
            return &lru_.front();
        }
        return nullptr;
    }

    Entry* insert(const PsfKey& key, const float* taps, size_t n, size_t g2_bytes, size_t cap_bytes)
    {
        stats_.misses += 1;
        const size_t psf_bytes = n * sizeof(float), need = g2_bytes + psf_bytes;
        if (!alloc_ || !free_ || need > cap_bytes) return nullptr;
        void *g2 = nullptr, *psf = nullptr;
        while (!lru_.empty() && (size_t)stats_.bytes + need > cap_bytes) {
            Entry& v = lru_.back();
            if (!g2 && v.g2_bytes == g2_bytes && v.psf_bytes == psf_bytes) { g2 = v.g2; psf = v.psf; v.g2 = v.psf = nullptr; }
            drop_back();
            stats_.evictions += 1;
        }
        if (!g2) {
            g2 = alloc_(g2_bytes);
            psf = g2 ? alloc_(psf_bytes) : nullptr;
            if (!g2 || !psf) { if (g2) free_(g2); return nullptr; }
        }
        lru_.emplace_front();
        Entry& e = lru_.front();
        e.hash = hash_of(key, taps, n);
        e.key = key;
        e.taps.assign(taps, taps + n);
        e.g2 = g2; e.psf = psf; e.g2_bytes = g2_bytes; e.psf_bytes = psf_bytes;
        stats_.bytes += (int64_t)need;
        return &e;
    }

    void discard(Entry* e)
    {
        for (auto it = lru_.begin(); it != lru_.end(); ++it)
            if (&*it == e) { lru_.splice(lru_.end(), lru_, it); drop_back(); return; }
    }

    void clear()
    {
        while (!lru_.empty()) drop_back();
    }

private:
    uint64_t hash_of(const PsfKey& key, const float* taps, size_t n) const
    {
        return hash_(taps, n * sizeof(float), hash_(&key, sizeof(PsfKey), 0));
    }
    void drop_back()
    {
        Entry& v = lru_.back();
        if (v.g2) free_(v.g2);
        if (v.psf) free_(v.psf);
        stats_.bytes -= (int64_t)(v.g2_bytes + v.psf_bytes);
        lru_.pop_back();
    }

    std::list<Entry> lru_;
    Stats stats_;
    DevAlloc alloc_ = nullptr;
    DevFree free_ = nullptr;
    Hash hash_ = psf_hash64;
};
// ... 3 lines not shown
```

multiview-simulation_amd/csrc/zconv.hip:

```cpp
#include "fft_host.h"

#include <algorithm>

namespace mvsim {
namespace fft {
constexpr int ZPITCH = NLZ + 1;
constexpr int ZLPR = NLZ / 2;
#ifndef MVSIM_ZBLK
#define MVSIM_ZBLK 3
#endif
#ifndef MVSIM_ZLDS
#define MVSIM_ZLDS (44 * 1024)
#endif
constexpr int ZBLOCKS_PER_CU = MVSIM_ZBLK;
constexpr size_t ZLDS_TARGET = MVSIM_ZLDS;
__host__ __device__ constexpr size_t zconv_frows(int zc, int kz, int kzp)
{
    return (((size_t)(kzp - kz + zc + kz - 1) * ZPITCH) + 1) & ~(size_t)1;
}

__device__ __forceinline__ void zconv_view(ZConvArgs& p)
{
    const long long v = blockIdx.y;
    p.src += v * p.src_view;
    p.dst += v * p.dst_view;
    p.taps += v * p.taps_view;
    if (p.sum_partial) p.sum_partial += v * ((long long)p.nch * p.nkxb * p.py);
}

__device__ __forceinline__ bool zconv_tile(const ZConvArgs& p, int& chunk, int& kxb, int& ky, long long& tile)
{
    const long long total = (long long)p.nch * p.nkxb * p.py, per = (total + 7) / 8;
    const long long l = blockIdx.x;
    tile = p.plain_order ? l : (l & 7) * per + (l >> 3);
    if (tile >= total) return false;
    chunk = (int)(tile % p.nch);
    const long long col = tile / p.nch;
    kxb = (int)(col % p.nkxb);
    ky = (int)(col / p.nkxb);
    return true;
}

typedef float v2f __attribute__((ext_vector_type(2)));


constexpr int TNIT = 64 / ZRPI;

__global__ __launch_bounds__(ZT, ZBLOCKS_PER_CU) void k_zconv(ZConvArgs p)
{
    extern __shared__ __align__(16) float2 lds[];
    zconv_view(p);
    const int kzp = (p.kz + ZJ - 1) / ZJ * ZJ;
    const int padf = kzp - p.kz;
    int chunk, kxb, ky;
    long long tile;
    if (!zconv_tile(p, chunk, kxb, ky, tile)) return;
    const int zc0 = chunk * p.zc;
    const int zn = min(p.zc, p.nz - zc0);
    const int rows = padf + zn + p.kz - 1;
    float2* f = lds;
    float2* g = lds + zconv_frows(p.zc, p.kz, kzp);
    const int tid = threadIdx.x;
    const long long rowb = (long long)(ky & (ZB - 1)) * p.hxp + (long long)kxb * NLZ;
    const long long scol = (long long)(ky >> ZBS) * p.src_blk + rowb, dcol = (long long)(ky >> ZBS) * p.dst_blk + rowb;
    const long long tcol = (long long)(ky >> ZBS) * p.taps_blk + rowb;
    const int c2 = (tid % ZLPR) * 2;
    const int hl = p.kz - 1 - p.c;
    float4 v[ZNIT], tv[TNIT];
    static_assert(ZRPI == 32, "one word of plane bits per staging iteration");
    unsigned int rowbits[ZNIT];
    unsigned int zbmask = 0xFFFFFFFFu;
#pragma unroll
    for (int it = 0; it < ZNIT; ++it) rowbits[it] = 0xFFFFFFFFu;
    if (p.nzbits) {
        const int b0 = p.z_out0 + zc0 - hl + NZ_EXT - padf;
        const unsigned int* __restrict__ wp = p.nzbits + (b0 >> 5);
        const int sh = b0 & 31;
        unsigned int anyrow = 0u, missing = 0u;
#pragma unroll
        for (int it = 0; it < ZNIT; ++it) {
            const unsigned long long two = ((unsigned long long)wp[it + 1] << 32) | wp[it];
            unsigned int m = (unsigned int)(two >> sh);
            const int lo = padf - it * 32, hi = rows - it * 32;
            unsigned int valid = ~0u;
            if (lo > 0) valid &= lo >= 32 ? 0u : ~0u << lo;
// ... 333 lines not shown
{
    int zc = (nz + ZU - 1) / ZU * ZU;
    const int kzp = (kz + ZJ - 1) / ZJ * ZJ;
    while (zc > ZU && (zconv_lds(zc, kz) > ZLDS_TARGET || (kzp - kz) + zc + kz - 1 > ZNIT * ZRPI)) zc -= ZU;
    const int nchunks = (nz + zc - 1) / zc;
    const int even = ((nz + nchunks - 1) / nchunks + ZU - 1) / ZU * ZU;
    return even < zc ? even : zc;
}

long long zconv_blocks(const ZConvArgs& a, int py, int cols)
{
    return (long long)((a.nz + a.zc - 1) / a.zc) * ((cols > 0 ? cols : a.hxp) / NLZ) * py;
}

static dim3 zconv_grid(const mvsim_ctx* ctx, ZConvArgs& a, int py, int views)
{
    a.nch = (a.nz + a.zc - 1) / a.zc; a.nkxb = a.hxp / NLZ; a.py = py;
    a.plain_order = (ctx->opt.exp & 1) ? 1 : 0;
    const long long total = (long long)a.nch * a.nkxb * a.py;
    return dim3((unsigned)((total + 7) / 8 * 8), (unsigned)views);
}

int launch_zconv(mvsim_ctx* ctx, const ZConvArgs& args, int py, int views)
{
    hipStream_t s = ctx->stream;
    ZConvArgs a = args;
    const size_t lds = zconv_lds(a.zc, a.kz);
    const dim3 grid = zconv_grid(ctx, a, py, views);
    MVSIM_TRY(set_lds(ctx, k_zconv, lds));
    hipLaunchKernelGGL(k_zconv, grid, dim3(ZT), lds, s, a);
    MVSIM_HIP(hipGetLastError());
    return MVSIM_OK;
}

#ifndef MVSIM_ZLDS_S
#define MVSIM_ZLDS_S (52 * 1024)
#endif
int zconv_strided_chunk(int nz, int kz, int s, bool force, int* frows_out, size_t* lds_out)
{
    if (s < 2 || s > 4 || kz > 64) return 0;
    const int nq = (kz + s - 1) / s, qp = (nq + ZJ - 1) / ZJ * ZJ, gr = s * qp, padf = gr - kz;
    if (kz - 1 - kz / 2 + padf > NZ_EXT) return 0;
    auto geometry = [&](int zc, int* frows, size_t* lds) {
        const int nout = (zc + s - 1) / s;
        int kmax = 0;
        for (int kb = 0; kb < nout; kb += 64) {
            const int nt = std::min(64, nout - kb), zu = (nt + 3) / 4;
            kmax = std::max(kmax, kb + 3 * zu + ZU - 1);
        }
        const int staged = padf + zc + kz - 1;
        *frows = std::max(staged, padf + kz - 1 + s * kmax + 1);
        *lds = ((size_t)*frows * NLZ + (size_t)gr * NLZ + (size_t)(kz + 1 + ZT / NLZ) * NLZ) * sizeof(float2);
        return staged;
    };
    int zc = (nz + s - 1) / s * s, frows = 0;
    size_t lds = 0;
    while (zc > s && (geometry(zc, &frows, &lds) > ZNIT * ZRPI || lds > (size_t)MVSIM_ZLDS_S)) zc -= s;
    if (geometry(zc, &frows, &lds) > ZNIT * ZRPI || lds > (size_t)MVSIM_ZLDS_S) return 0;
    const int nchunks = (nz + zc - 1) / zc;
    if (!force) {
        const int zc1 = zconv_chunk(nz, kz), nch1 = (nz + zc1 - 1) / zc1;
        if (nchunks * 15.5 >= nch1 * (13.0 + 0.17 * kz)) return 0;
    }
    const int even = ((nz + nchunks - 1) / nchunks + s - 1) / s * s;
    if (even < zc) { zc = even; geometry(zc, &frows, &lds); }
    *frows_out = frows; *lds_out = lds;
    return zc;
}

int launch_zconv_strided(mvsim_ctx* ctx, const ZConvArgs& args, int py, size_t lds, int views)
{
    hipStream_t s = ctx->stream;
    ZConvArgs a = args;
    const dim3 grid = zconv_grid(ctx, a, py, views);
    switch (a.stride) {
    case 2: MVSIM_TRY(set_lds(ctx, k_zconv_strided<2>, lds)); hipLaunchKernelGGL(k_zconv_strided<2>, grid, dim3(ZT), lds, s, a); break;
    case 3: MVSIM_TRY(set_lds(ctx, k_zconv_strided<3>, lds)); hipLaunchKernelGGL(k_zconv_strided<3>, grid, dim3(ZT), lds, s, a); break;
    case 4: MVSIM_TRY(set_lds(ctx, k_zconv_strided<4>, lds)); hipLaunchKernelGGL(k_zconv_strided<4>, grid, dim3(ZT), lds, s, a); break;
    default: set_error("k_zconv_strided: stride %d", a.stride); return MVSIM_EINVAL;
    }
    MVSIM_HIP(hipGetLastError());
    return MVSIM_OK;
}
}
}
```

Before: 88300.

## Add z-lines spectrum layout with register-streaming z convolution kernel

Adds an alternative spectrum layout where each kx holds contiguous z-by-ky lines, written by the forward y pass and read back by the inverse y pass. A new wavefront-per-64-lines kernel then convolves along z with a register ring buffer and packed complex FMAs instead of the LDS-blocked zconv, and also folds in the early-sum reduction. The layout is chosen automatically when the plan allows it (single view, not a slab, no fused tail). PSF cache entries are tagged with their layout so they are refilled on a mismatch. The aim is to remove LDS staging and blocked-layout traffic in the z pass, at the cost of more complex y-pass indexing and higher register pressure.

```diff
diff --git a/include/mvsim.h b/include/mvsim.h
--- a/include/mvsim.h
+++ b/include/mvsim.h
@@ -474,6 +474,7 @@
 } mvsim_timings;
 int mvsim_fft_geometry(const int64_t dim[3], const int64_t kdim[3], int64_t geometry[5]);
 int mvsim_zpass_geometry(const int64_t dim[3], const int64_t kdim[3], int inc, int64_t out[4]);
+int mvsim_zpass_layout(const int64_t dim[3], const int64_t kdim[3], int inc, int* lines);
 int mvsim_stencil_geometry(const int64_t kdim[3], int64_t geometry[5]);
 int mvsim_extract_path(const int64_t dim[3], int inc, int index_inc, uint64_t index_offset, int aligned16, int queue_share, int64_t path[4]);
 int mvsim_get_extract_path(mvsim_ctx* ctx, int64_t path[5]);
diff --git a/multiview-simulation_amd/__init__.py b/multiview-simulation_amd/__init__.py
--- a/multiview-simulation_amd/__init__.py
+++ b/multiview-simulation_amd/__init__.py
@@ -24,7 +24,7 @@
 __all__ = ["AffineTransform3D", "BeadRegistration", "Context", "DeconParams", "DifferenceOfGaussian", "DogParams", "MatchParams", "MultiViewDeconvolution", "Group", "Hessian", "HypersphereCollectionRealRandomAccessible", "JavaRandom", "Lightsheet",
            "PerlinNoiseRealRandomAccessible", "PointRejectionSampling", "RayTracingTest", "Raytrace", "RefractiveIndexMap", "ClearingMap", "SimpleCalculatedRealRandomAccessible", "SimulateBeads",
            "SimulateBeads2", "SimulateMultiViewAberrations", "SimulateMultiViewDataset", "Tools", "VolumeInjection", "broadcast_plan", "default_context", "MvsimError", "MvsimNoDeviceError", "ViewParams", "shard_views",
-           "version", "zpass_geometry", "ViewFusion", "FuseParams", "PsfExtraction", "PsfParams"]
+           "version", "zpass_geometry", "zpass_layout", "ViewFusion", "FuseParams", "PsfExtraction", "PsfParams"]
 
 
 def broadcast_plan(nranks: int, rank: int, root: int, count: int, pieces: int = 8):
@@ -44,6 +44,12 @@
     g = (C.c_int64 * 4)()
     rc = _lib.load().mvsim_zpass_geometry((C.c_int64 * 3)(*dim_xyz), (C.c_int64 * 3)(*kdim_xyz), int(inc), g)
     return tuple(int(x) for x in g) if rc == 0 else None
+
+
+def zpass_layout(dim_xyz, kdim_xyz, inc: int = 1):
+    lines = C.c_int(0)
+    rc = _lib.load().mvsim_zpass_layout((C.c_int64 * 3)(*dim_xyz), (C.c_int64 * 3)(*kdim_xyz), int(inc), C.byref(lines))
+    return ("lines" if lines.value else "blocked") if rc == 0 else None
 
 
 class JavaRandom:
diff --git a/multiview-simulation_amd/_lib.py b/multiview-simulation_amd/_lib.py
--- a/multiview-simulation_amd/_lib.py
+++ b/multiview-simulation_amd/_lib.py
@@ -231,6 +231,7 @@
                                              C.POINTER(_vp), _i64p, C.c_int, C.POINTER(C.c_double)]),
     "mvsim_fft_geometry": (C.c_int, [_i64p, _i64p, _i64p]),
     "mvsim_zpass_geometry": (C.c_int, [_i64p, _i64p, C.c_int, _i64p]),
+    "mvsim_zpass_layout": (C.c_int, [_i64p, _i64p, C.c_int, C.POINTER(C.c_int)]),
     "mvsim_rotate_around_axis_zslabs": (C.c_int, [_vp, C.POINTER(_vp), _i64p, C.c_int, _i64p, C.c_int, C.c_int, C.POINTER(_vp), _i64p, C.c_int]),
     "mvsim_attenuate3d_zslabs": (C.c_int, [_vp, C.POINTER(_vp), _i64p, C.c_int, _i64p, C.c_double, C.POINTER(_vp), _i64p, C.c_int]),
     "mvsim_convolve_zslabs": (C.c_int, [_vp, C.POINTER(_vp), _i64p, C.c_int, _i64p, _vp, _i64p, C.c_int, C.POINTER(_vp), _i64p, C.c_int]),
diff --git a/multiview-simulation_amd/build.py b/multiview-simulation_amd/build.py
--- a/multiview-simulation_amd/build.py
+++ b/multiview-simulation_amd/build.py
@@ -9,7 +9,7 @@
 CSRC = os.path.join(HERE, "csrc")
 LIB = os.path.join(HERE, "libmvsim.so")
 SOURCES = ["api.cpp", "api_view.cpp", "api_host.cpp", "api_sims.cpp", "comm.cpp", "kernels.hip", "rotate.hip", "extract.hip", "extract_interval.hip", "fftconv.hip", "fft_driver.hip", "fft_passes.hip", "zconv.hip", "rotate_fft.hip", "stencil.hip", "phantom.hip", "beads.hip", "aberrations.hip", "raytrace.hip", "procedural.hip", "sphere_walk.hip", "api_decon.cpp", "deconvolve.hip", "api_detect.cpp", "detect.hip", "api_register.cpp", "register.hip", "api_fuse.cpp", "fuse.hip", "api_psf.cpp", "psf.hip"]
-HEADERS = ["common.h", "api_internal.h", "host_pool.h", "jrandom.h", "extract_plan.h", "interval_plan.h", "poisson_dev.h", "poisson_recipe.h", "fft_dev.h", "fft_host.h", "rotate_rounds.h", "row_bits.h", "rotate_dev.h", "sphere_walk.h", "aberr_dev.h", "bricks.h", "decon.h", "detect.h", "register.h", "register_dev.h", "fuse.h", "fuse_dev.h", "psf.h", "psf_dev.h", "psf_cache.h", "../../include/mvsim.h"]
+HEADERS = ["common.h", "api_internal.h", "host_pool.h", "jrandom.h", "extract_plan.h", "interval_plan.h", "poisson_dev.h", "poisson_recipe.h", "fft_dev.h", "fft_host.h", "zlines_geom.h", "rotate_rounds.h", "row_bits.h", "rotate_dev.h", "sphere_walk.h", "aberr_dev.h", "bricks.h", "decon.h", "detect.h", "register.h", "register_dev.h", "fuse.h", "fuse_dev.h", "psf.h", "psf_dev.h", "psf_cache.h", "../../include/mvsim.h"]
 ROCM = os.environ.get("ROCM_PATH", "/opt/rocm")
 
 
diff --git a/multiview-simulation_amd/csrc/api.cpp b/multiview-simulation_amd/csrc/api.cpp
--- a/multiview-simulation_amd/csrc/api.cpp
+++ b/multiview-simulation_amd/csrc/api.cpp
@@ -42,6 +42,7 @@
     if (n == "attenuate") return word({{"serial", 0}, {"scan", 1}}, &o.attenuate_scan);
     if (n == "early_sum") return flag(&o.early_sum);
     if (n == "zconv_strided") return flag(&o.zconv_strided);
+    if (n == "zpass_layout") return word({{"auto", 0}, {"blocked", 1}, {"lines", 2}}, &o.zpass_layout);
     if (n == "exp") return number(2, 0, 15, &o.exp);
     if (n == "beads_pair_cap") return number(10, 1024, 1LL << 31, &o.beads_pair_cap);
     if (n == "reject_batch") return number(7, 1, 1LL << 20, &o.reject_batch, 0);
@@ -1007,6 +1008,15 @@
     return MVSIM_OK;
 }
 
+int mvsim_zpass_layout(const int64_t dim[3], const int64_t kdim[3], int inc, int* lines)
+{
+    int64_t g[4];
+    if (!lines) { set_error("invalid argument: null pointer"); return MVSIM_EINVAL; }
+    MVSIM_TRY(mvsim_zpass_geometry(dim, kdim, inc, g));
+    *lines = custom_zpass_lines(dim, kdim, inc, env_options()) ? 1 : 0;
+    return MVSIM_OK;
+}
+
 int mvsim_enable_timing(mvsim_ctx* ctx, int enable)
 {
     MVSIM_TRY(set_device(ctx));
diff --git a/multiview-simulation_amd/csrc/api_view.cpp b/multiview-simulation_amd/csrc/api_view.cpp
--- a/multiview-simulation_amd/csrc/api_view.cpp
+++ b/multiview-simulation_amd/csrc/api_view.cpp
@@ -151,9 +151,9 @@
     add(&o->rot, sizeof(o->rot)); add(&o->att, sizeof(o->att)); add(&o->con, sizeof(o->con)); add(&o->acq, sizeof(o->acq));
     add(&ctx->stream, sizeof(ctx->stream));
     const Options& q = ctx->opt;
-    const int oo[16] = {q.zpass, q.rocfft ? 1 : 0, q.fused_rotate, q.poisson_queue, q.early_sum ? 1 : 0, q.fuse_tail ? 1 : 0, q.psf_overlap ? 1 : 0,
+    const int oo[17] = {q.zpass, q.rocfft ? 1 : 0, q.fused_rotate, q.poisson_queue, q.early_sum ? 1 : 0, q.fuse_tail ? 1 : 0, q.psf_overlap ? 1 : 0,
                         q.attenuate_scan ? 1 : 0, q.fused_fftx, q.zconv_strided ? 1 : 0, q.skip_empty ? 1 : 0, q.exp, q.poisson_queue_share, ctx->queue_share_learned,
-                        q.skip_rows ? 1 : 0, q.skip_tail ? 1 : 0};
+                        q.skip_rows ? 1 : 0, q.skip_tail ? 1 : 0, q.zpass_layout};
     add(oo, sizeof(oo));
     add(q.fft_pad, sizeof(q.fft_pad));
     return k;
diff --git a/multiview-simulation_amd/csrc/common.h b/multiview-simulation_amd/csrc/common.h
--- a/multiview-simulation_amd/csrc/common.h
+++ b/multiview-simulation_amd/csrc/common.h
@@ -143,6 +143,7 @@
     bool    early_sum = true;
     int     exp = 0;
     bool    zconv_strided = true;
+    int     zpass_layout = 0;
     bool    psf_overlap = true;
     int     tail_overlap = 1;
     bool    fuse_tail = false;
@@ -502,6 +503,7 @@
     bool    ymirror;
     bool    early;
     bool    zinline_auto;
+    bool    zlines_ok;
     int     hxp, pyb;
     int     e_rows;
     size_t spectrum_bytes(int nz_in, int nz_out, int nz_pitch, int views) const
@@ -521,6 +523,7 @@
 void custom_fft_release(mvsim_ctx* ctx);
 bool custom_fft_geometry(const int64_t dim[3], const int64_t kdim[3], int64_t g[5], const Options& opt);
 bool custom_zpass_geometry(const int64_t dim[3], const int64_t kdim[3], int inc, int64_t g[4], const Options& opt);
+bool custom_zpass_lines(const int64_t dim[3], const int64_t kdim[3], int inc, const Options& opt);
 bool fused_tail_geometry(const int64_t dim[3], const int64_t kdim[3], int inc, bool con_wanted, const Options& opt, ExtractPlan* fp);
 bool custom_fft_batchable(const mvsim_ctx* ctx, const int64_t dim[3], const int64_t kdim[3]);
 
diff --git a/multiview-simulation_amd/csrc/fft_driver.hip b/multiview-simulation_amd/csrc/fft_driver.hip
--- a/multiview-simulation_amd/csrc/fft_driver.hip
+++ b/multiview-simulation_amd/csrc/fft_driver.hip
@@ -142,6 +142,7 @@
     pl->hxp = (pl->M + 1 + tw_max - 1) / tw_max * tw_max;
     pl->pyb = (pl->py + ZB - 1) / ZB * ZB;
     pl->e_rows = find_len(pl->M)->nlx;
+    pl->zlines_ok = pl->zdirect && !(pl->py % 2 == 0 && lines_split_exists(pl->py / 2));
     return true;
 }
 
@@ -277,6 +278,15 @@
     const int zc = zs_chunk > 0 ? zs_chunk : zconv_chunk(nz, kz);
     g[0] = zs_chunk > 0 ? zstride : 0; g[1] = zc; g[2] = (nz + zc - 1) / zc; g[3] = pl.hxp / NLZ;
     return true;
+}
+
+bool custom_zpass_lines(const int64_t dim[3], const int64_t kdim[3], int inc, const Options& o)
+{
+    using namespace fft;
+    ConvPlan pl;
+    int64_t g[4];
+    if (!custom_zpass_geometry(dim, kdim, inc, g, o) || !conv_plan(dim, kdim, o, &pl)) return false;
+    return g[0] == 0 && pl.zlines_ok && !o.fuse_tail && o.zpass_layout != 1;
 }
 
 bool custom_fft_batchable(const mvsim_ctx* ctx, const int64_t dim[3], const int64_t kdim[3])
@@ -358,6 +368,7 @@
     int zs_chunk, zs_frows;
     size_t zs_lds;
     bool zinline;
+    bool zlines;
     long long corr_n;
     float corr_min, corr_target;
     const float2 *tw_m, *tw_px, *tw_py, *tw_pz;
@@ -382,6 +393,7 @@
     a.src_es = hxp; a.src_outer = (long long)hxp * ky;
     a.dst_es = hxp; a.dst_outer = r.plane;
     if (pl.zdirect) { a.dst_outer = (long long)ZB * hxp; a.dst_blk = (long long)kz * V * ZB * hxp; }
+    if (r.zlines) { a.dst_tile_major = 2; a.dst_es = (long long)kz * pl.py; a.dst_outer = pl.py; a.dst_blk = 0; }
     a.lmap = DimMap{ky, pl.py, ky - ky / 2, ky / 2, 1, ky / 2};
     MVSIM_TRY(launch_lines(ctx, pl.py, FWD, true, a, hxp / pl.tile_y, kz * V));
     if (pl.zdirect) return MVSIM_OK;
@@ -397,7 +409,7 @@
 static int psf_spectrum(mvsim_ctx* ctx, const ConvRun& r, const float* psf, PsfCache::Entry* entry, bool flags_follow)
 {
     hipStream_t s = ctx->stream;
-    const bool hit = entry && entry->filled;
+    const bool hit = entry && entry->filled && entry->layout == (r.zlines ? 1 : 0);
     const bool side = ctx->opt.psf_overlap && (int64_t)r.pl.n[0] * r.pl.n[1] * r.pl.n[2] >= (int64_t)1 << 24 && (!hit || flags_follow);
     ctx->psf_on_side = side;
     if (side) {
@@ -415,7 +427,7 @@
     ev_begin(ctx, ST_PSF);
     const int rc = psf_passes(ctx, r, psf);
     ev_end(ctx, ST_PSF);
-    if (entry && rc == MVSIM_OK) entry->filled = true;
+    if (entry) { entry->filled = rc == MVSIM_OK; entry->layout = r.zlines ? 1 : 0; }
     if (side) {
         ctx->stream = s;
         MVSIM_HIP(hipEventRecord(ctx->ev_join, ctx->side_stream));
@@ -471,6 +483,7 @@
         b.outer_skip_lo = pl.n[2] + kz / 2;
         b.outer_skip_len = std::max(0, pl.pz - (kz - 1 - kz / 2) - b.outer_skip_lo);
     }
+    if (r.zlines) { b.dst_tile_major = 2; b.dst_es = (long long)r.slab.nz_in * pl.py; b.dst_outer = pl.py; b.dst_blk = 0; }
     if (r.pnz) { b.nzflags = r.pnz; b.nz_stride = 1; }
     if (r.rowbits) { b.rowbits = r.rowbits; b.rowbits_stride = row_bits_words(pl.py); }
     ev_begin(ctx, ST_PASS_B);
@@ -511,8 +524,34 @@
     return MVSIM_OK;
 }
 
+static int zpass_lines(mvsim_ctx* ctx, const ConvRun& r)
+{
+    const ConvPlan& pl = r.pl;
+    const int kz = pl.k[2];
+    ZLinesArgs z{};
+    z.src = r.G; z.dst = r.F; z.taps = r.G2; z.hxp = pl.hxp; z.L = pl.py; z.nz = pl.n[2]; z.kz = kz; z.c = kz / 2;
+    z.zc = zconv_chunk(pl.n[2], kz);
+    z.flags = r.pnz; z.dil = r.pnz_dil;
+    const float scale_f = (float)(0.25 / ((double)pl.px * (double)pl.py));
+    const long long waves = zconv_lines_waves(pl.hxp, pl.py);
+    if (pl.early) {
+        MVSIM_TRY(ensure_box_weights(ctx, pl.n[0], pl.px, pl.hxp, true, &z.wx));
+        MVSIM_TRY(ensure_box_weights(ctx, pl.n[1], pl.py, pl.py, false, &z.wy));
+        MVSIM_TRY(ctx->partials_z.reserve((size_t)waves * sizeof(double)));
+        z.sum_partial = ctx->partials_z.as<double>();
+    }
+    MVSIM_TRY(launch_zconv_lines(ctx, z));
+    if (pl.early) {
+        hipLaunchKernelGGL(k_reduce_partials, dim3(1), dim3(1024), 0, ctx->stream, z.sum_partial, waves, r.scal, (double)scale_f,
+                           r.corr_n, r.corr_min, r.corr_target);
+        MVSIM_HIP(hipGetLastError());
+    }
+    return MVSIM_OK;
+}
+
 static int zpass_direct(mvsim_ctx* ctx, const ConvRun& r)
 {
+    if (r.zlines) return zpass_lines(ctx, r);
     const ConvPlan& pl = r.pl;
     const int kz = pl.k[2], hxp = pl.hxp, V = r.V;
     ZConvArgs z{};
@@ -565,6 +604,7 @@
     d.src = r.F; d.dst = dst; d.tw = r.tw_py; d.src_es = d.dst_es = hxp;
     d.src_outer = d.dst_outer = r.plane * r.zstride;
     if (pl.zdirect) { d.src_outer = (long long)ZB * hxp * r.zstride; d.src_blk = (long long)r.nzp * r.V * ZB * hxp; }
+    if (r.zlines) { d.src_lines = 1; d.src_es = (long long)r.nzp * pl.py; d.src_outer = (long long)pl.py * r.zstride; d.src_blk = 0; }
     d.lmap = DimMap{0, 0, 0, 0, 1, 0};
     d.outer_skip_lo = 1 << 30;
     d.store_limit = pl.n[1];
@@ -650,11 +690,17 @@
     r.zs_chunk = (pl.zdirect && r.zstride > 1 && o.zconv_strided && o.zpass != 3)
                      ? zconv_strided_chunk(slab.nz_out, kz, r.zstride, (o.exp & 2) != 0, &r.zs_frows, &r.zs_lds) : 0;
     r.zinline = pl.zdirect && !r.is_slab && r.zs_chunk == 0 && r.V == 1 && (o.zpass == 3 || pl.zinline_auto);
+    const bool lines_can = pl.zlines_ok && !r.zinline && r.zs_chunk == 0 && !r.is_slab && r.V == 1 && !fuse;
+    if (o.zpass_layout == 2 && !lines_can) {
+        set_error("zpass_layout=lines: this call keeps the z-blocked layout (a z slab, stacked views, the fused tail, another z kernel or split y lines)");
+        return MVSIM_EINVAL;
+    }
+    r.zlines = lines_can && o.zpass_layout != 1;
     const size_t g2_bytes = (size_t)r.V * pl.hxp * pl.pyb * kz * sizeof(float2);
     PsfCache::Entry* pe = ctx->psf_entry;
     ctx->psf_entry = nullptr;
     if (pe && !(r.V == 1 && !r.is_slab && pl.zdirect && !r.zinline && psf == pe->psf && pe->g2_bytes == g2_bytes)) pe = nullptr;
-    if (!(pe && pe->filled)) MVSIM_TRY(ctx->cfft_g1.reserve((size_t)r.V * pl.hxp * pl.k[1] * kz * sizeof(float2)));
+    if (!(pe && pe->filled && pe->layout == (r.zlines ? 1 : 0))) MVSIM_TRY(ctx->cfft_g1.reserve((size_t)r.V * pl.hxp * pl.k[1] * kz * sizeof(float2)));
     if (!pe) MVSIM_TRY(ctx->cfft_g2.reserve(g2_bytes));
     MVSIM_TRY(ctx->partials.reserve(PARTIALS_BYTES));
     MVSIM_TRY(ctx->partials_e.reserve((size_t)((rows_out_early + 3) / 4 + 16) * sizeof(double)));
diff --git a/multiview-simulation_amd/csrc/fft_host.h b/multiview-simulation_amd/csrc/fft_host.h
--- a/multiview-simulation_amd/csrc/fft_host.h
+++ b/multiview-simulation_amd/csrc/fft_host.h
@@ -1,5 +1,6 @@
 #pragma once
 #include "fft_dev.h"
+#include "zlines_geom.h"
 
 namespace mvsim {
 struct PItem;
@@ -18,6 +19,7 @@
     int           outer_skip_lo, outer_skip_len;
     int           store_limit;
     int           dst_tile_major;
+    int           src_lines;
     long long     src_blk, dst_blk;
     int           src_mirror;
     const int*    nzflags;
@@ -108,6 +110,19 @@
     long long     src_view, dst_view, taps_view;
 };
 
+struct ZLinesArgs {
+    const float2* src;
+    float2*       dst;
+    const float2* taps;
+    int           hxp, L, nz, kz, c;
+    int           zc;
+    const double2* wx;
+    const double2* wy;
+    double*       sum_partial;
+    const int*    flags;
+    const int*    dil;
+};
+
 template <class K> static int set_lds(mvsim_ctx* ctx, K kernel, size_t bytes)
 {
     return ensure_lds_attr(ctx, reinterpret_cast<const void*>(kernel), bytes);
@@ -124,6 +139,8 @@
 int       zconv_strided_chunk(int nz, int kz, int s, bool force, int* frows_out, size_t* lds_out);
 int       launch_zconv(mvsim_ctx* ctx, const ZConvArgs& args, int py, int views = 1);
 int       launch_zconv_strided(mvsim_ctx* ctx, const ZConvArgs& args, int py, size_t lds, int views = 1);
+long long zconv_lines_waves(int hxp, int L);
+int       launch_zconv_lines(mvsim_ctx* ctx, const ZLinesArgs& args);
 
 }
 
diff --git a/multiview-simulation_amd/csrc/fft_passes.hip b/multiview-simulation_amd/csrc/fft_passes.hip
--- a/multiview-simulation_amd/csrc/fft_passes.hip
+++ b/multiview-simulation_amd/csrc/fft_passes.hip
@@ -92,7 +92,25 @@
             }
         }
     }
-    float4 v[NIT];
+    constexpr bool SRC_LINES = MODE == INV && !SPARSE;
+    constexpr int WIT = (L / 2 + 63) / 64;
+    constexpr int NV = (SRC_LINES && LW * WIT > NIT) ? LW * WIT : NIT;
+    float4 v[NV];
+    bool from_lines = false;
+    if constexpr (SRC_LINES) {
+        if (p.src_lines) {
+            from_lines = true;
+            const float2* gl = p.src + (long long)(tile_x * NL + wave * LW) * p.src_es + (long long)by * p.src_outer;
+#pragma unroll
+            for (int j = 0; j < LW; ++j)
+#pragma unroll
+                for (int w = 0; w < WIT; ++w) {
+                    const int n2 = lane * 2 + w * 128;
+                    v[j * WIT + w] = make_float4(0.f, 0.f, 0.f, 0.f);
+                    if ((L % 128 == 0) || n2 < L) v[j * WIT + w] = *reinterpret_cast<const float4*>(gl + (long long)j * p.src_es + n2);
+                }
+        }
+    }
     bool under_bits = false;
     if constexpr (ROWBITS) {
         if (rec) {
@@ -122,7 +140,7 @@
             }
         }
     }
-    if (!under_bits) {
+    if (!under_bits && !from_lines) {
 #pragma unroll
     for (int it = 0; it < NIT; ++it) {
         const int n = r0 + it * ROWS;
@@ -157,6 +175,21 @@
         PLAN::template capture_first_pass<LW, IT1>(wbuf, lane, ps);
         __syncthreads();
     }
+    if constexpr (SRC_LINES) {
+        if (from_lines) {
+#pragma unroll
+            for (int j = 0; j < LW; ++j)
+#pragma unroll
+                for (int w = 0; w < WIT; ++w) {
+                    const int n2 = lane * 2 + w * 128;
+                    if ((L % 128 == 0) || n2 < L) {
+                        wbuf[j * LP + n2] = cconj(make_float2(v[j * WIT + w].x, v[j * WIT + w].y));
+                        wbuf[j * LP + n2 + 1] = cconj(make_float2(v[j * WIT + w].z, v[j * WIT + w].w));
+                    }
+                }
+        }
+    }
+    if (!from_lines) {
 #pragma unroll
     for (int it = 0; it < NIT; ++it) {
         const int n = r0 + it * ROWS;
@@ -167,6 +200,7 @@
             buf[(c2 + 1) * LP + n] = b;
         }
     }
+    }
     __syncthreads();
     MVSIM_STAMP(3);
     PLAN::template run<LW>(wbuf, tw, lane);
@@ -177,12 +211,15 @@
     }
     if constexpr (MODE == CONVZ) PLAN::template run_op<LW>(wbuf, tw, lane, LoadMulConjReg<IT1, R1>{ps});
     if (MODE == FWD && p.dst_tile_major) {
-        float2* gl = p.dst + (((long long)tile_o * gridDim.x + tile_x) * NL + (long long)wave * LW) * L;
+        const bool lm = p.dst_tile_major == 2;
+        float2* gl = lm ? p.dst + (long long)(tile_x * NL + wave * LW) * p.dst_es + (long long)by * p.dst_outer
+                        : p.dst + (((long long)tile_o * gridDim.x + tile_x) * NL + (long long)wave * LW) * L;
+        const long long ls = lm ? p.dst_es : (long long)L;
 #pragma unroll
         for (int j = 0; j < LW; ++j)
             for (int n2 = lane * 2; n2 < L; n2 += 128) {
                 const float2 a = wbuf[j * LP + n2], b = wbuf[j * LP + n2 + 1];
-                *reinterpret_cast<float4*>(gl + j * L + n2) = make_float4(a.x, a.y, b.x, b.y);
+                *reinterpret_cast<float4*>(gl + j * ls + n2) = make_float4(a.x, a.y, b.x, b.y);
             }
         return;
     }
@@ -411,8 +448,9 @@
         set_error("custom FFT: row bits on a pass that does not read them (length %d, mode %d)", L, mode);
         return MVSIM_EINVAL;
     }
+    if (a.src_lines && (mode != INV || sparse)) { set_error("custom FFT: line-major loads on a pass that has none (mode %d)", mode); return MVSIM_EINVAL; }
     const LinesSplitFn split = (L % 2 || a.rowbits) ? nullptr : lines_split_fn(L / 2);
-    if ((mode == FWD || mode == INV) && !sparse && !a.dst_tile_major && !(s->opt.exp & 8) && split && tiles % 2 == 0 &&
+    if ((mode == FWD || mode == INV) && !sparse && !a.dst_tile_major && !a.src_lines && !(s->opt.exp & 8) && split && tiles % 2 == 0 &&
         (!a.src_mirror || (a.lmap.mode == 0 && a.lmap.b < a.lmap.n && a.lmap.a - a.lmap.n < a.lmap.n))) {
         const float2* tw2 = nullptr;
         MVSIM_TRY(ensure_twiddles(s, L / 2, 0, &a.tw));
diff --git a/multiview-simulation_amd/csrc/psf_cache.h b/multiview-simulation_amd/csrc/psf_cache.h
--- a/multiview-simulation_amd/csrc/psf_cache.h
+++ b/multiview-simulation_amd/csrc/psf_cache.h
@@ -47,6 +47,7 @@
         void* psf = nullptr;
         size_t g2_bytes = 0, psf_bytes = 0;
         bool filled = false;
+        int layout = 0;
     };
     struct Stats { int64_t hits = 0, misses = 0, evictions = 0, bytes = 0; };
 
diff --git a/multiview-simulation_amd/csrc/zconv.hip b/multiview-simulation_amd/csrc/zconv.hip
--- a/multiview-simulation_amd/csrc/zconv.hip
+++ b/multiview-simulation_amd/csrc/zconv.hip
@@ -1,6 +1,7 @@
 #include "fft_host.h"
 
 #include <algorithm>
+#include <utility>
 
 namespace mvsim {
 namespace fft {
@@ -500,5 +501,168 @@
     MVSIM_HIP(hipGetLastError());
     return MVSIM_OK;
 }
-}
-}
+
+constexpr int zl_ahead(int kzp) { return kzp == 32 ? 4 : 8; }
+static_assert(ZL_TAP_PAD == ZJ, "the zero taps are k_zconv's");
+
+__device__ __forceinline__ void zl_cmac(v2f& acc, const v2f g, const float2 x)
+{
+    const v2f xv = v2f{x.x, x.y};
+    asm("v_pk_fma_f32 %0, %1, %2, %0 op_sel:[0,0,0] op_sel_hi:[0,1,1]" : "+v"(acc) : "v"(g), "v"(xv));
+    asm("v_pk_fma_f32 %0, %1, %2, %0 op_sel:[1,1,0] op_sel_hi:[1,0,1] neg_lo:[1,0,0]" : "+v"(acc) : "v"(g), "v"(xv));
+}
+
+__device__ __forceinline__ v2f zl_cmul(const v2f g, const float2 x)
+{
+    const v2f xv = v2f{x.x, x.y};
+    v2f acc;
+    asm("v_pk_fma_f32 %0, %1, %2, 0 op_sel:[0,0,0] op_sel_hi:[0,1,0]" : "=v"(acc) : "v"(g), "v"(xv));
+    asm("v_pk_fma_f32 %0, %1, %2, %0 op_sel:[1,1,0] op_sel_hi:[1,0,1] neg_lo:[1,0,0]" : "+v"(acc) : "v"(g), "v"(xv));
+    return acc;
+}
+
+template <int KZP> struct ZLinesWalk {
+    static constexpr int ZL_PF = zl_ahead(KZP);
+    static constexpr int W = KZP + ZL_PF;
+    const ZLinesArgs& p;
+    const int* __restrict__ flags;
+    const int* __restrict__ dil;
+    const float2* src;
+    long long     to_dst;
+    bool          own;
+    int           padf, l_next, zl;
+    unsigned int  fl;
+    int           last;
+    v2f           gt[KZP];
+    float2        w[W];
+    v2f           t1, t2, t4, t8;
+    double        sre, sim;
+
+    __device__ __forceinline__ ZLinesWalk(const ZLinesArgs& args) : p(args) {}
+    __device__ __forceinline__ int plane_of(int q) const { return (unsigned)q < (unsigned)p.nz ? q : zlines_mirror(q, p.nz); }
+    __device__ __forceinline__ int live_of(int i) const { return (unsigned)i < (unsigned)p.nz ? (dil ? dil[i] : 1) : 0; }
+    __device__ __forceinline__ void request(int q, int slot, int k)
+    {
+        const int qm = plane_of(q);
+        const int f = flags ? flags[qm] : 1;
+        fl = (fl & ~(1u << k)) | ((f ? 1u : 0u) << k);
+        last = f ? qm : last;
+        w[slot] = src[(long long)last * p.L];
+    }
+    __device__ __forceinline__ void clear(int slot, int k)
+    {
+        if (!flags) return;
+        const unsigned int m = ((fl >> k) & 1u) ? 0xFFFFFFFFu : 0u;
+        w[slot] = make_float2(__uint_as_float(__float_as_uint(w[slot].x) & m), __uint_as_float(__float_as_uint(w[slot].y) & m));
+    }
+    template <int B, int LOW> __device__ __forceinline__ void feed(v2f a, int i)
+    {
+        auto bit = [&](int k) { return (1 << k) < (1 << LOW) ? ((B >> k) & 1) != 0 : ((i >> k) & 1) != 0; };
+        if (!bit(0)) { t1 = a; return; }
+        a = t1 + a;
+        if (!bit(1)) { t2 = a; return; }
+        a = t2 + a;
+        if (!bit(2)) { t4 = a; return; }
+        a = t4 + a;
+        if (!bit(3)) { t8 = a; return; }
+        a = t8 + a;
+        sre += (double)a.x;
+        sim += (double)a.y;
+    }
+    template <int S> __device__ __forceinline__ void step(int i0)
+    {
+        const int i = i0 + S, nz = p.nz;
+        clear(S, S % ZL_PF);
+        const int l_now = l_next;
+        l_next = live_of(i + 1);
+        request(i + p.c + ZL_PF, (S + ZL_PF) % W, S % ZL_PF);
+        if (i < 0 || i >= nz) return;
+        v2f acc = v2f{0.f, 0.f};
+        if (l_now) {
+            acc = zl_cmul(gt[0], w[S]);
+#pragma unroll
+            for (int j = 1; j <= KZP - ZL_TAP_PAD; ++j) zl_cmac(acc, gt[j], w[(S - j + W) % W]);
+            if (zl >= padf) {
+#pragma unroll
+                for (int j = KZP - ZL_TAP_PAD + 1; j < KZP; ++j) zl_cmac(acc, gt[j], w[(S - j + W) % W]);
+            } else {
+#pragma unroll
+                for (int j = KZP - ZL_TAP_PAD + 1; j < KZP; ++j) {
+                    float2 x = w[(S - j + W) % W];
+                    if (!zlines_tap_reads(zl, j, p.kz, p.zc)) x = make_float2(0.f, 0.f);
+                    zl_cmac(acc, gt[j], x);
+                }
+            }
+            if (own) {
+                const char* at = reinterpret_cast<const char*>(src + (long long)i * p.L) + to_dst;
+                *reinterpret_cast<float2*>(const_cast<char*>(at)) = make_float2(acc.x, acc.y);
+            }
+        }
+        feed<S, 2>(acc, i);
+        zl = zl + 1 == p.zc ? 0 : zl + 1;
+    }
+    template <int... S> __device__ __forceinline__ void period(int i0, std::integer_sequence<int, S...>) { (step<S>(i0), ...); }
+};
+
+template <int KZP>
+__global__ __launch_bounds__(64, KZP <= 32 ? 3 : KZP <= 48 ? 2 : 1)
+void k_zconv_lines(ZLinesArgs p, const int* __restrict__ flags, const int* __restrict__ dil)
+{
+    constexpr int ZL_PF = zl_ahead(KZP), W = KZP + ZL_PF;
+    static_assert(KZP % ZL_TAP_PAD == 0 && (KZP + ZL_PF) % 4 == 0 && KZP % ZL_PF == 0, "whole chunks of taps; the low two bits of an output's index follow from its step");
+    const long long wave = blockIdx.x;
+    const int kx = zlines_wave_kx(wave, p.L), g = zlines_wave_group(wave, p.L);
+    const int lane = threadIdx.x, nz = p.nz, kz = p.kz, c = p.c, L = p.L;
+    ZLinesWalk<KZP> k(p);
+    k.flags = flags; k.dil = dil;
+    k.own = lane < zlines_lanes(g, L);
+    const unsigned int kyl = k.own ? 64u * g + lane : (unsigned int)(L - 1);
+    k.src = p.src + (long long)kx * nz * L + kyl;
+    k.to_dst = reinterpret_cast<const char*>(p.dst) - reinterpret_cast<const char*>(p.src);
+    k.padf = KZP - kz;
+    {
+        const float2* tp = p.taps + (long long)kx * kz * L;
+#pragma unroll
+        for (int j = 0; j < KZP; ++j) {
+            float2 t = make_float2(0.f, 0.f);
+            if (j <= KZP - ZL_TAP_PAD || j < kz) t = (tp + (long long)j * L)[kyl];
+            k.gt[j] = v2f{t.x, t.y};
+        }
+    }
+#pragma unroll
+    for (int j = 0; j < W; ++j) k.w[j] = make_float2(0.f, 0.f);
+    k.last = 0; k.fl = 0u;
+#pragma unroll
+    for (int q = 0; q < ZL_PF; ++q) k.request(-W + c + q, q, q);
+    k.l_next = 0;
+    k.zl = 0;
+    k.t1 = k.t2 = k.t4 = k.t8 = v2f{0.f, 0.f};
+    k.sre = k.sim = 0.0;
+    for (int i0 = -W; i0 < nz; i0 += W) k.period(i0, std::make_integer_sequence<int, W>{});
+    if (!p.sum_partial) return;
+    for (int i = nz; (i & 15) != 0; ++i) k.template feed<0, 0>(v2f{0.f, 0.f}, i);
+    const double2 wxa = p.wx[kx], wyb = p.wy[kyl];
+    const double wr = wxa.x * wyb.x - wxa.y * wyb.y, wi = wxa.x * wyb.y + wxa.y * wyb.x;
+    double t = k.own ? k.sre * wr - k.sim * wi : 0.0;
+#pragma unroll
+    for (int off = 32; off > 0; off >>= 1) t += __shfl_down(t, off, 64);
+    if (lane == 0) p.sum_partial[wave] = t;
+}
+
+long long zconv_lines_waves(int hxp, int L) { return zlines_waves(hxp, L); }
+
+int launch_zconv_lines(mvsim_ctx* ctx, const ZLinesArgs& a)
+{
+    const dim3 grid((unsigned)zlines_waves(a.hxp, a.L));
+    switch (zlines_kzp(a.kz)) {
+#define MVSIM_ZL_CASE(K) case K: hipLaunchKernelGGL(k_zconv_lines<K>, grid, dim3(64), 0, ctx->stream, a, a.flags, a.dil); break;
+    MVSIM_ZL_CASE(8) MVSIM_ZL_CASE(16) MVSIM_ZL_CASE(24) MVSIM_ZL_CASE(32)
+    MVSIM_ZL_CASE(40) MVSIM_ZL_CASE(48) MVSIM_ZL_CASE(56) MVSIM_ZL_CASE(64)
+#undef MVSIM_ZL_CASE
+    default: set_error("k_zconv_lines: %d taps", a.kz); return MVSIM_EINVAL;
+    }
+    MVSIM_HIP(hipGetLastError());
+    return MVSIM_OK;
+}
+}
+}
diff --git a/multiview-simulation_amd/csrc/zlines_geom.h b/multiview-simulation_amd/csrc/zlines_geom.h
--- /dev/null
+++ b/multiview-simulation_amd/csrc/zlines_geom.h
@@ -0,0 +1,34 @@
+#pragma once
+
+#if defined(__HIPCC__) || defined(__CUDACC__)
+#define MVSIM_ZL_HD __host__ __device__
+#else
+#define MVSIM_ZL_HD
+#endif
+
+namespace mvsim {
+namespace fft {
+
+constexpr int ZL_TAP_PAD = 8;
+
+MVSIM_ZL_HD constexpr int zlines_kzp(int kz) { return (kz + ZL_TAP_PAD - 1) / ZL_TAP_PAD * ZL_TAP_PAD; }
+MVSIM_ZL_HD constexpr int zlines_groups(int L) { return (L + 63) / 64; }
+MVSIM_ZL_HD constexpr long long zlines_waves(int hxp, int L) { return (long long)hxp * zlines_groups(L); }
+MVSIM_ZL_HD constexpr int zlines_wave_kx(long long wave, int L) { return (int)(wave / zlines_groups(L)); }
+MVSIM_ZL_HD constexpr int zlines_wave_group(long long wave, int L) { return (int)(wave % zlines_groups(L)); }
+MVSIM_ZL_HD constexpr int zlines_lanes(int g, int L) { return L - 64 * g < 64 ? L - 64 * g : 64; }
+MVSIM_ZL_HD constexpr long long zlines_index(int kx, int z, int ky, int nz, int L) { return ((long long)kx * nz + z) * L + ky; }
+
+MVSIM_ZL_HD inline int zlines_mirror(int i, int n)
+{
+    if (n == 1) return 0;
+    const int p = 2 * n - 2;
+    i %= p;
+    if (i < 0) i += p;
+    return i < n ? i : p - i;
+}
+
+MVSIM_ZL_HD inline bool zlines_tap_reads(int z, int j, int kz, int zc) { return j <= (z % zc) + kz - 1; }
+
+}
+}
```

Result: no change. 88080 (-0.3%).
